# syncdoth/face_mask_inpaint

Hardware: AMD Instinct MI355X
Metric: train images/sec at 256x256 bs=8 per GPU (PICNet-ref train step) (higher is better)
Workload: dtype f32; 1 GPU; train_reference_fill.py PICNet-ref 256x256 fp32, bs=8 per GPU, synthetic CelebA-HQ-shaped batch + random binary_map (BASELINE configs[1]); global_batch=8, parallelism=dp1

## Files before the change

face_mask_inpaint_amd/_lib.py:

```python
from __future__ import annotations

import ctypes as C
import os

_HERE = os.path.dirname(os.path.abspath(__file__))
LIB_PATH = os.path.join(_HERE, "csrc", "libfmi_hip.so")

c_f = C.c_void_p
i32, i64, f32, f64, vp = C.c_int, C.c_int64, C.c_float, C.c_double, C.c_void_p


class ConvDesc(C.Structure):

    _fields_ = [(n, C.c_int) for n in ("N", "H", "W", "C", "OH", "OW", "K", "x_cstride", "y_cstride", "kh", "kw", "stride", "pad", "pad_mode", "dil")] + [("w3", C.c_void_p), ("x3", C.c_void_p), ("y3", C.c_void_p)]


class WeightEntry(C.Structure):
    _fields_ = [("w", vp), ("u", vp), ("v", vp), ("wf", vp), ("wt", vp), ("sigma", vp), ("rows", i32), ("C", i32), ("taps", i32), ("iters", i32), ("wf3", vp), ("wt3", vp)]


class WeightGradEntry(C.Structure):
    _fields_ = [("w", vp), ("u", vp), ("v", vp), ("sigma", vp), ("dwf", vp), ("dw", vp), ("rows", i32), ("C", i32), ("taps", i32), ("pad_", i32)]


class AdamEntry(C.Structure):
    _fields_ = [("p", vp), ("g", vp), ("m", vp), ("v", vp), ("n", i64)]


class RangerEntry(C.Structure):
    _fields_ = [("p", vp), ("g", vp), ("m", vp), ("v", vp), ("slow", vp), ("row_mean", vp), ("n", i64), ("cols", i64)]


PD = C.POINTER(ConvDesc)

SIGNATURES = {
    "fmi_gemm_f32": [vp, vp, vp, i32, i32, i32, i64, i64, i64, i64, i64, i64, i32, i64, i64, i64, f32, f32, vp, vp],
    "fmi_ssim_valid_f32": [vp, vp, vp, i32, i32, i32, i32, f32, f32, vp, vp, i64, vp],
    "fmi_avgpool2_pad_f32": [vp, vp, i32, i32, i32, i32, i32, vp],
    "fmi_resample_u8": [vp, vp, i32, i32, i32, i32, i32, i32, i32, i32, vp, vp, i32, vp],
    "fmi_gather_u8_i64": [vp, vp, i32, i32, i32, i32, i32, vp, vp, vp],
    "fmi_u8_lut_chw_f32": [vp, vp, vp, i32, i32, i32, i32, vp],
    "fmi_split3_f32": [vp, vp, vp, i64, i32, i32, f32, vp],
    "fmi_split3_colsum_f32": [vp, vp, vp, i64, i32, vp],
    "fmi_merge3_f32": [vp, vp, i64, i32, vp],
    "fmi_conv2d_fwd_f32": [PD, vp, vp, vp, vp, vp, i32, i32, i64, vp],
    "fmi_conv2d_dgrad_f32": [PD, vp, vp, vp, vp, vp, i32, i64, vp],
    "fmi_conv_transpose2d_pair_f32": [PD, vp, vp, i32, vp, vp, vp, vp],
    "fmi_conv_transpose2d_pair_bwd_f32": [PD, vp, vp, i32, vp, vp, vp, vp, vp, vp, vp, vp, vp, i64, vp],
    "fmi_conv2d_dgrad_masked_f32": [PD, vp, vp, vp, f32, vp, vp],
    "fmi_conv2d_dgrad_masked_add_f32": [PD, vp, vp, vp, f32, vp, vp, vp],
    "fmi_conv2d_wgrad_f32": [PD, vp, vp, vp, vp, i32, i64, vp],
    "fmi_conv2d_thin_fwd_f32": [PD, vp, vp, vp, vp, vp, i32, vp],
    "fmi_conv2d_thin_dgrad_f32": [PD, vp, vp, vp, vp],
    "fmi_conv2d_thin_input_dgrad_f32": [PD, vp, vp, vp, vp],
    "fmi_conv2d_thin_in_fwd_f32": [PD, vp, vp, vp, vp, vp, i32, vp],
    "fmi_conv2d_thin_in_wgrad_f32": [PD, vp, vp, vp, vp, vp, i64, vp],
    "fmi_conv2d_thin_lrelu_fwd_f32": [PD, vp, f32, vp, vp, vp, i32, vp],
    "fmi_conv2d_thin_lrelu_fwd_bf16": [PD, vp, f32, vp, vp, vp, i32, vp],
    "fmi_conv2d_thin_lrelu_dgrad_f32": [PD, vp, vp, vp, f32, vp, vp],
    "fmi_conv2d_thin_lrelu_wgrad_f32": [PD, vp, f32, vp, vp, vp, vp],
    "fmi_conv2d_thin_wgrad_f32": [PD, vp, vp, vp, vp, vp],
    "fmi_conv2d_thin_lrelu_bwd_f32": [PD, vp, f32, vp, vp, vp, vp, vp, vp, vp, i64, vp],
    "fmi_conv2d_fwd_bf16": [PD, vp, vp, vp, vp, vp, i64, vp],
    "fmi_conv2d_dgrad_bf16": [PD, vp, vp, vp, vp, vp, i64, vp],
    "fmi_conv2d_wgrad_bf16": [PD, vp, vp, vp, vp],
    "fmi_pack_weight_bf16": [vp, vp, i32, i32, i32, vp],
    "fmi_scale_channels_bf16": [vp, vp, vp, i32, i64, i32, vp],
    "fmi_scale_channels_gs_bf16": [vp, vp, vp, vp, i64, i32, i64, i32, vp],
    "fmi_noise_bias_act_bf16": [vp, vp, vp, vp, vp, i64, i32, f32, f32, vp],
    "fmi_noise_bias_act_bwd_bf16": [vp, vp, vp, vp, vp, vp, vp, i64, i64, i32, f32, f32, vp],
    "fmi_upfirdn2d_nhwc_bf16": [vp, vp, vp] + [i32] * 14 + [vp],
    "fmi_styled_out_bwd_bf16": [vp] * 11 + [i64, vp, i32, i64, i32, f32, f32, vp],
    "fmi_conv2d_fwd_act_bf16": [PD, vp, vp, vp, vp, vp, vp, f32, f32, vp, vp],
    "fmi_conv2d_fwd_chan_bf16": [PD, vp, vp, vp, vp, vp, vp, vp, i64, vp],
    "fmi_se_gate_f32": [vp, i32, i64, f32, vp, vp, vp, i32, i32, vp],
    "fmi_irse_tail_bf16": [vp] * 8 + [i32] * 7 + [vp],
    "fmi_irse_stem_bf16": [vp] * 5 + [i64, i32, vp],
    "fmi_conv2d_thin_in_fwd_bf16": [PD, vp, vp, vp, f32, vp, vp],
    "fmi_conv2d_c32_fwd_bf16": [PD, vp, vp, vp, f32, vp, vp],
    "fmi_resblock_tail_bf16": [vp] * 5 + [i32] * 5 + [f32, vp],
    "fmi_picnet_stem_tail_bf16": [vp] * 6 + [i32] * 5 + [f32, vp],
    "fmi_guided_attention_fwd_bf16": [vp] * 5 + [i32] * 5 + [vp],
    "fmi_blur_act_bf16": [vp, vp, vp] + [i32] * 8 + [vp, vp, vp, vp, f32, f32, i32, vp],
    "fmi_torgb_fwd_bf16": [vp, vp, vp, vp, vp, vp, i32, i64, i32, vp],
    "fmi_torgb_bwd_bf16": [vp, vp, vp, vp, vp, vp, i64, vp, vp, vp, i32, i64, i32, vp],
    "fmi_bias_grad_f32": [vp, i64, i32, i32, vp, vp],
    "fmi_reflect_pad_fold_f32": [vp, vp, i32, i32, i32, i32, i32, vp],
    "fmi_weight_prepare_f32": [vp, i32, vp],
    "fmi_weight_grad_f32": [vp, i32, vp, vp],
    "fmi_softmax_rows_f32": [vp, vp, i64, i32, vp],
    "fmi_softmax_rows_bwd_f32": [vp, vp, vp, i64, i32, vp],
    "fmi_attention_fwd_f32": [vp, vp, vp, vp, vp, vp, i32, i32, i32, i32, i32, vp],
    "fmi_attention_fwd_bf16": [vp] * 6 + [i32] * 5 + [vp],
    "fmi_attention_bwd_f32": [vp] * 12 + [i32] * 5 + [vp],
    "fmi_attention_fwd_image_bytes": [i32, i32, i32, i32, i32, C.POINTER(i64)],
    "fmi_attention_fwd_pieces_f32": [vp] * 4 + [i64] + [vp] * 3 + [i32] * 5 + [vp],
    "fmi_attention_bwd_image_bytes": [i32, i32, i32, i32, i32, C.POINTER(i64)],
    "fmi_attention_bwd_pieces_f32": [vp] * 10 + [i64] + [vp] * 3 + [i32] * 5 + [vp],
    "fmi_eltwise_f32": [i32, vp, vp, vp, i64, f32, vp],
    "fmi_axpy_dev_f32": [vp, vp, vp, vp, i64, vp],
    "fmi_dot_f32": [vp, vp, i64, f32, vp, vp],
    "fmi_mask_binarise_i64": [vp, vp, i64, vp],
    "fmi_mask_mul_f32": [vp, vp, vp, i64, i32, i32, vp],
    "fmi_guide_blend_f32": [vp, vp, vp, vp, i64, i32, i32, vp],
    "fmi_guide_blend_bwd_f32": [vp, vp, vp, vp, i64, i32, i32, vp],
    "fmi_vae_sample_f32": [vp, vp, vp, vp, vp, i64, i32, vp],
    "fmi_vae_sample_bwd_f32": [vp, vp, vp, vp, vp, vp, vp, i64, i32, vp],
    "fmi_avgpool_f32": [vp, vp, i32, i32, i32, i32, i32, vp],
    "fmi_avgpool_bwd_f32": [vp, vp, i32, i32, i32, i32, i32, vp],
    "fmi_maxpool2_f32": [vp, vp, i32, i32, i32, i32, vp],
    "fmi_maxpool2_bf16": [vp, vp, i32, i32, i32, i32, vp],
    "fmi_maxpool2_bwd_bf16": [vp, vp, vp, i32, i32, i32, i32, vp],
    "fmi_up2_cat_bf16": [vp, vp, vp, i32, i32, i32, i32, i32, i32, i32, vp],
    "fmi_up2_cat_bwd_bf16": [vp, vp, vp, i32, i32, i32, i32, i32, i32, i32, vp],
    "fmi_head1x1_bf16": [vp, vp, vp, vp, i64, i32, i32, vp],
    "fmi_head1x1_argmax_bf16": [vp, vp, vp, vp, i64, i32, i32, vp],
    "fmi_head1x1_bwd_bf16": [vp, vp, vp, vp, vp, vp, vp, i64, i64, i32, i32, vp],
    "fmi_adaptive_avgpool_f32": [vp, vp, i32, i32, i32, i32, i32, i32, vp],
    "fmi_adaptive_avgpool_bwd_f32": [vp, vp, i32, i32, i32, i32, i32, i32, vp],
    "fmi_maxpool_f32": [vp, vp, vp, i32, i32, i32, i32, i32, i32, vp],
    "fmi_maxpool_bwd_f32": [vp, vp, vp, i32, i32, i32, i32, i32, i32, vp],
    "fmi_argmax_channels_f32": [vp, vp, i64, i32, vp],
    "fmi_image_tail_f32": [vp, vp, vp, vp, i32, i32, f32, f32, vp],
    "fmi_planes_to_u8_f32": [vp, vp, i32, i32, i32, i32, f32, f32, vp],
    "fmi_instnorm_stats_bf16": [vp, vp, vp, i32, i32, i32, f32, vp, i64, vp],
    "fmi_instnorm_apply_bf16": [vp, vp, vp, vp, vp, i32, i32, i32, f32, vp],
    "fmi_instnorm_bwd_reduce_bf16": [vp, vp, vp, vp, vp, vp, i32, i32, i32, f32, vp, i64, vp],
    "fmi_instnorm_bwd_apply_bf16": [vp, vp, vp, vp, vp, vp, vp, vp, vp, vp, i32, i32, i32, f32, vp],
    "fmi_prelu_bf16": [vp, vp, vp, i64, i32, vp],
    "fmi_prelu_bwd_bf16": [vp, vp, vp, vp, vp, vp, i64, i64, i32, vp],
    "fmi_scale_channels_add_bf16": [vp, vp, vp, vp, i32, i64, i32, vp],
    "fmi_add_bf16": [vp, vp, vp, i64, vp],
    "fmi_global_avgpool_bf16": [vp, vp, vp, i64, i32, i64, i32, vp],
    "fmi_add_bcast_bf16": [vp, vp, vp, i32, i64, i32, vp],
    "fmi_add_bcast_f32": [vp, vp, vp, i32, i64, i32, vp],
    "fmi_scale_channels_bwd_f32": [vp, vp, vp, vp, vp, vp, i64, i32, i64, i32, vp],
    "fmi_subsample_bf16": [vp, vp, i32, i32, i32, i32, i32, i32, vp],
    "fmi_scale_channels_add_f32": [vp, vp, vp, vp, i32, i64, i32, vp],
    "fmi_instnorm_bwd_apply_add_f32": [vp, vp, vp, vp, vp, vp, vp, vp, vp, vp, i32, i32, i32, f32, vp],
    "fmi_copy_channels_f32": [vp, vp, i64, i32, i32, i32, i32, i32, vp],
    "fmi_copy_channels_bf16": [vp, vp, i64, i32, i32, i32, i32, i32, vp],
    "fmi_l2norm_rows_f32": [vp, vp, vp, i64, i32, f32, vp],
    "fmi_l2norm_rows_bwd_f32": [vp, vp, vp, vp, i64, i32, f32, vp],
    "fmi_lpips_layer_f32": [vp, vp, vp, vp, i64, i32, f32, vp],
    "fmi_lpips_layer_bwd_f32": [vp, vp, vp, vp, vp, vp, i64, i32, f32, vp],
    "fmi_maxpool2_bwd_f32": [vp, vp, vp, i32, i32, i32, i32, vp],
    "fmi_resize_bilinear_f32": [vp, vp, i32, i32, i32, i32, i32, i32, vp, vp, vp],
    "fmi_resize_bilinear_bwd_f32": [vp, vp, i32, i32, i32, i32, i32, i32, vp, vp],
    "fmi_instnorm_stats_f32": [vp, vp, vp, i32, i32, i32, f32, vp, i64, vp],
    "fmi_batchnorm_running_update_f32": [vp, vp, vp, vp, vp, i32, i64, f32, f32, vp],
    "fmi_batchnorm_running_update_offset_f32": [vp, vp, vp, vp, vp, vp, i32, i64, f32, f32, vp],
    "fmi_instnorm_apply_f32": [vp, vp, vp, vp, vp, i32, i32, i32, f32, vp],
    "fmi_instnorm_bwd_reduce_f32": [vp, vp, vp, vp, vp, vp, i32, i32, i32, f32, vp, i64, vp],
    "fmi_instnorm_bwd_apply_f32": [vp, vp, vp, vp, vp, vp, vp, vp, vp, i32, i32, i32, f32, vp],
    "fmi_reduce_loss_f32": [i32, vp, vp, i64, f32, f32, vp, vp],
    "fmi_reduce_loss_bwd_f32": [i32, vp, vp, i64, f32, f32, vp, vp, vp],
    "fmi_ssim_f32": [vp, vp, vp, i32, i32, i32, i32, i32, vp, vp],
    "fmi_seg_ce_dice_fwd_f32": [vp, vp, i32, i64, i32, f64, vp, vp, vp, i64, vp],
    "fmi_seg_ce_dice_bwd_f32": [vp, vp, i32, i64, i32, f64, vp, vp, vp, vp],
    "fmi_seg_dice_score_f32": [vp, vp, i32, i32, i64, i32, f64, vp, vp, i64, vp],
    "fmi_plane_sums_f32": [vp, vp, i32, i64, vp, vp, i64, vp],
    "fmi_psp_pixel_head_fwd_f32": [vp, vp, vp, vp, vp, vp, vp, vp, i32, i32, i32, i32, vp, i64, vp],
    "fmi_psp_pixel_head_bwd_f32": [vp, vp, vp, vp, vp, vp, vp, vp, i32, i32, i32, i32, vp],
    "fmi_gan_image_head_fwd_f32": [vp, vp, vp, vp, vp, vp, vp, vp, vp, vp, i32, i32, i32, i32, i32, i32, vp, i64, vp],
    "fmi_gan_image_head_bwd_f32": [vp, vp, vp, vp, vp, vp, vp, i32, i32, i32, i32, i32, i32, vp],
    "fmi_cx_channel_mean_f32": [vp, vp, i64, i32, vp],
    "fmi_cx_normalise_f32": [vp, vp, vp, vp, i64, i32, vp],
    "fmi_cx_normalise_bwd_f32": [vp, vp, vp, vp, i64, i32, vp],
    "fmi_cx_rows_f32": [vp, vp, vp, vp, vp, i32, i32, f32, vp],
    "fmi_cx_cols_f32": [vp, vp, vp, i32, i32, vp],
    "fmi_cx_loss_f32": [vp, vp, vp, i32, i32, f32, vp],
    "fmi_cx_bwd_f32": [vp, vp, vp, vp, vp, vp, vp, vp, vp, i32, i32, f32, f32, vp],
    "fmi_adam_step_f32": [vp, i32, i64, f32, f32, f32, f32, f32, i32, vp],
    "fmi_adam_step_dev_f32": [vp, i32, f32, f32, f32, f32, f32, vp, vp],
    "fmi_adam_step_dev_guarded_f32": [vp, i32, f32, f32, f32, f32, f32, vp, vp, vp],
    "fmi_ranger_step_f32": [vp, i32, f32, f32, f32, f32, f32, f32, i32, f32, i32, vp],
    "fmi_upfirdn2d_f32": [vp, vp, vp, i32, i32, i32, i32, i32, i32, i32, i32, i32, i32, i32, i32, i32, vp],
    "fmi_upfirdn2d_bf16": [vp, vp, vp, i32, i32, i32, i32, i32, i32, i32, i32, i32, i32, i32, i32, i32, vp],
    "fmi_fused_bias_act_f32": [vp, vp, vp, vp, i64, i32, i32, i32, i32, f32, f32, vp],
    "fmi_fused_bias_act_bf16": [vp, vp, vp, vp, i64, i32, i32, i32, i32, f32, f32, vp],
    "fmi_scale_channels_f32": [vp, vp, vp, i32, i64, i32, vp],
    "fmi_scale_channels_gs_f32": [vp, vp, vp, vp, i64, i32, i64, i32, vp],
    "fmi_sqsum_last_f32": [vp, vp, i64, i32, vp],
    "fmi_sqsum_last_bwd_f32": [vp, vp, vp, i64, i32, vp],
    "fmi_noise_bias_act_bwd_f32": [vp, vp, vp, vp, vp, i64, i32, f32, f32, vp],
    "fmi_upfirdn2d_nhwc_f32": [vp, vp, vp, i32, i32, i32, i32, i32, i32, i32, i32, i32, i32, i32, i32, i32, i32, vp],
    "fmi_prelu_f32": [vp, vp, vp, i64, i32, vp],
    "fmi_prelu_bwd_f32": [vp, vp, vp, vp, vp, vp, i64, i64, i32, vp],
    "fmi_subsample_f32": [vp, vp, i32, i32, i32, i32, i32, i32, vp],
    "fmi_bias_grad_nchw_f32": [vp, i32, i32, i64, vp, vp],
    "fmi_bias_grad_nchw_bf16": [vp, i32, i32, i64, vp, vp],
    "fmi_noise_bias_act_f32": [vp, vp, vp, vp, vp, i64, i32, f32, f32, vp],
}

STATUS = {0: "ok", 1: "bad argument", 2: "unsupported shape/mode", 3: "kernel launch failed"}


PREDICATES = {"fmi_debug_bf16_tile": [i32], "fmi_set_deterministic": [i32], "fmi_get_deterministic": [], "fmi_conv2d_thin_supported": [PD], "fmi_conv2d_bf16_supported": [PD], "fmi_conv2d_thin_lrelu_supported": [PD], "fmi_conv2d_thin_lrelu_bwd_ws_bytes": [PD], "fmi_conv2d_thin_in_supported": [PD], "fmi_conv2d_thin_in_routed": [PD], "fmi_conv2d_thin_in_wgrad_ws_bytes": [PD], "fmi_conv_transpose2d_pair_bwd_supported": [PD, i32, i32], "fmi_conv_transpose2d_pair_bwd_ws_bytes": [PD, i32, i32], "fmi_attention_fwd_uses_pieces": [i32] * 5, "fmi_attention_bwd_uses_pieces": [i32] * 5, "fmi_attention_fwd_waves": [i32] * 2, "fmi_attention_fwd_bf16_waves": [i32] * 2, "fmi_guided_attention_fwd_bf16_waves": [i32] * 2, "fmi_attention_bwd_structure": [i32] * 2}


class FmiError(RuntimeError):
    pass


class Library:

    def __init__(self, path: str = LIB_PATH, strict: bool = True):
        if not os.path.exists(path):
            raise FmiError(
                f"{path} not found: build the HIP extension first (python -c 'import __graft_entry__ as g; g.build()'). "
                "There is no CPU fallback."
            )
        self.path = path
        self.cdll = C.CDLL(path)
        self.missing = []
        for name, argtypes in SIGNATURES.items():
            try:
                fn = getattr(self.cdll, name)
            except AttributeError:
                self.missing.append(name)
                continue
            fn.argtypes = argtypes
            fn.restype = C.c_int
            setattr(self, name[4:], self._checked(name, fn))
        for name, argtypes in PREDICATES.items():
            try:
                fn = getattr(self.cdll, name)
            except AttributeError:
                self.missing.append(name)
                continue
            fn.argtypes = argtypes
            fn.restype = C.c_int
            setattr(self, name[4:], fn)
        if strict and self.missing:
            raise FmiError(f"{path} lacks symbols {self.missing}")

    @staticmethod
    def _checked(name, fn):
        def call(*args):
            rc = fn(*args)
            if rc != 0:
                raise FmiError(f"{name} failed: {STATUS.get(rc, rc)}")

        call.__name__ = name
        return call


_LIB = None


def lib() -> Library:
    global _LIB
    if _LIB is None:
        _LIB = Library(os.environ.get("FMI_LIB_PATH", LIB_PATH))
    return _LIB
```

face_mask_inpaint_amd/csrc/conv.hip:

```cpp
#include "gemm_core.h"
#include "conv3x3.h"
#include "conv_p3.h"
#include "convt3x3.h"

static bool aligned16(const void* p) { return ((uintptr_t)p & 15) == 0; }
static int ep_vec(const ConvEp& ep, int Nout) {
  return Nout % 4 == 0 && ep.cstride % 4 == 0 && aligned16(ep.y) && aligned16(ep.bias) && aligned16(ep.res) && aligned16(ep.mask);
}

static int check_desc(const fmi_conv_desc* d) {
  if (!d) return FMI_ERR_BAD_ARG;
  if (d->N <= 0 || d->H <= 0 || d->W <= 0 || d->C <= 0 || d->K <= 0 || d->kh <= 0 || d->kw <= 0 || d->stride <= 0 ||
      d->pad < 0 || d->x_cstride < d->C || d->y_cstride < d->K)
    return FMI_ERR_BAD_ARG;
  const int pe = d->pad, dl = d->dil > 1 ? d->dil : 1;
  if (d->dil < 0 || (dl > 1 && d->pad_mode)) return FMI_ERR_BAD_ARG;
  if (d->OH != (d->H + 2 * pe - dl * (d->kh - 1) - 1) / d->stride + 1 || d->OW != (d->W + 2 * pe - dl * (d->kw - 1) - 1) / d->stride + 1)
    return FMI_ERR_BAD_ARG;
  if (d->OH <= 0 || d->OW <= 0) return FMI_ERR_BAD_ARG;
  if (d->pad_mode == 1 && (d->pad >= d->H || d->pad >= d->W)) return FMI_ERR_UNSUPPORTED;
  if (d->pad_mode != 0 && d->pad_mode != 1) return FMI_ERR_UNSUPPORTED;
  if ((int64_t)d->N * d->H * d->W > 0x7fffffffLL / 2 || (int64_t)d->kh * d->kw * d->C > 0x3fffffffLL) return FMI_ERR_UNSUPPORTED;
  return FMI_OK;
}

static ConvGeom fwd_geom(const fmi_conv_desc* d, const float* x, int n_eff) {
  ConvGeom g{};
  g.N = n_eff; g.IH = d->H; g.IW = d->W; g.C = d->C; g.cstride = d->x_cstride;
  g.GH = d->OH; g.GW = d->OW; g.S = d->stride;
  const int dl = d->dil > 1 ? d->dil : 1;
  g.nty = d->kh; g.ntx = d->kw; g.dy0 = -d->pad; g.dx0 = -d->pad; g.ystep = dl; g.xstep = dl;
  g.kh0 = 0; g.kw0 = 0; g.khstep = 1; g.kwstep = 1; g.kw = d->kw;
  g.pad_mode = d->pad_mode;
  g.vec = (d->C % 4 == 0) && (d->x_cstride % 4 == 0) && aligned16(x);
  g.dGW = make_fastdiv(g.GW); g.dG = make_fastdiv(g.GH * g.GW); g.dC = make_fastdiv(g.C); g.dntx = make_fastdiv(g.ntx);
  g.img_bs = (int64_t)d->H * d->W * d->x_cstride;
  return g;
}

static ConvGeom adj_geom(const fmi_conv_desc* d, const float* dy, int n_eff, int py, int px) {
  const int s = d->stride, dl = d->dil > 1 ? d->dil : 1;
  ConvGeom g{};
  g.N = n_eff; g.IH = d->OH; g.IW = d->OW; g.C = d->K; g.cstride = d->y_cstride;
  g.GH = (d->H - py + s - 1) / s; g.GW = (d->W - px + s - 1) / s; g.S = 1;
  g.kh0 = (py + d->pad) % s; g.kw0 = (px + d->pad) % s;
  g.nty = g.kh0 < d->kh ? (d->kh - g.kh0 + s - 1) / s : 0;
  g.ntx = g.kw0 < d->kw ? (d->kw - g.kw0 + s - 1) / s : 0;
  g.dy0 = (py + d->pad - g.kh0) / s; g.dx0 = (px + d->pad - g.kw0) / s;
  g.ystep = -dl; g.xstep = -dl; g.khstep = s; g.kwstep = s; g.kw = d->kw;
  g.pad_mode = 0;
  g.vec = (d->K % 4 == 0) && (d->y_cstride % 4 == 0) && aligned16(dy);
  g.dGW = make_fastdiv(g.GW); g.dG = make_fastdiv(g.GH * g.GW); g.dC = make_fastdiv(g.C);
  g.dntx = make_fastdiv(g.ntx > 0 ? g.ntx : 1);
  g.img_bs = (int64_t)d->OH * d->OW * d->y_cstride;
  if (g.nty == 0 || g.ntx == 0) { g.nty = 0; g.ntx = 1; }
  return g;
}

#ifndef FMI_HOST_EMU
__global__ void __launch_bounds__(256) conv_split_init_kernel(float* __restrict__ y, const float* __restrict__ bias,
                                                             const float* __restrict__ res, int K, int cstride, int64_t total) {
  for (int64_t i = (int64_t)blockIdx.x * 256 + threadIdx.x; i < total; i += (int64_t)gridDim.x * 256) {
    const int k = (int)(i % K);
    const int64_t o = (i / K) * cstride + k;
    float v = bias ? bias[k] : 0.f;
    if (res) v += res[o];
    y[o] = v;
  }
}
#endif

static int conv_ksplit(int64_t M, int N, int K) {
#ifdef FMI_HOST_EMU
  return 1;
#else
  const int64_t tiles = ceil_div64(M, 128) * ceil_div64(N, N <= 32 ? 32 : (N <= 64 ? 64 : 128));
  if (K < 512 || fmi_det()) return 1;
  if (tiles >= 320) {
    if (tiles >= 800 || K < 2304) return 1;
    return tiles <= 520 ? 2 : 3;
  }
  if (tiles >= 192 && K < 4608) return 1;
  int64_t ks = ceil_div64(384, tiles);
  const int64_t kmin = (M <= 128 && tiles <= 16) ? 64 : 256;
  if (ks > K / kmin) ks = K / kmin;
  return ks < 2 ? 1 : (int)(ks > (kmin == 64 ? 64 : 16) ? (kmin == 64 ? 64 : 16) : ks);
#endif
}

static int conv_phase(const fmi_conv_desc* d, const ConvGeom& g, const float* x, const void* x3, const float* w, const void* w3p,
                      int64_t w_bstride, int Nout, int flip, ConvEp ep, int batch_w, bool may_split, bool shared_init, hipStream_t st) {
  ConvK la{x, g};
  ConvWX lb{w, g, w_bstride, Nout, (Nout % 4 == 0) && aligned16(w) && (w_bstride % 4 == 0)};
  const int ks = may_split ? conv_ksplit(g.Mdim(), Nout, g.Kdim()) : 1;
#ifndef FMI_HOST_EMU
  if (shared_init || ks > 1) {
    if (!shared_init) {
      const int64_t total = (int64_t)g.N * ep.OHt * ep.OWt * Nout;
      hipLaunchKernelGGL(conv_split_init_kernel, dim3(fmi_bw_grid(total, 256)), dim3(256), 0, st, ep.y, ep.bias, ep.res, Nout, ep.cstride,
                         total);
    }
    ep.bias = nullptr;
    ep.res = nullptr;
    ep.act = 3;
    ep.vec = 0;
  }
  const uint16_t* w3 = (const uint16_t*)w3p;
  const int64_t w3_stride = (int64_t)d->kh * d->kw * d->C * d->K;
  const int64_t pixels = (int64_t)g.N * g.IH * g.IW;
  const bool tap3 = d->kh == 3 && d->kw == 3 && d->stride == 1 && d->pad == 1 && d->dil <= 1 && g.pad_mode == 0;
  const bool p3 = batch_w == 1 && g.cstride == g.C && g.Kdim() > 0 && p3_generic_ok(g, x3, w3, Nout);
  if (p3 && tap3 && conv3x3_p3_eligible(x3, w3, g.C, Nout, pixels)) {
    const C3P3Args ca{(const uint16_t*)x3, w3, g.N, g.IH, g.IW, g.C, Nout, flip, make_fastdiv(g.IW), make_fastdiv(g.IH * g.IW)};
    return launch_conv3x3_p3(ca, ep, g.Mdim(), ks, st);
  }
  if (p3)
    return launch_gemm_p3(ConvK3{(const uint16_t*)x3, g, make_fastdiv(g.ntaps())}, ConvWX3{w3, g, w3_stride, Nout}, ep, g.Mdim(), Nout,
                          g.Kdim(), ks, st);
  if (batch_w == 1 && tap3 && conv3x3_eligible(x, w, g.C, g.cstride, Nout, pixels)) {
    const C3Args ca{x, w, g.N, g.IH, g.IW, g.C, g.cstride, Nout, flip, make_fastdiv(g.IW), make_fastdiv(g.IH * g.IW), w3};
    return launch_conv3x3(ca, ep, g.Mdim(), ks, st);
  }
  if (w3 && la.dma_ok()) return launch_gemm(la, ConvWX3{w3, g, w3_stride, Nout}, ep, g.Mdim(), Nout, g.Kdim(), 1, ks, st);
#endif
  return launch_gemm(la, lb, ep, g.Mdim(), Nout, g.Kdim(), batch_w, ks, st);
}

static const void* weight_pieces(const fmi_conv_desc* d, int batch_w, int red_c) {
#ifndef FMI_HOST_EMU
  if (batch_w == 1 && red_c % 16 == 0 && aligned16(d->w3)) return d->w3;
#endif
  return nullptr;
}

static int check_y3(const fmi_conv_desc* d, int out_c, int out_cs) {
  if (!d->y3) return FMI_OK;
  return (out_c % 16 == 0 && out_cs == out_c && aligned16(d->y3)) ? FMI_OK : FMI_ERR_BAD_ARG;
}

extern "C" int fmi_conv2d_fwd_f32(const fmi_conv_desc* d, const float* x, const float* wf, const float* bias,
                                  const float* residual, float* y, int act, int batch_w, int64_t w_bstride,
                                  void* stream) {
  if (!d) return FMI_ERR_BAD_ARG;
  int rc = check_y3(d, d->K, d->y_cstride);
  if (rc) return rc;
  rc = check_desc(d);
  if (rc) return rc;
  if (!x || !wf || !y || batch_w < 1 || act < 0 || act > 2) return FMI_ERR_BAD_ARG;
  if (batch_w > 1 && batch_w != d->N) return FMI_ERR_BAD_ARG;
  auto finish = [&](int rc) {
#ifndef FMI_HOST_EMU
    if (rc == FMI_OK && d->y3) rc = fmi_split3_f32(y, d->y3, nullptr, (int64_t)d->N * d->OH * d->OW, d->K, 0, 0.f, stream);
#endif
    return rc;
  };
#ifndef FMI_HOST_EMU
  if (batch_w == 1 && fmi_conv2d_thin_supported(d) && aligned16(x))
    return finish(fmi_conv2d_thin_fwd_f32(d, x, wf, bias, residual, y, act, stream));
  if (batch_w == 1 && d->kh == 3 && fmi_conv2d_thin_in_routed(d) && aligned16(y) && aligned16(residual))
    return finish(fmi_conv2d_thin_in_fwd_f32(d, x, wf, bias, residual, y, act, stream));
#endif
  const ConvGeom g = fwd_geom(d, x, batch_w > 1 ? 1 : d->N);
  const void* w3 = weight_pieces(d, batch_w, d->C);
  ConvEp ep{y, bias, residual, d->OH, d->OW, 1, 0, 0, d->OH, d->OW, d->y_cstride, act, g.dGW, g.dG, (int64_t)d->OH * d->OW * d->y_cstride};
  ep.vec = ep_vec(ep, d->K);
  return finish(conv_phase(d, g, x, d->x3, wf, w3, w_bstride, d->K, 0, ep, batch_w, act == 0 && batch_w == 1, false, (hipStream_t)stream));
}

static int dgrad_impl(const fmi_conv_desc* d, const float* dy, const float* wt, const float* bias, const float* residual,
                      const float* mask, float mslope, float* dx, int batch_w, int64_t w_bstride, void* stream) {
  if (!d) return FMI_ERR_BAD_ARG;
  int rc = check_y3(d, d->C, d->x_cstride);
  if (rc) return rc;
  rc = check_desc(d);
  if (rc) return rc;
  if (!dy || !wt || !dx || batch_w < 1) return FMI_ERR_BAD_ARG;
  if (d->pad_mode != 0) return FMI_ERR_UNSUPPORTED;
  if (batch_w > 1 && batch_w != d->N) return FMI_ERR_BAD_ARG;
  if (mask && bias) return FMI_ERR_UNSUPPORTED;
  auto finish = [&](int rc) {
#ifndef FMI_HOST_EMU
    if (rc == FMI_OK && d->y3) rc = fmi_split3_f32(dx, d->y3, nullptr, (int64_t)d->N * d->H * d->W, d->C, 0, 0.f, stream);
#endif
    return rc;
  };
#ifndef FMI_HOST_EMU
  if (batch_w == 1 && !bias && !residual && !mask && fmi_conv2d_thin_supported(d) && aligned16(dx))
    return finish(fmi_conv2d_thin_dgrad_f32(d, dy, wt, dx, stream));
  if (batch_w == 1 && !bias && !residual && !mask && d->C <= 4 && d->x_cstride == d->C && d->kh == 3) {
    const int rc_thin = fmi_conv2d_thin_input_dgrad_f32(d, dy, wt, dx, stream);
    if (rc_thin != FMI_ERR_UNSUPPORTED) return finish(rc_thin);
  }
#endif
  const int n_eff = batch_w > 1 ? 1 : d->N;
  const int s = d->stride;
  const void* w3 = weight_pieces(d, batch_w, d->K);
  if (d->dil > 1 && s != 1) return FMI_ERR_UNSUPPORTED;
  bool strided_split = false;
#ifndef FMI_HOST_EMU
  if (s > 1 && batch_w == 1) {
    for (int py = 0; py < s && !strided_split; ++py)
      for (int px = 0; px < s && !strided_split; ++px) {
        const ConvGeom g = adj_geom(d, dy, n_eff, py, px);
        if (g.GH > 0 && g.GW > 0 && conv_ksplit(g.Mdim(), d->C, g.Kdim()) > 1) strided_split = true;
      }
    if (strided_split) {
      const int64_t total = (int64_t)d->N * d->H * d->W * d->C;
      hipLaunchKernelGGL(conv_split_init_kernel, dim3(fmi_bw_grid(total, 256)), dim3(256), 0, (hipStream_t)stream, dx, bias, residual, d->C,
                         d->x_cstride, total);
    }
  }
  if (batch_w == 1 && !strided_split && !d->x3 && convt3x3_eligible(d, dy, (const uint16_t*)w3)) {
    CT3Args ca{};
    ca.x = dy; ca.w3 = (const uint16_t*)w3; ca.N = d->N; ca.H = d->OH; ca.W = d->OW; ca.Cred = d->K; ca.cs = d->y_cstride; ca.Nout = d->C;
    ca.dW = make_fastdiv(d->OW); ca.dHW = make_fastdiv(d->OH * d->OW);
    ConvEp ep{dx, bias, residual, d->OH, d->OW, 2, 0, 0, d->H, d->W, d->x_cstride, 0, ca.dW, ca.dHW, (int64_t)d->H * d->W * d->x_cstride};
    ep.mask = mask;
    ep.mslope = mslope;
    ep.vec = ep_vec(ep, d->C);
    ca.ep = ep;
    return finish(launch_convt3x3(ca, d->N * d->OH * d->OW, (hipStream_t)stream));
  }
#endif
  for (int py = 0; py < s; ++py) {
    for (int px = 0; px < s; ++px) {
      const ConvGeom g = adj_geom(d, dy, n_eff, py, px);
      if (g.GH <= 0 || g.GW <= 0) continue;
      ConvEp ep{dx, bias, residual, g.GH, g.GW, s, py, px, d->H, d->W, d->x_cstride, 0, g.dGW, g.dG,
                (int64_t)d->H * d->W * d->x_cstride};
      ep.mask = mask;
      ep.mslope = mslope;
      ep.vec = ep_vec(ep, d->C);
      rc = conv_phase(d, g, dy, d->x3, wt, w3, w_bstride, d->C, 1, ep, batch_w, batch_w == 1 && (s == 1 || strided_split), strided_split,
                      (hipStream_t)stream);
      if (rc) return rc;
    }
  }
  return finish(FMI_OK);
}
extern "C" int fmi_conv2d_dgrad_f32(const fmi_conv_desc* d, const float* dy, const float* wt, const float* bias,
                                    const float* residual, float* dx, int batch_w, int64_t w_bstride, void* stream) {
  return dgrad_impl(d, dy, wt, bias, residual, nullptr, 0.f, dx, batch_w, w_bstride, stream);
}
extern "C" int fmi_conv_transpose2d_pair_f32(const fmi_conv_desc* d, const float* x1, const float* x2, int K2, const void* w3b,
                                             const float* bias, float* y, void* stream) {
  int rc = check_desc(d);
  if (rc) return rc;
  if (!x1 || !x2 || !w3b || !d->w3 || !y || K2 <= 0) return FMI_ERR_BAD_ARG;
#ifndef FMI_HOST_EMU
  const uint16_t* w3 = (d->K % 16 == 0 && aligned16(d->w3)) ? (const uint16_t*)d->w3 : nullptr;
  if (!convt3x3_eligible(d, x1, w3) || (K2 & 15) || !aligned16(x2) || !aligned16(w3b) || d->pad_mode != 0 || d->x3) return FMI_ERR_UNSUPPORTED;
  CT3Args ca{};
  ca.x = x1; ca.w3 = w3; ca.x2 = x2; ca.w3b = (const uint16_t*)w3b; ca.Cred2 = K2; ca.cs2 = K2;
  ca.N = d->N; ca.H = d->OH; ca.W = d->OW; ca.Cred = d->K; ca.cs = d->y_cstride; ca.Nout = d->C;
  ca.dW = make_fastdiv(d->OW); ca.dHW = make_fastdiv(d->OH * d->OW);
  ConvEp ep{y, bias, nullptr, d->OH, d->OW, 2, 0, 0, d->H, d->W, d->x_cstride, 0, ca.dW, ca.dHW, (int64_t)d->H * d->W * d->x_cstride};
  ep.vec = ep_vec(ep, d->C);
  ca.ep = ep;
  return launch_convt3x3(ca, d->N * d->OH * d->OW, (hipStream_t)stream);
#else
  return FMI_ERR_UNSUPPORTED;
#endif
}
extern "C" int fmi_conv2d_dgrad_masked_f32(const fmi_conv_desc* d, const float* dy, const float* wt, const float* mask, float mask_slope,
                                           float* dx, void* stream) {
  if (!mask) return FMI_ERR_BAD_ARG;
  return dgrad_impl(d, dy, wt, nullptr, nullptr, mask, mask_slope, dx, 1, 0, stream);
}

extern "C" int fmi_conv2d_dgrad_masked_add_f32(const fmi_conv_desc* d, const float* dy, const float* wt, const float* mask, float mask_slope,
                                               const float* gadd, float* dx, void* stream) {
  if (!mask || !gadd) return FMI_ERR_BAD_ARG;
  return dgrad_impl(d, dy, wt, nullptr, gadd, mask, mask_slope, dx, 1, 0, stream);
}

extern "C" int fmi_conv2d_wgrad_f32(const fmi_conv_desc* d, const float* x, const float* dy, float* dwf, float* dbias,
                                    int batch_w, int64_t w_bstride, void* stream) {
  int rc = check_desc(d);
  if (rc) return rc;
  if (!x || !dy || !dwf || batch_w < 1) return FMI_ERR_BAD_ARG;
  if (batch_w > 1 && batch_w != d->N) return FMI_ERR_BAD_ARG;
#ifndef FMI_HOST_EMU
  if (batch_w == 1 && fmi_conv2d_thin_supported(d) && aligned16(x)) return fmi_conv2d_thin_wgrad_f32(d, x, dy, dwf, dbias, stream);
#endif
#ifndef FMI_HOST_EMU
  if (batch_w == 1 && !dbias && wgrad_p3_ok(d, d->x3, d->y3))
    return launch_wgrad_p3(d, (const uint16_t*)d->x3, (const uint16_t*)d->y3, dwf, (hipStream_t)stream);
#endif
  const int n_eff = batch_w > 1 ? 1 : d->N;
  ConvGeom g = fwd_geom(d, x, n_eff);
  const bool fuse_bias = dbias && batch_w == 1 && (g.Kdim() % 4 == 0);
  if (dbias && !fuse_bias) return FMI_ERR_UNSUPPORTED;
  const int ones_row = fuse_bias ? g.Kdim() : -1;
  const int Mg = g.Kdim() + (fuse_bias ? 1 : 0), Ng = d->K, Kg = g.Mdim();
  WgradAX la{x, g, ones_row};
  DenseX lb{dy, (int64_t)d->y_cstride, (int64_t)d->OH * d->OW * d->y_cstride, Ng, Kg,
            (d->K % 4 == 0) && (d->y_cstride % 4 == 0) && aligned16(dy)};
  WgradEp ep{dwf, g, d->K, w_bstride, dbias, ones_row};
  const int64_t tiles = ceil_div64(Mg, 128) * ceil_div64(Ng, Ng <= 32 ? 32 : (Ng <= 64 ? 64 : 128));
  int64_t ksplit = 2048 / (tiles * batch_w);
  const int64_t kmax = Kg / 512;
  if (ksplit > kmax) ksplit = kmax;
  if (ksplit < 1) ksplit = 1;
  if (fmi_det()) ksplit = 1;
  if (ksplit * batch_w > 65535) ksplit = 65535 / batch_w;
  return launch_gemm(la, lb, ep, Mg, Ng, Kg, batch_w, (int)ksplit, (hipStream_t)stream);
}

#ifndef FMI_HOST_EMU
__global__ void __launch_bounds__(256) bias_grad_vec_f64_kernel(const float* __restrict__ g, int64_t rows, int K4, float* __restrict__ dbias) {
  __shared__ double part[256][4];
  const int cg = threadIdx.x % K4, rl = threadIdx.x / K4, RL = 256 / K4;
  double s[4] = {0, 0, 0, 0};
  for (int64_t r = rl; r < rows; r += RL) {
    const float4 v = reinterpret_cast<const float4*>(g)[r * K4 + cg];
    s[0] += v.x, s[1] += v.y, s[2] += v.z, s[3] += v.w;
  }
#pragma unroll
  for (int e = 0; e < 4; ++e) part[threadIdx.x][e] = s[e];
  __syncthreads();
  if (threadIdx.x < K4) {
    double t[4] = {0, 0, 0, 0};
    for (int l = 0; l < RL; ++l)
#pragma unroll
      for (int e = 0; e < 4; ++e) t[e] += part[l * K4 + threadIdx.x][e];
#pragma unroll
    for (int e = 0; e < 4; ++e) atomicAdd(dbias + 4 * threadIdx.x + e, (float)t[e]);
  }
}
__global__ void __launch_bounds__(256) bias_grad_vec_kernel(const float* __restrict__ g, int64_t rows, int K4,
                                                            float* __restrict__ dbias, int64_t rows_per_block) {
  __shared__ float4 part[256];
  const int cg = threadIdx.x % K4, rl = threadIdx.x / K4, RL = 256 / K4;
  const int64_t r0 = (int64_t)blockIdx.x * rows_per_block;
  int64_t r1 = r0 + rows_per_block;
  if (r1 > rows) r1 = rows;
  float4 s = make_float4(0.f, 0.f, 0.f, 0.f);
  int64_t r = r0 + rl;
  for (; r + 3 * RL < r1; r += 4 * RL) {
    const float4 v0 = reinterpret_cast<const float4*>(g)[r * K4 + cg];
    const float4 v1 = reinterpret_cast<const float4*>(g)[(r + RL) * K4 + cg];
    const float4 v2 = reinterpret_cast<const float4*>(g)[(r + 2 * RL) * K4 + cg];
    const float4 v3 = reinterpret_cast<const float4*>(g)[(r + 3 * RL) * K4 + cg];
    s.x += (v0.x + v1.x) + (v2.x + v3.x);
    s.y += (v0.y + v1.y) + (v2.y + v3.y);
    s.z += (v0.z + v1.z) + (v2.z + v3.z);
    s.w += (v0.w + v1.w) + (v2.w + v3.w);
  }
  for (; r < r1; r += RL) {
    const float4 v = reinterpret_cast<const float4*>(g)[r * K4 + cg];
    s.x += v.x; s.y += v.y; s.z += v.z; s.w += v.w;
  }
  part[threadIdx.x] = s;
  __syncthreads();
  if (threadIdx.x < K4) {
    float4 t = part[threadIdx.x];
    for (int l = 1; l < RL; ++l) {
      const float4 v = part[l * K4 + threadIdx.x];
      t.x += v.x; t.y += v.y; t.z += v.z; t.w += v.w;
    }
    atomicAdd(dbias + 4 * threadIdx.x + 0, t.x);
    atomicAdd(dbias + 4 * threadIdx.x + 1, t.y);
    atomicAdd(dbias + 4 * threadIdx.x + 2, t.z);
    atomicAdd(dbias + 4 * threadIdx.x + 3, t.w);
  }
}
__global__ void __launch_bounds__(256) bias_grad_kernel(const float* __restrict__ g, int64_t rows, int K, int cstride,
                                                        float* __restrict__ dbias, int64_t rows_per_block) {
  __shared__ float part[4][64];
  const int tx = threadIdx.x & 63, ty = threadIdx.x >> 6;
  const int64_t r0 = (int64_t)blockIdx.x * rows_per_block;
  int64_t r1 = r0 + rows_per_block;
  if (r1 > rows) r1 = rows;
  for (int cg = 0; cg < K; cg += 64) {
    const int c = cg + tx;
    float s = 0.f;
    if (c < K)
      for (int64_t r = r0 + ty; r < r1; r += 4) s += g[r * cstride + c];
    part[ty][tx] = s;
    __syncthreads();
    if (ty == 0 && c < K) atomicAdd(dbias + c, part[0][tx] + part[1][tx] + part[2][tx] + part[3][tx]);
    __syncthreads();
  }
}

extern "C" int fmi_bias_grad_f32(const float* g, int64_t rows, int K, int cstride, float* dbias, void* stream) {
  if (!g || !dbias || rows <= 0 || K <= 0 || cstride < K) return FMI_ERR_BAD_ARG;
// ... 48 lines not shown
```

face_mask_inpaint_amd/csrc/gemm_core.h:

```cpp
#pragma once
#include "common.h"
#include <cstdio>
#include <cstdlib>
extern "C" long fmi_debug_launch_counter;
#include <type_traits>

#ifndef FMI_HOST_EMU
#include "x6.h"
#endif

struct FastDiv {
  uint32_t m, s1, s2, d;
};
static inline FastDiv make_fastdiv(uint32_t d) {
  FastDiv f;
  if (d == 0) d = 1;
  f.d = d;
  uint32_t l = 0;
  while ((1ull << l) < d) ++l;
  f.m = (uint32_t)(((1ull << 32) * ((1ull << l) - d)) / d + 1);
  f.s1 = l < 1 ? l : 1;
  f.s2 = l > 0 ? l - 1 : 0;
  return f;
}
// ... 261 lines not shown
    const uint16_t* q = p3 + (((int64_t)wtap * g.C + c) >> 3) * Nout * 8 + (int64_t)x * 8 + (c & 7);
    const float x0 = __uint_as_float((uint32_t)q[0] << 16), x1 = __uint_as_float((uint32_t)q[pstride] << 16), x2 = __uint_as_float((uint32_t)q[2 * pstride] << 16);
    return (x2 + x1) + x0;
  }
  __device__ __forceinline__ float4 load4(const Ctx&, int x, int k) const { return make_float4(elem(x, k), elem(x + 1, k), elem(x + 2, k), elem(x + 3, k)); }
  __host__ __device__ __forceinline__ bool dma_ok() const { return (g.C & 15) == 0 && ((uintptr_t)p3 & 15) == 0; }
  struct DCtx {
    int64_t off;
  };
  struct Tile {
    const uint16_t* base;
  };
  __device__ __forceinline__ DCtx dprep3(int piece, int kg, int x) const { return DCtx{x < Nout ? piece * pstride + ((int64_t)kg * Nout + x) * 8 : -1}; }
  __device__ __forceinline__ Tile tile(int k0) const {
    const int t = (int)fdiv((uint32_t)k0, g.dC);
    if (t >= g.ntaps()) return Tile{nullptr};
    const int i = (int)fdiv((uint32_t)t, g.dntx), j = t - i * g.ntx;
    const int wtap = (g.kh0 + g.khstep * i) * g.kw + (g.kw0 + g.kwstep * j);
    return Tile{p3 + (((int64_t)wtap * g.C + (k0 - t * g.C)) >> 3) * Nout * 8};
  }
  __device__ __forceinline__ const void* chunk(const DCtx& d, const Tile& t) const { return (d.off >= 0 && t.base) ? (const void*)(t.base + d.off) : nullptr; }
};
#endif

struct WgradAX {
  static constexpr bool KMODE = false;
  const float* p;
  ConvGeom g;
  int ones_row;
  struct Ctx {
    int t0, c0;
  };
  __device__ __forceinline__ void set_batch(int b) { p += (int64_t)b * g.img_bs; }
  __device__ __forceinline__ Ctx prep(int x) const {
    Ctx c;
    c.t0 = (int)fdiv((uint32_t)x, g.dC);
    c.c0 = x - c.t0 * g.C;
    return c;
  }
  __device__ __forceinline__ float elem_tc(int t, int c, int n, int gy, int gx) const {
    if (t >= g.ntaps()) return 0.f;
    const int i = (int)fdiv((uint32_t)t, g.dntx), j = t - i * g.ntx;
    int iy = gy * g.S + g.dy0 + g.ystep * i, ix = gx * g.S + g.dx0 + g.xstep * j;
    if (g.pad_mode) {
      iy = reflect_idx(iy, g.IH);
      ix = reflect_idx(ix, g.IW);
    }
    if ((unsigned)iy >= (unsigned)g.IH || (unsigned)ix >= (unsigned)g.IW) return 0.f;
    return p[((int64_t)(n * g.IH + iy) * g.IW + ix) * g.cstride + c];
  }
  __device__ __forceinline__ float4 load4(const Ctx& cx, int x, int k) const {
    const int t0 = cx.t0, c0 = cx.c0;
    if (k >= g.Mdim()) return zero4();
    if (x == ones_row) return make_float4(1.f, 0.f, 0.f, 0.f);
    const uint32_t n = fdiv((uint32_t)k, g.dG);
    const uint32_t rem = (uint32_t)k - n * (uint32_t)(g.GH * g.GW);
    const uint32_t gy = fdiv(rem, g.dGW);
    const uint32_t gx = rem - gy * (uint32_t)g.GW;
    if (g.vec) {
      if (t0 >= g.ntaps()) return zero4();
      const int i = (int)fdiv((uint32_t)t0, g.dntx), j = t0 - i * g.ntx;
      int iy = (int)gy * g.S + g.dy0 + g.ystep * i, ix = (int)gx * g.S + g.dx0 + g.xstep * j;
      if (g.pad_mode) {
        iy = reflect_idx(iy, g.IH);
        ix = reflect_idx(ix, g.IW);
      }
      if ((unsigned)iy >= (unsigned)g.IH || (unsigned)ix >= (unsigned)g.IW) return zero4();
      return ldg4(p + ((int64_t)((int)n * g.IH + iy) * g.IW + ix) * g.cstride + c0);
    }
    float v[4];
#pragma unroll
    for (int e = 0; e < 4; ++e) {
      const int xe = x + e;
      const int t = (int)fdiv((uint32_t)xe, g.dC);
      v[e] = elem_tc(t, xe - t * g.C, (int)n, (int)gy, (int)gx);
    }
    return make_float4(v[0], v[1], v[2], v[3]);
  }
  __host__ __device__ __forceinline__ bool dma_ok() const { return g.vec != 0; }
  struct DCtx {
    Ctx c;
    int x, kr, dy, dx;
    int k, n, gy, gx;
  };
  struct Tile {
    int k0;
  };
  __device__ __forceinline__ void dstart(DCtx& d, int k_begin) const {
    d.k = k_begin + d.kr;
    const uint32_t n = fdiv((uint32_t)d.k, g.dG);
    const uint32_t rem = (uint32_t)d.k - n * (uint32_t)(g.GH * g.GW);
    const uint32_t gy = fdiv(rem, g.dGW);
    d.n = (int)n;
    d.gy = (int)gy;
    d.gx = (int)(rem - gy * (uint32_t)g.GW);
  }
  __device__ __forceinline__ void advance(DCtx& d) const {
    d.k += 16;
    d.gx += 16;
    while (d.gx >= g.GW) {
      d.gx -= g.GW;
      if (++d.gy == g.GH) {
        d.gy = 0;
        ++d.n;
      }
    }
  }
  __device__ __forceinline__ DCtx dprep(int x, int kr) const {
    DCtx d;
    d.c = prep(x);
    d.x = x;
    d.kr = kr;
    const int i = (int)fdiv((uint32_t)d.c.t0, g.dntx), j = d.c.t0 - i * g.ntx;
    d.dy = g.dy0 + g.ystep * i;
    d.dx = g.dx0 + g.xstep * j;
    return d;
  }
  __device__ __forceinline__ Tile tile(int k0) const { return Tile{k0}; }
  __device__ __forceinline__ const float* chunk(const DCtx& d, const Tile& t) const;
};

struct DenseEp {
  static constexpr bool HAS_VEC4 = false;
  float* c;
  const float* bias;
  int64_t sc_m, sc_n, bs;
  float alpha, beta;
  int atomic;
  __device__ __forceinline__ void set_batch(int b) { c += (int64_t)b * bs; }
  __device__ __forceinline__ int64_t row_off(int row) const { return (int64_t)row * sc_m; }
  __device__ __forceinline__ void store(int64_t off, int col, float v) const {
    float* q = c + off + (int64_t)col * sc_n;
    v *= alpha;
    if (bias) v += bias[col];
    if (atomic) {
      atomicAdd(q, v);
      return;
    }
    if (beta != 0.f) v += beta * *q;
    *q = v;
  }
};

struct ConvEp {
  float* y;
  const float* bias;
  const float* res;
  int GH, GW, OS, py, px, OHt, OWt, cstride, act;
  FastDiv dGW, dG;
  int64_t bs;
  int vec = 0;
  const float* mask = nullptr;
  float mslope = 0.f;
  static constexpr bool HAS_VEC4 = true;
  __device__ __forceinline__ void set_batch(int b) {
    y += (int64_t)b * bs;
    if (res) res += (int64_t)b * bs;
    if (mask) mask += (int64_t)b * bs;
  }
  __device__ __forceinline__ void store4(int64_t off, int col, float4 v) const {
    if (mask) {
      const float4 m4 = *reinterpret_cast<const float4*>(mask + off + col);
      v.x *= m4.x > 0.f ? 1.f : mslope, v.y *= m4.y > 0.f ? 1.f : mslope, v.z *= m4.z > 0.f ? 1.f : mslope, v.w *= m4.w > 0.f ? 1.f : mslope;
    }
    if (bias) {
      const float4 b4 = *reinterpret_cast<const float4*>(bias + col);
      v.x += b4.x, v.y += b4.y, v.z += b4.z, v.w += b4.w;
    }
    if (res) {
      const float4 r4 = *reinterpret_cast<const float4*>(res + off + col);
      v.x += r4.x, v.y += r4.y, v.z += r4.z, v.w += r4.w;
    }
    if (act == 1) v.x = tanhf(v.x), v.y = tanhf(v.y), v.z = tanhf(v.z), v.w = tanhf(v.w);
    else if (act == 2) v.x = fmaxf(v.x, 0.f), v.y = fmaxf(v.y, 0.f), v.z = fmaxf(v.z, 0.f), v.w = fmaxf(v.w, 0.f);
    *reinterpret_cast<float4*>(y + off + col) = v;
  }
  __device__ __forceinline__ int64_t row_off(int row) const {
    const uint32_t n = fdiv((uint32_t)row, dG);
    const uint32_t rem = (uint32_t)row - n * (uint32_t)(GH * GW);
    const uint32_t gy = fdiv(rem, dGW);
    const uint32_t gx = rem - gy * (uint32_t)GW;
    return ((int64_t)((int)n * OHt + (int)gy * OS + py) * OWt + ((int)gx * OS + px)) * cstride;
  }
  __device__ __forceinline__ void store(int64_t off, int col, float v) const {
    if (mask) v *= mask[off + col] > 0.f ? 1.f : mslope;
    if (act == 3) {
      atomicAdd(y + off + col, v);
      return;
    }
    if (bias) v += bias[col];
    if (res) v += res[off + col];
    if (act == 1) v = tanhf(v);
    else if (act == 2) v = fmaxf(v, 0.f);
    y[off + col] = v;
  }
};

struct WgradEp {
  static constexpr bool HAS_VEC4 = false;
  float* dw;
  ConvGeom g;
  int Kout;
  int64_t bs;
  float* dbias;
  int ones_row;
  __device__ __forceinline__ void set_batch(int b) { dw += (int64_t)b * bs; }
  __device__ __forceinline__ int64_t row_off(int row) const {
    if (row == ones_row) return -1;
    const int t = (int)fdiv((uint32_t)row, g.dC);
    const int i = (int)fdiv((uint32_t)t, g.dntx), j = t - i * g.ntx;
    const int wtap = (g.kh0 + g.khstep * i) * g.kw + (g.kw0 + g.kwstep * j);
    return ((int64_t)wtap * g.C + (row - t * g.C)) * Kout;
  }
  __device__ __forceinline__ void store(int64_t off, int col, float v) const {
    if (off < 0) atomicAdd(dbias + col, v);
    else atomicAdd(dw + off + col, v);
  }
};

#ifndef FMI_HOST_EMU
__device__ __forceinline__ float dpp_quad(float v, bool stage2) {
  const int i = __float_as_int(v);
  return __int_as_float(stage2 ? __builtin_amdgcn_mov_dpp(i, 0x4E, 0xF, 0xF, true)
                               : __builtin_amdgcn_mov_dpp(i, 0xB1, 0xF, 0xF, true));
}
__device__ __forceinline__ void quad_transpose(float (&a)[4], int c) {
  const bool b0 = c & 1, b1 = c & 2;
#pragma unroll
  for (int p = 0; p < 4; p += 2) {
    const float recv = dpp_quad(b0 ? a[p] : a[p + 1], false);
    a[p] = b0 ? recv : a[p];
    a[p + 1] = b0 ? a[p + 1] : recv;
  }
#pragma unroll
  for (int q = 0; q < 2; ++q) {
    const float recv = dpp_quad(b1 ? a[q] : a[q + 2], true);
    a[q] = b1 ? recv : a[q];
    a[q + 2] = b1 ? a[q + 2] : recv;
  }
}

template <class EP, class T>
__device__ __forceinline__ void store_tile(const EP& ep, f32x16 (&acc)[T::TM][T::TN], int M, int N, int row0, int col0, int lh, int l31) {
  if constexpr (EP::HAS_VEC4) {
    if (ep.vec) {
      const int c = l31 & 3, colq = l31 & ~3;
#pragma unroll
      for (int i = 0; i < T::TM; ++i) {
#pragma unroll
        for (int g = 0; g < 4; ++g) {
          const int row = row0 + i * 32 + 8 * g + 4 * lh + c;
          const int64_t off = row < M ? ep.row_off(row) : 0;
#pragma unroll
          for (int j = 0; j < T::TN; ++j) {
            float a[4] = {acc[i][j][4 * g + 0], acc[i][j][4 * g + 1], acc[i][j][4 * g + 2], acc[i][j][4 * g + 3]};
            quad_transpose(a, c);
            const int col = col0 + j * 32 + colq;
            if (row < M && col < N) ep.store4(off, col, make_float4(a[0], a[1], a[2], a[3]));
          }
        }
      }
      return;
    }
  }
#pragma unroll
  for (int i = 0; i < T::TM; ++i) {
#pragma unroll
    for (int r = 0; r < 16; ++r) {
      const int row = row0 + i * 32 + (r & 3) + 8 * (r >> 2) + 4 * lh;
      if (row >= M) continue;
      const int64_t off = ep.row_off(row);
#pragma unroll
      for (int j = 0; j < T::TN; ++j) {
        const int col = col0 + j * 32 + l31;
        if (col < N) ep.store(off, col, acc[i][j][r]);
      }
    }
  }
}

static __device__ __attribute__((aligned(16))) float fmi_chunk_zero[4] = {0.f, 0.f, 0.f, 0.f};
__device__ __forceinline__ const float* fmi_zero_chunk_ptr() {
  const float* p = fmi_chunk_zero;
  asm volatile("" : "+s"(p));
  return p;
}
static __device__ __attribute__((aligned(16))) float fmi_chunk_one[4] = {1.f, 0.f, 0.f, 0.f};

__device__ __forceinline__ const float* WgradAX::chunk(const DCtx& d, const Tile&) const {
  if (d.k >= g.Mdim()) return nullptr;
  if (d.x == ones_row) return fmi_chunk_one;
  if (d.c.t0 >= g.ntaps()) return nullptr;
  const int n = d.n;
  int iy = d.gy * g.S + d.dy, ix = d.gx * g.S + d.dx;
  if (g.pad_mode) {
    iy = reflect_idx(iy, g.IH);
    ix = reflect_idx(ix, g.IW);
  }
  if ((unsigned)iy >= (unsigned)g.IH || (unsigned)ix >= (unsigned)g.IW) return nullptr;
  return p + ((int64_t)(n * g.IH + iy) * g.IW + ix) * g.cstride + d.c.c0;
}
#endif

#ifndef FMI_HOST_EMU
template <class LA, class LB, class EP, class T>
__global__ void __launch_bounds__(256) gemm_mfma_f32_kernel(LA la, LB lb, EP ep, int M, int N, int K, int tiles_n,
                                                            int ksplit, int kchunk) {
  constexpr int BM = T::BM, BN = T::BN, BK = T::BK, LDA = T::LDA, LDB = T::LDB;
  constexpr int NLA = BM / 64 > 0 ? BM / 64 : 1, NLB = BN / 64 > 0 ? BN / 64 : 1;
  __shared__ __attribute__((aligned(16))) float lds[2 * BK * (LDA + LDB)];
  float* As = lds;
  float* Bs = lds + 2 * BK * LDA;

  const int tid = threadIdx.x, lane = tid & 63, wid = tid >> 6;
  const int l31 = lane & 31, lh = lane >> 5;
  const int lid = xcd_remap(blockIdx.x, gridDim.x);
  const int tile_m = lid / tiles_n, tile_n = lid - tile_m * tiles_n;
  const int zb = blockIdx.y / ksplit, zs = blockIdx.y - zb * ksplit;
  la.set_batch(zb);
  lb.set_batch(zb);
  ep.set_batch(zb);
  const int m0 = tile_m * BM, n0 = tile_n * BN;
  const int k_begin = zs * kchunk;
  int k_end = k_begin + kchunk;
  if (k_end > K) k_end = K;
  const int wm = (wid / T::WN) * T::TM * 32, wn = (wid % T::WN) * T::TN * 32;

  int ax[NLA], ak[NLA], bx[NLB], bk[NLB];
  bool aact[NLA], bact[NLB];
  typename LA::Ctx ca[NLA];
  typename LB::Ctx cb[NLB];
#pragma unroll
  for (int j = 0; j < NLA; ++j) {
    if (LA::KMODE) {
      ax[j] = (tid >> 2) + 64 * j;
      ak[j] = (tid & 3) * 4;
      aact[j] = ax[j] < BM;
    } else {
      const int idx = tid + 256 * j;
      ak[j] = idx / (BM / 4);
      ax[j] = (idx % (BM / 4)) * 4;
      aact[j] = ak[j] < BK;
    }
    ca[j] = la.prep(m0 + ax[j]);
  }
#pragma unroll
  for (int j = 0; j < NLB; ++j) {
    if (LB::KMODE) {
// ... 451 lines not shown
```

face_mask_inpaint_amd/csrc/pool.hip:

```cpp
#include "common.h"


template <int V>
struct VecT;
template <>
struct VecT<1> {
  typedef float T;
  static __device__ __forceinline__ float zero() { return 0.f; }
  static __device__ __forceinline__ void add(float& a, float b) { a += b; }
  static __device__ __forceinline__ void scale(float& a, float s) { a *= s; }
};
template <>
struct VecT<4> {
  typedef float4 T;
  static __device__ __forceinline__ float4 zero() { return make_float4(0.f, 0.f, 0.f, 0.f); }
  static __device__ __forceinline__ void add(float4& a, float4 b) {
    a.x += b.x; a.y += b.y; a.z += b.z; a.w += b.w;
  }
  static __device__ __forceinline__ void scale(float4& a, float s) {
    a.x *= s; a.y *= s; a.z *= s; a.w *= s;
  }
};

template <int V>
__global__ void __launch_bounds__(256) avgpool_kernel(const float* __restrict__ x, float* __restrict__ y, int H, int W,
                                                      int CV, int k, int64_t total) {
  typedef typename VecT<V>::T T;
  const int OH = H / k, OW = W / k;
  const float inv = 1.f / (float)(k * k);
  for (int64_t i = (int64_t)blockIdx.x * 256 + threadIdx.x; i < total; i += (int64_t)gridDim.x * 256) {
    const int c = (int)(i % CV);
    int64_t r = i / CV;
    const int ox = (int)(r % OW);
    r /= OW;
    const int oy = (int)(r % OH);
    const int n = (int)(r / OH);
    T s = VecT<V>::zero();
    for (int a = 0; a < k; ++a)
      for (int b = 0; b < k; ++b)
        VecT<V>::add(s, reinterpret_cast<const T*>(x)[(((int64_t)n * H + oy * k + a) * W + ox * k + b) * CV + c]);
    VecT<V>::scale(s, inv);
    reinterpret_cast<T*>(y)[i] = s;
  }
}
template <int V>
__global__ void __launch_bounds__(256) avgpool_bwd_kernel(const float* __restrict__ gy, float* __restrict__ gx, int H,
                                                          int W, int CV, int k, int64_t total) {
  typedef typename VecT<V>::T T;
  const int OH = H / k, OW = W / k;
  const float inv = 1.f / (float)(k * k);
  for (int64_t i = (int64_t)blockIdx.x * 256 + threadIdx.x; i < total; i += (int64_t)gridDim.x * 256) {
    const int c = (int)(i % CV);
    int64_t r = i / CV;
    const int xx = (int)(r % W);
    r /= W;
    const int yy = (int)(r % H);
    const int n = (int)(r / H);
    T v = VecT<V>::zero();
    if (yy / k < OH && xx / k < OW) {
      v = reinterpret_cast<const T*>(gy)[(((int64_t)n * OH + yy / k) * OW + xx / k) * CV + c];
      VecT<V>::scale(v, inv);
    }
    reinterpret_cast<T*>(gx)[i] = v;
  }
}

__global__ void __launch_bounds__(256) global_avgpool_kernel(const float* __restrict__ x, float* __restrict__ y, int64_t HW, int C4,
                                                            int64_t rows_per_block, float inv) {
  __shared__ float4 part[256];
  const int cg = threadIdx.x % C4, rl = threadIdx.x / C4, RL = 256 / C4;
  const int n = blockIdx.y;
  const int64_t r0 = (int64_t)blockIdx.x * rows_per_block;
  int64_t r1 = r0 + rows_per_block;
  if (r1 > HW) r1 = HW;
  const float4* xp = reinterpret_cast<const float4*>(x) + (int64_t)n * HW * C4;
  float4 s = make_float4(0.f, 0.f, 0.f, 0.f);
  int64_t r = r0 + rl;
  for (; r + RL < r1; r += 2 * RL) {
    const float4 v0 = xp[r * C4 + cg], v1 = xp[(r + RL) * C4 + cg];
    s.x += v0.x + v1.x; s.y += v0.y + v1.y; s.z += v0.z + v1.z; s.w += v0.w + v1.w;
  }
  for (; r < r1; r += RL) {
    const float4 v = xp[r * C4 + cg];
    s.x += v.x; s.y += v.y; s.z += v.z; s.w += v.w;
  }
  part[threadIdx.x] = s;
  __syncthreads();
  if (threadIdx.x < C4) {
    float4 t = part[threadIdx.x];
    for (int l = 1; l < RL; ++l) {
      const float4 v = part[l * C4 + threadIdx.x];
      t.x += v.x; t.y += v.y; t.z += v.z; t.w += v.w;
    }
    float* o = y + ((int64_t)n * C4 + threadIdx.x) * 4;
    atomicAdd(o + 0, t.x * inv);
    atomicAdd(o + 1, t.y * inv);
    atomicAdd(o + 2, t.z * inv);
    atomicAdd(o + 3, t.w * inv);
  }
}

extern "C" int fmi_avgpool_f32(const float* x, float* y, int N, int H, int W, int C, int k, void* stream) {
  if (!x || !y || N <= 0 || H <= 0 || W <= 0 || C <= 0 || k <= 0 || H / k <= 0 || W / k <= 0) return FMI_ERR_BAD_ARG;
  {
    const int C4 = C / 4;
    if (k == H && k == W && k >= 8 && C % 4 == 0 && C4 <= 256 && (C4 & (C4 - 1)) == 0 && fmi_al16(x) && fmi_al16(y) && N <= 65535) {
      const int64_t HW = (int64_t)H * W;
      int64_t blocks = ceil_div64(HW, 128);
      if (blocks * N > 2048) blocks = ceil_div64(2048, N);
      if (fmi_det()) blocks = 1;
      const int64_t rpb = ceil_div64(HW, blocks);
      blocks = ceil_div64(HW, rpb);
      if (hipMemsetAsync(y, 0, (size_t)N * C * sizeof(float), (hipStream_t)stream) != hipSuccess) return FMI_ERR_LAUNCH;
      hipLaunchKernelGGL(global_avgpool_kernel, dim3((unsigned)blocks, (unsigned)N), dim3(256), 0, (hipStream_t)stream, x, y, HW, C4, rpb,
                         1.f / (float)HW);
      return fmi_launch_status();
    }
  }
  const bool v4 = (C % 4 == 0) && fmi_al16(x) && fmi_al16(y);
  const int CV = v4 ? C / 4 : C;
  const int64_t total = (int64_t)N * (H / k) * (W / k) * CV;
  if (v4) hipLaunchKernelGGL((avgpool_kernel<4>), dim3(fmi_bw_grid(total, 256)), dim3(256), 0, (hipStream_t)stream, x, y, H, W, CV, k, total);
  else hipLaunchKernelGGL((avgpool_kernel<1>), dim3(fmi_bw_grid(total, 256)), dim3(256), 0, (hipStream_t)stream, x, y, H, W, CV, k, total);
  return fmi_launch_status();
}
extern "C" int fmi_avgpool_bwd_f32(const float* gy, float* gx, int N, int H, int W, int C, int k, void* stream) {
  if (!gy || !gx || N <= 0 || H <= 0 || W <= 0 || C <= 0 || k <= 0 || H / k <= 0 || W / k <= 0) return FMI_ERR_BAD_ARG;
  const bool v4 = (C % 4 == 0) && fmi_al16(gx) && fmi_al16(gy);
  const int CV = v4 ? C / 4 : C;
  const int64_t total = (int64_t)N * H * W * CV;
  if (v4) hipLaunchKernelGGL((avgpool_bwd_kernel<4>), dim3(fmi_bw_grid(total, 256)), dim3(256), 0, (hipStream_t)stream, gy, gx, H, W, CV, k, total);
  else hipLaunchKernelGGL((avgpool_bwd_kernel<1>), dim3(fmi_bw_grid(total, 256)), dim3(256), 0, (hipStream_t)stream, gy, gx, H, W, CV, k, total);
  return fmi_launch_status();
}

__global__ void __launch_bounds__(256) maxpool2_kernel(const float* __restrict__ x, float* __restrict__ y, int H, int W,
                                                       int C, int64_t total) {
  const int OH = H / 2, OW = W / 2;
  for (int64_t i = (int64_t)blockIdx.x * 256 + threadIdx.x; i < total; i += (int64_t)gridDim.x * 256) {
    const int c = (int)(i % C);
    int64_t r = i / C;
    const int ox = (int)(r % OW);
    r /= OW;
    const int oy = (int)(r % OH);
    const int n = (int)(r / OH);
    const float* p = x + (((int64_t)n * H + oy * 2) * W + ox * 2) * C + c;
    float m = p[0];
    m = fmaxf(m, p[C]);
    m = fmaxf(m, p[(int64_t)W * C]);
    m = fmaxf(m, p[(int64_t)W * C + C]);
    y[i] = m;
  }
}
__global__ void __launch_bounds__(256) maxpool2_bwd_kernel(const float* __restrict__ x, const float* __restrict__ gy,
                                                           float* __restrict__ gx, int H, int W, int C, int64_t total) {
  const int OH = H / 2, OW = W / 2;
  for (int64_t i = (int64_t)blockIdx.x * 256 + threadIdx.x; i < total; i += (int64_t)gridDim.x * 256) {
    const int c = (int)(i % C);
    int64_t r = i / C;
    const int xx = (int)(r % W);
    r /= W;
    const int yy = (int)(r % H);
    const int n = (int)(r / H);
    const int oy = yy >> 1, ox = xx >> 1;
    float g = 0.f;
    if (oy < OH && ox < OW) {
      const float* p = x + (((int64_t)n * H + oy * 2) * W + ox * 2) * C + c;
      const float v0 = p[0], v1 = p[C], v2 = p[(int64_t)W * C], v3 = p[(int64_t)W * C + C];
      int arg = 0;
      float m = v0;
      if (v1 > m) { m = v1; arg = 1; }
      if (v2 > m) { m = v2; arg = 2; }
      if (v3 > m) { m = v3; arg = 3; }
      if (arg == ((yy & 1) * 2 + (xx & 1))) g = gy[(((int64_t)n * OH + oy) * OW + ox) * C + c];
    }
    gx[i] = g;
  }
}
extern "C" int fmi_maxpool2_f32(const float* x, float* y, int N, int H, int W, int C, void* stream) {
  if (!x || !y || N <= 0 || H < 2 || W < 2 || C <= 0) return FMI_ERR_BAD_ARG;
  const int64_t total = (int64_t)N * (H / 2) * (W / 2) * C;
  hipLaunchKernelGGL(maxpool2_kernel, dim3(fmi_bw_grid(total, 256)), dim3(256), 0, (hipStream_t)stream, x, y, H, W, C, total);
  return fmi_launch_status();
}
extern "C" int fmi_maxpool2_bwd_f32(const float* x, const float* gy, float* gx, int N, int H, int W, int C, void* stream) {
  if (!x || !gy || !gx || N <= 0 || H < 2 || W < 2 || C <= 0) return FMI_ERR_BAD_ARG;
  const int64_t total = (int64_t)N * H * W * C;
  hipLaunchKernelGGL(maxpool2_bwd_kernel, dim3(fmi_bw_grid(total, 256)), dim3(256), 0, (hipStream_t)stream, x, gy, gx, H, W, C, total);
  return fmi_launch_status();
}

__global__ void __launch_bounds__(256) resize_kernel(const float* __restrict__ x, float* __restrict__ y, int H, int W, int C,
                                                     int OH, int OW, const float* __restrict__ mean,
                                                     const float* __restrict__ stdv, int64_t total) {
  for (int64_t i = (int64_t)blockIdx.x * 256 + threadIdx.x; i < total; i += (int64_t)gridDim.x * 256) {
    const int c = (int)(i % C);
    int64_t r = i / C;
    const int ox = (int)(r % OW);
    r /= OW;
    const int oy = (int)(r % OH);
    const int n = (int)(r / OH);
    const Lerp ly = lerp_of(oy, H, OH), lx = lerp_of(ox, W, OW);
    const float* b = x + (int64_t)n * H * W * C + c;
    const float v00 = b[((int64_t)ly.i0 * W + lx.i0) * C], v01 = b[((int64_t)ly.i0 * W + lx.i1) * C];
    const float v10 = b[((int64_t)ly.i1 * W + lx.i0) * C], v11 = b[((int64_t)ly.i1 * W + lx.i1) * C];
    float v = ly.l0 * (lx.l0 * v00 + lx.l1 * v01) + ly.l1 * (lx.l0 * v10 + lx.l1 * v11);
    if (mean) v = (v - mean[c]) / stdv[c];
    y[i] = v;
  }
}
__global__ void __launch_bounds__(256) resize_bwd_kernel(const float* __restrict__ gy, float* __restrict__ gx, int H, int W,
                                                         int C, int OH, int OW, const float* __restrict__ stdv,
                                                         int64_t total) {
  for (int64_t i = (int64_t)blockIdx.x * 256 + threadIdx.x; i < total; i += (int64_t)gridDim.x * 256) {
    const int c = (int)(i % C);
    int64_t r = i / C;
    const int ox = (int)(r % OW);
    r /= OW;
    const int oy = (int)(r % OH);
    const int n = (int)(r / OH);
    const Lerp ly = lerp_of(oy, H, OH), lx = lerp_of(ox, W, OW);
    float g = gy[i];
    if (stdv) g = g / stdv[c];
    float* b = gx + (int64_t)n * H * W * C + c;
    atomicAdd(b + ((int64_t)ly.i0 * W + lx.i0) * C, ly.l0 * lx.l0 * g);
    atomicAdd(b + ((int64_t)ly.i0 * W + lx.i1) * C, ly.l0 * lx.l1 * g);
    atomicAdd(b + ((int64_t)ly.i1 * W + lx.i0) * C, ly.l1 * lx.l0 * g);
    atomicAdd(b + ((int64_t)ly.i1 * W + lx.i1) * C, ly.l1 * lx.l1 * g);
  }
}
__global__ void __launch_bounds__(256) resize_bwd_gather_kernel(const float* __restrict__ gy, float* __restrict__ gx, int H, int W, int C,
                                                                int OH, int OW, const float* __restrict__ stdv, int64_t total) {
  for (int64_t i = (int64_t)blockIdx.x * 256 + threadIdx.x; i < total; i += (int64_t)gridDim.x * 256) {
    const int c = (int)(i % C);
    int64_t r = i / C;
    const int ix = (int)(r % W);
    r /= W;
    const int iy = (int)(r % H);
    const int n = (int)(r / H);
    int ylo, yhi, xlo, xhi;
    resize_cands(iy, H, OH, ylo, yhi);
    resize_cands(ix, W, OW, xlo, xhi);
    const float* b = gy + (int64_t)n * OH * OW * C + c;
    float s = 0.f;
    for (int oy = ylo; oy <= yhi; ++oy) {
      const Lerp ly = lerp_of(oy, H, OH);
      const float wy = (ly.i0 == iy ? ly.l0 : 0.f) + (ly.i1 == iy ? ly.l1 : 0.f);
      if (ly.i0 != iy && ly.i1 != iy) continue;
      for (int ox = xlo; ox <= xhi; ++ox) {
        const Lerp lx = lerp_of(ox, W, OW);
        if (lx.i0 != ix && lx.i1 != ix) continue;
        const float wx = (lx.i0 == ix ? lx.l0 : 0.f) + (lx.i1 == ix ? lx.l1 : 0.f);
        float g = b[((int64_t)oy * OW + ox) * C];
        if (stdv) g = g / stdv[c];
        if (ly.i0 == iy && ly.i1 == iy) {
          if (lx.i0 == ix) s += ly.l0 * lx.l0 * g + ly.l1 * lx.l0 * g;
          if (lx.i1 == ix) s += ly.l0 * lx.l1 * g + ly.l1 * lx.l1 * g;
        } else {
          const float w1 = ly.i0 == iy ? ly.l0 : ly.l1;
          if (lx.i0 == ix) s += w1 * lx.l0 * g;
          if (lx.i1 == ix) s += w1 * lx.l1 * g;
        }
        (void)wx;
        (void)wy;
      }
    }
    gx[i] = s;
  }
}
extern "C" int fmi_resize_bilinear_f32(const float* x, float* y, int N, int H, int W, int C, int OH, int OW,
                                       const float* ch_mean, const float* ch_std, void* stream) {
  if (!x || !y || N <= 0 || H <= 0 || W <= 0 || C <= 0 || OH <= 0 || OW <= 0) return FMI_ERR_BAD_ARG;
  if ((ch_mean == nullptr) != (ch_std == nullptr)) return FMI_ERR_BAD_ARG;
  const int64_t total = (int64_t)N * OH * OW * C;
  hipLaunchKernelGGL(resize_kernel, dim3(fmi_bw_grid(total, 256)), dim3(256), 0, (hipStream_t)stream, x, y, H, W, C, OH, OW,
                     ch_mean, ch_std, total);
  return fmi_launch_status();
}
extern "C" int fmi_resize_bilinear_bwd_f32(const float* gy, float* gx, int N, int H, int W, int C, int OH, int OW,
                                           const float* ch_std, void* stream) {
  if (!gy || !gx || N <= 0 || H <= 0 || W <= 0 || C <= 0 || OH <= 0 || OW <= 0) return FMI_ERR_BAD_ARG;
  if (fmi_det()) {
    const int64_t tin = (int64_t)N * H * W * C;
    hipLaunchKernelGGL(resize_bwd_gather_kernel, dim3(fmi_bw_grid(tin, 256)), dim3(256), 0, (hipStream_t)stream, gy, gx, H, W, C, OH, OW, ch_std, tin);
    return fmi_launch_status();
  }
  const int64_t total = (int64_t)N * OH * OW * C;
  hipLaunchKernelGGL(resize_bwd_kernel, dim3(fmi_bw_grid(total, 256)), dim3(256), 0, (hipStream_t)stream, gy, gx, H, W, C, OH,
                     OW, ch_std, total);
  return fmi_launch_status();
}

__device__ __forceinline__ int aap_lo(int i, int L, int OL) { return (int)(((int64_t)i * L) / OL); }
__device__ __forceinline__ int aap_hi(int i, int L, int OL) { return (int)(((int64_t)(i + 1) * L + OL - 1) / OL); }
template <int V>
__global__ void __launch_bounds__(256) adaptive_avgpool_kernel(const float* __restrict__ x, float* __restrict__ y, int H, int W, int OH,
                                                               int OW, int CV, int64_t total) {
  typedef typename VecT<V>::T T;
  for (int64_t i = (int64_t)blockIdx.x * 256 + threadIdx.x; i < total; i += (int64_t)gridDim.x * 256) {
    const int c = (int)(i % CV);
    int64_t r = i / CV;
    const int ox = (int)(r % OW);
    r /= OW;
    const int oy = (int)(r % OH);
    const int n = (int)(r / OH);
    const int y0 = aap_lo(oy, H, OH), y1 = aap_hi(oy, H, OH), x0 = aap_lo(ox, W, OW), x1 = aap_hi(ox, W, OW);
    T s = VecT<V>::zero();
    for (int a = y0; a < y1; ++a)
      for (int b = x0; b < x1; ++b) VecT<V>::add(s, reinterpret_cast<const T*>(x)[(((int64_t)n * H + a) * W + b) * CV + c]);
    VecT<V>::scale(s, 1.f / (float)((y1 - y0) * (x1 - x0)));
    reinterpret_cast<T*>(y)[i] = s;
  }
}
template <int V>
__global__ void __launch_bounds__(256) adaptive_avgpool_bwd_kernel(const float* __restrict__ gy, float* __restrict__ gx, int H, int W,
                                                                   int OH, int OW, int CV, int64_t total) {
  typedef typename VecT<V>::T T;
  for (int64_t i = (int64_t)blockIdx.x * 256 + threadIdx.x; i < total; i += (int64_t)gridDim.x * 256) {
    const int c = (int)(i % CV);
    int64_t r = i / CV;
    const int xx = (int)(r % W);
    r /= W;
    const int yy = (int)(r % H);
    const int n = (int)(r / H);
    int oy0 = (int)(((int64_t)yy * OH) / H);
    while (oy0 > 0 && aap_hi(oy0 - 1, H, OH) > yy) --oy0;
    int ox0 = (int)(((int64_t)xx * OW) / W);
    while (ox0 > 0 && aap_hi(ox0 - 1, W, OW) > xx) --ox0;
    T s = VecT<V>::zero();
    for (int oy = oy0; oy < OH && aap_lo(oy, H, OH) <= yy; ++oy) {
      if (aap_hi(oy, H, OH) <= yy) continue;
      const int hy = aap_hi(oy, H, OH) - aap_lo(oy, H, OH);
      for (int ox = ox0; ox < OW && aap_lo(ox, W, OW) <= xx; ++ox) {
        if (aap_hi(ox, W, OW) <= xx) continue;
        const int hx = aap_hi(ox, W, OW) - aap_lo(ox, W, OW);
        T v = reinterpret_cast<const T*>(gy)[(((int64_t)n * OH + oy) * OW + ox) * CV + c];
        VecT<V>::scale(v, 1.f / (float)(hy * hx));
        VecT<V>::add(s, v);
      }
// ... 130 lines not shown
```

face_mask_inpaint_amd/functional.py:

```python
from __future__ import annotations

import ctypes as C
import math
from typing import List, Optional, Sequence, Tuple

import torch

from . import _lib
from ._lib import ConvDesc, FmiError

EW_LRELU, EW_LRELU_BWD, EW_TANH_BWD, EW_ADD, EW_SCALE, EW_AXPY, EW_MUL, EW_RELU_BWD_OUT, EW_SOFTPLUS, EW_SOFTPLUS_BWD, EW_SUB, EW_RSQRT, EW_RSQRT_BWD, EW_SIGMOID, EW_SIGMOID_BWD = range(15)
ACT_NONE, ACT_TANH, ACT_RELU = 0, 1, 2

ATTN_CHUNK_BYTES = 96 * 1024 * 1024

PROFILE = None


class _prof:
    def __init__(self, tag, flops):
        self.tag, self.flops = tag, flops

    def __enter__(self):
        if PROFILE is not None:
            self.s = torch.cuda.Event(enable_timing=True)
            self.e = torch.cuda.Event(enable_timing=True)
            self.s.record()
        return self

    def __exit__(self, *exc):
        if PROFILE is not None:
            self.e.record()
            PROFILE.append((self.tag, float(self.flops), self.s, self.e))
        return False


class _ZeroSlab:

    SLAB_BYTES = 32 << 20
    MAX_BYTES = 4 << 20
    buf = None
    off = 0

    @classmethod
    def take(cls, shape, device, dtype=torch.float32):
        if isinstance(shape, int):
            shape = (shape,)
        numel = 1
        for d in shape:
            numel *= int(d)
        nbytes = numel * torch.empty((), dtype=dtype).element_size()
        if nbytes > cls.MAX_BYTES or nbytes == 0 or device.type != "cuda" or torch.cuda.is_current_stream_capturing():
            return torch.zeros(shape, device=device, dtype=dtype)
        nbytes_al = (nbytes + 255) & ~255
        if cls.buf is None or cls.buf.device != device or cls.off + nbytes_al > cls.SLAB_BYTES:
            cls.buf = torch.zeros(cls.SLAB_BYTES, device=device, dtype=torch.uint8)
            cls.off = 0
        out = cls.buf[cls.off:cls.off + nbytes].view(dtype).view(shape)
        cls.off += nbytes_al
        return out


def _zeros(shape, device, dtype=torch.float32):
    return _ZeroSlab.take(tuple(shape) if not isinstance(shape, int) else shape, device, dtype)


def _zeros_like(t):
    return _ZeroSlab.take(tuple(t.shape), t.device, t.dtype)


def _L():
    return _lib.lib()


def _typed(name, t):
    return getattr(_L(), f"{name}_{'bf16' if t.dtype == torch.bfloat16 else 'f32'}")


def _st():
    return C.c_void_p(torch.cuda.current_stream().cuda_stream)


def _p(t: Optional[torch.Tensor], off: int = 0):
    if t is None:
        return None
    return C.c_void_p(t.data_ptr() + 4 * off)


def _chk(*ts, dtype=torch.float32):
    for t in ts:
        if t is None:
            continue
        if not t.is_cuda:
            raise FmiError("face_mask_inpaint_amd ops need device tensors (there is no CPU fallback)")
        if t.dtype != dtype:
            raise FmiError(f"expected {dtype}, got {t.dtype}")
        if not t.is_contiguous():
            raise FmiError("expected a contiguous tensor")


class deterministic:

    def __init__(self, on: bool = True):
        self.on = bool(on)

    def __enter__(self):
        self.prev = _L().set_deterministic(1 if self.on else 0)
        return self

    def __exit__(self, *exc):
        _L().set_deterministic(self.prev)
        return False


def to_nhwc(x: torch.Tensor) -> torch.Tensor:
    return x.permute(0, 2, 3, 1).contiguous()


def to_nchw(x: torch.Tensor) -> torch.Tensor:
    return x.permute(0, 3, 1, 2)


def gemm_raw(a_ptr, b_ptr, c_ptr, M, N, K, sa, sb, sc, batch=1, bs=(0, 0, 0), alpha=1.0, beta=0.0, bias=None, tag="gemm"):
    with _prof(f"{tag}|{M}x{N}x{K} b{batch}", 2.0 * M * N * K * batch):
        _L().gemm_f32(a_ptr, b_ptr, c_ptr, M, N, K, sa[0], sa[1], sb[0], sb[1], sc[0], sc[1], batch, bs[0], bs[1], bs[2],
                      alpha, beta, _p(bias), _st())


def eltwise(op: int, a: torch.Tensor, b: Optional[torch.Tensor] = None, p0: float = 0.0, out: Optional[torch.Tensor] = None):
    _chk(a, b)
    y = torch.empty_like(a) if out is None else out
    if a.numel():
        _L().eltwise_f32(op, _p(a), _p(b), _p(y), a.numel(), float(p0), _st())
    return y


def conv_desc(n, h, w, c, k, kh, kw, stride, pad, pad_mode=0, x_cs=None, y_cs=None, dil=1, w3=None, x3=None) -> Tuple[ConvDesc, int, int]:
    oh = (h + 2 * pad - dil * (kh - 1) - 1) // stride + 1
    ow = (w + 2 * pad - dil * (kw - 1) - 1) // stride + 1
    d = ConvDesc(n, h, w, c, oh, ow, k, x_cs or c, y_cs or k, kh, kw, stride, pad, pad_mode, dil)
    if w3 is not None:
        d.w3 = w3.data_ptr()
        if x3 is not None:
            d.x3 = x3.data_ptr()
    return d, oh, ow


P3_ENABLED = True
P3_MIN_PIXELS = 16384
P3_MIN_WORK = 1152
P3_MIN_COUT = 64


def p3_wanted(pixels: int, cred: int, cout: int, taps: int) -> bool:
    return P3_ENABLED and cred % 16 == 0 and cred >= 64 and cout >= P3_MIN_COUT and pixels >= P3_MIN_PIXELS and taps * cout >= P3_MIN_WORK


def p3_of(t: torch.Tensor, lrelu_from: Optional[torch.Tensor] = None, slope: float = 0.0, colsum: Optional[list] = None) -> Optional[torch.Tensor]:
    c = t.shape[-1]
    if c % 16 or t.dtype != torch.float32 or not t.is_cuda or not t.is_contiguous() or t.data_ptr() % 16:
        if lrelu_from is not None:
            eltwise(EW_LRELU, lrelu_from, None, slope, out=t)
        return None
    p = getattr(t, "_fmi_p3", None)
    if p is not None and p[1] == t._version and lrelu_from is None:
        return p[0]
    x3 = torch.empty(t.numel() * 3, device=t.device, dtype=torch.bfloat16)
    if lrelu_from is not None:
        _L().split3_f32(_p(lrelu_from), C.c_void_p(x3.data_ptr()), _p(t), t.numel() // c, c, 1, float(slope), _st())
    elif colsum is not None and c <= 512 and 256 % (c // 8) == 0 and not _L().get_deterministic():
        gb = _zeros(c, t.device, torch.float32)
        _L().split3_colsum_f32(_p(t), C.c_void_p(x3.data_ptr()), _p(gb), t.numel() // c, c, _st())
        colsum.append(gb)
    else:
        _L().split3_f32(_p(t), C.c_void_p(x3.data_ptr()), None, t.numel() // c, c, 0, 0.0, _st())
    t._fmi_p3 = (x3, t._version)
    return x3


class PackedWeight:

    __slots__ = ("wf", "wt", "rows", "C", "kh", "kw", "w3", "wnk")

    def __init__(self, wf, wt, rows, Cc, kh, kw, w3=(None, None)):
        self.wf, self.wt, self.rows, self.C, self.kh, self.kw = wf, wt, rows, Cc, kh, kw
        self.w3 = w3
        self.wnk = None


W3_ENABLED = True
_LAST_W3: List[Tuple[Optional[torch.Tensor], Optional[torch.Tensor]]] = []


class _WeightPrepare(torch.autograd.Function):

    @staticmethod
    def forward(ctx, metas, *ws):
        lib = _L()
        n = len(ws)
        dev = ws[0].device
        sig = torch.ones(n, device=dev, dtype=torch.float32)
        entries = (_lib.WeightEntry * n)()
        wfs, wts, w3s = [], [], []
        for i, (w, meta) in enumerate(zip(ws, metas)):
            u, v = meta[0], meta[1]
            want_w3 = meta[2] if len(meta) > 2 else True
            iters = int(meta[3]) if len(meta) > 3 else 1
            _chk(w, u, v)
            rows, cc, kh, kw = w.shape
            if u is not None and rows > 4096:
                raise FmiError("spectral-norm weight with more than 4096 rows")
            wf = torch.empty((kh * kw, cc, rows), device=dev, dtype=torch.float32)
            wt = torch.empty((kh * kw, rows, cc), device=dev, dtype=torch.float32)
            pieces = W3_ENABLED and want_w3 and kh * kw <= 36 and w.is_cuda
            wf3 = torch.empty(3 * kh * kw * cc * rows, device=dev, dtype=torch.bfloat16) if pieces and cc % 16 == 0 else None
            wt3 = torch.empty(3 * kh * kw * cc * rows, device=dev, dtype=torch.bfloat16) if pieces and rows % 16 == 0 else None
            w3s.append((wf3, wt3))
            e = entries[i]
            e.wf3 = wf3.data_ptr() if wf3 is not None else None
            e.wt3 = wt3.data_ptr() if wt3 is not None else None
            e.w = w.data_ptr()
            e.u = u.data_ptr() if u is not None else None
            e.v = v.data_ptr() if v is not None else None
            e.wf, e.wt = wf.data_ptr(), wt.data_ptr()
            e.sigma = sig.data_ptr() + 4 * i
            e.rows, e.C, e.taps, e.iters = rows, cc, kh * kw, iters
            wfs.append(wf)
            wts.append(wt)
        lib.weight_prepare_f32(entries, n, _st())
        ctx.metas, ctx.ws, ctx.sig = metas, ws, sig
        _LAST_W3[:] = w3s
        ctx.mark_non_differentiable(sig, *wts)
        ctx.set_materialize_grads(False)
        return (sig,) + tuple(wfs) + tuple(wts)

    @staticmethod
    def backward(ctx, _gsig, *gs):
        lib = _L()
        n = len(ctx.ws)
        gwf = gs[:n]
        live = [i for i, g in enumerate(gwf) if g is not None and ctx.needs_input_grad[1 + i]]
        grads: List[Optional[torch.Tensor]] = [None] * n
        if live:
            entries = (_lib.WeightGradEntry * len(live))()
            keep = []
            for j, i in enumerate(live):
                w = ctx.ws[i]
                u, v = ctx.metas[i][0], ctx.metas[i][1]
                g = gwf[i].contiguous()
                dw = torch.empty_like(w)
                keep.append(g)
                e = entries[j]
                e.w = w.data_ptr()
                e.u = u.data_ptr() if u is not None else None
                e.v = v.data_ptr() if v is not None else None
                e.sigma = ctx.sig.data_ptr() + 4 * i
                e.dwf = g.data_ptr()
                e.dw = dw.data_ptr()
                e.rows, e.C, e.taps = w.shape[0], w.shape[1], w.shape[2] * w.shape[3]
                grads[i] = dw
            scratch = _zeros(len(live), ctx.sig.device, torch.float32)
            lib.weight_grad_f32(entries, len(live), _p(scratch), _st())
        return (None,) + tuple(grads)


def prepare_weights(items: Sequence[tuple]) -> List[PackedWeight]:
    metas = tuple(tuple(it[1:]) for it in items)
    ws = tuple(it[0] for it in items)
    n = len(ws)
    res = _WeightPrepare.apply(metas, *ws)
    w3s = list(_LAST_W3)
    _LAST_W3.clear()
    return [PackedWeight(res[1 + i], res[1 + n + i], w.shape[0], w.shape[1], w.shape[2], w.shape[3], w3s[i]) for i, w in enumerate(ws)]


def _act_bwd(g, y, act):
    if act == ACT_TANH:
        return eltwise(EW_TANH_BWD, g, y)
    if act == ACT_RELU:
        return eltwise(EW_RELU_BWD_OUT, g, y)
    return g


class _Conv2d(torch.autograd.Function):

    @staticmethod
    def forward(ctx, x, wf, bias, residual, wt, kh, kw, stride, pad, pad_mode, act, in_act=None, skip_act_bwd=False, dil=1, passthrough=False, w3=(None, None)):
        _chk(x, wf, bias, residual)
        lib = _L()
        x_in = x
        n, h, w, c = x.shape
        k = wf.shape[2]
        use3 = w3[0] is not None and pad_mode == 0 and p3_wanted(n * h * w, c, k, kh * kw)
        x3 = None
        if in_act is not None and in_act[0] == "apply":
            if use3:
                x = torch.empty_like(x_in)
                x3 = p3_of(x, lrelu_from=x_in, slope=in_act[1])
            else:
                x = eltwise(EW_LRELU, x, None, in_act[1])
        elif use3:
            x3 = p3_of(x)
        d, oh, ow = conv_desc(n, h, w, c, k, kh, kw, stride, pad, pad_mode, dil=dil, w3=w3[0], x3=x3)
        ctx.wt3 = w3[1]
        ctx.x3 = x3
        y = torch.empty((n, oh, ow, k), device=x.device, dtype=torch.float32)
        with _prof(f"conv_fwd|{n}x{h}x{w} {c}->{k} k{kh}s{stride}" + (f"d{dil}" if dil > 1 else ""), 2.0 * n * oh * ow * k * c * kh * kw):
            lib.conv2d_fwd_f32(C.byref(d), _p(x), _p(wf), _p(bias), _p(residual), _p(y), act, 1, 0, _st())
        ctx.save_for_backward(x, wf, y if (act and not skip_act_bwd) else None)
        ctx.wt, ctx.cfg, ctx.has = wt, (kh, kw, stride, pad, pad_mode, act), (bias is not None, residual is not None)
        ctx.dil = dil
        ctx.in_slope = None if in_act is None else float(in_act[1])
        ctx.skip_act_bwd = bool(skip_act_bwd)
        if passthrough:
            return y, x_in.view_as(x_in)
        return y

    @staticmethod
    def backward(ctx, gy, gpass=None):
        lib = _L()
        x, wf, y = ctx.saved_tensors
        if gy is None:
            return (gpass,) + (None,) * 15
        kh, kw, stride, pad, pad_mode, act = ctx.cfg
        gy = gy.contiguous()
        if act and not ctx.skip_act_bwd:
            gy = _act_bwd(gy, y, act)
        n, h, w, c = x.shape
        k = wf.shape[2]
        gx = gwf = gb = gres = None
        masked = False
        dil = ctx.dil
        gb_of_split = [] if (ctx.has[0] and ctx.needs_input_grad[2]) else None
        if ctx.needs_input_grad[0]:
            d0, _, _ = conv_desc(n, h, w, c, k, kh, kw, stride, pad, pad_mode, dil=dil)
            if pad_mode == 1 and lib.conv2d_thin_supported(C.byref(d0)):
                gx = torch.empty_like(x)
                with _prof(f"conv_dgrad|{n}x{h}x{w} {c}->{k} k{kh}s{stride}", 2.0 * gy.numel() * c * kh * kw):
                    lib.conv2d_thin_dgrad_f32(C.byref(d0), _p(gy), _p(ctx.wt), _p(gx), _st())
            elif pad_mode == 1:
                hp, wp = h + 2 * pad, w + 2 * pad
                d, _, _ = conv_desc(n, hp, wp, c, k, kh, kw, stride, 0, w3=ctx.wt3)
                gpad = torch.empty((n, hp, wp, c), device=x.device, dtype=torch.float32)
                with _prof(f"conv_dgrad|{n}x{h}x{w} {c}->{k} k{kh}s{stride}", 2.0 * gy.numel() * c * kh * kw):
                    lib.conv2d_dgrad_f32(C.byref(d), _p(gy), _p(ctx.wt), None, None, _p(gpad), 1, 0, _st())
                gx = torch.empty_like(x)
                lib.reflect_pad_fold_f32(_p(gpad), _p(gx), n, h, w, c, pad, _st())
            else:
                oh_, ow_ = gy.shape[1], gy.shape[2]
                gy3 = p3_of(gy, colsum=gb_of_split) if (ctx.wt3 is not None and p3_wanted(n * oh_ * ow_, k, c, kh * kw)) else None
                d, _, _ = conv_desc(n, h, w, c, k, kh, kw, stride, pad, dil=dil, w3=ctx.wt3, x3=gy3)
                gx = torch.empty_like(x)
                with _prof(f"conv_dgrad|{n}x{h}x{w} {c}->{k} k{kh}s{stride}", 2.0 * gy.numel() * c * kh * kw):
                    if ctx.in_slope is not None and gpass is not None:
                        lib.conv2d_dgrad_masked_add_f32(C.byref(d), _p(gy), _p(ctx.wt), _p(x), ctx.in_slope, _p(gpass.contiguous()), _p(gx), _st())
                        masked, gpass = True, None
                    elif ctx.in_slope is not None:
                        lib.conv2d_dgrad_masked_f32(C.byref(d), _p(gy), _p(ctx.wt), _p(x), ctx.in_slope, _p(gx), _st())
                        masked = True
                    elif gpass is not None:
                        lib.conv2d_dgrad_f32(C.byref(d), _p(gy), _p(ctx.wt), None, _p(gpass.contiguous()), _p(gx), 1, 0, _st())
                        gpass = None
                    else:
                        lib.conv2d_dgrad_f32(C.byref(d), _p(gy), _p(ctx.wt), None, None, _p(gx), 1, 0, _st())
            if ctx.in_slope is not None and not masked:
                gx = eltwise(EW_LRELU_BWD, gx, x, ctx.in_slope)
            if gpass is not None:
                gx = eltwise(EW_ADD, gx, gpass.contiguous())
        elif gpass is not None:
            gx = gpass
        if ctx.needs_input_grad[1]:
            d, _, _ = conv_desc(n, h, w, c, k, kh, kw, stride, pad, pad_mode, dil=dil)
            want_gb = ctx.has[0] and ctx.needs_input_grad[2]
            if lib.conv2d_thin_in_routed(C.byref(d)) and gy.data_ptr() % 16 == 0:
                gwf = torch.empty(wf.shape, device=x.device, dtype=torch.float32)
                if want_gb:
                    gb = torch.empty(k, device=x.device, dtype=torch.float32)
                ws_bytes = lib.conv2d_thin_in_wgrad_ws_bytes(C.byref(d))
                ws = _parts_ws(x.device, ws_bytes // 4)
                with _prof(f"conv_wgrad|{n}x{h}x{w} {c}->{k} k{kh}s{stride}", 2.0 * gy.numel() * c * kh * kw):
                    lib.conv2d_thin_in_wgrad_f32(C.byref(d), _p(x), _p(gy), _p(gwf), _p(gb), _p(ws), ws_bytes, _st())
            else:
                gwf = _zeros_like(wf)
                if ctx.x3 is not None and pad_mode == 0 and c % 32 == 0 and k % 16 == 0 and p3_wanted(gy.numel() // k, c, k, kh * kw):
                    gy3 = p3_of(gy, colsum=gb_of_split)
                    if gy3 is not None:
                        d.w3 = None
                        d.x3, d.y3 = ctx.x3.data_ptr(), gy3.data_ptr()
                        want_gb_fused = False
                    else:
                        want_gb_fused = want_gb
                else:
                    want_gb_fused = want_gb
                fuse = want_gb_fused and (kh * kw * c) % 4 == 0
                if fuse:
                    gb = _zeros(k, x.device, torch.float32)
                with _prof(f"conv_wgrad|{n}x{h}x{w} {c}->{k} k{kh}s{stride}", 2.0 * gy.numel() * c * kh * kw):
                    lib.conv2d_wgrad_f32(C.byref(d), _p(x), _p(gy), _p(gwf), _p(gb) if fuse else None, 1, 0, _st())
        if ctx.has[0] and ctx.needs_input_grad[2] and gb is None:
            if gb_of_split:
                gb = gb_of_split[0]
            else:
                gb = _zeros(k, x.device, torch.float32)
                lib.bias_grad_f32(_p(gy), gy.numel() // k, k, k, _p(gb), _st())
        if ctx.has[1] and ctx.needs_input_grad[3]:
            gres = gy
        return gx, gwf, gb, gres, None, None, None, None, None, None, None, None, None, None, None, None


class _ThinConvLReLU(torch.autograd.Function):

    @staticmethod
    def forward(ctx, x, wf, bias, wt, slope, pad_mode, act):
        _chk(x, wf, bias)
        n, h, w, c = x.shape
        k = wf.shape[2]
        d, oh, ow = conv_desc(n, h, w, c, k, 3, 3, 1, 1, pad_mode)
        y = torch.empty((n, oh, ow, k), device=x.device, dtype=torch.float32)
        with _prof(f"conv_fwd|{n}x{h}x{w} {c}->{k} k3s1", 2.0 * n * oh * ow * k * c * 9):
            _L().conv2d_thin_lrelu_fwd_f32(C.byref(d), _p(x), slope, _p(wf), _p(bias), _p(y), act, _st())
        ctx.save_for_backward(x, wf, y if act else None)
        ctx.wt, ctx.cfg, ctx.has_b = wt, (slope, pad_mode, act), bias is not None
        return y

    @staticmethod
    def backward(ctx, gy):
        lib = _L()
        x, wf, y = ctx.saved_tensors
        slope, pad_mode, act = ctx.cfg
        gy = gy.contiguous()
        n, h, w, c = x.shape
        k = wf.shape[2]
        d, _, _ = conv_desc(n, h, w, c, k, 3, 3, 1, 1, pad_mode)
        gx = gwf = gb = None
        if ctx.needs_input_grad[0] and ctx.needs_input_grad[1]:
            yt = None
            if act == ACT_TANH:
                yt = y
            elif act:
                gy = _act_bwd(gy, y, act)
            gx = torch.empty_like(x)
            gwf = torch.empty(wf.shape, device=x.device, dtype=torch.float32)
            if ctx.has_b and ctx.needs_input_grad[2]:
                gb = torch.empty(k, device=x.device, dtype=torch.float32)
            ws_bytes = lib.conv2d_thin_lrelu_bwd_ws_bytes(C.byref(d))
            ws = torch.empty(ws_bytes // 4, device=x.device, dtype=torch.float32)
            with _prof(f"conv_bwd|{n}x{h}x{w} {c}->{k} k3s1", 4.0 * gy.numel() * c * 9):
                lib.conv2d_thin_lrelu_bwd_f32(C.byref(d), _p(x), slope, _p(gy), _p(yt), _p(ctx.wt), _p(gx), _p(gwf), _p(gb), _p(ws), ws_bytes, _st())
            return gx, gwf, gb, None, None, None, None
        if act:
            gy = _act_bwd(gy, y, act)
        if ctx.needs_input_grad[0]:
            gx = torch.empty_like(x)
            with _prof(f"conv_dgrad|{n}x{h}x{w} {c}->{k} k3s1", 2.0 * gy.numel() * c * 9):
                lib.conv2d_thin_lrelu_dgrad_f32(C.byref(d), _p(gy), _p(ctx.wt), _p(x), slope, _p(gx), _st())
        if ctx.needs_input_grad[1]:
            gwf = _zeros_like(wf)
            if ctx.has_b and ctx.needs_input_grad[2]:
                gb = _zeros(k, x.device, torch.float32)
            with _prof(f"conv_wgrad|{n}x{h}x{w} {c}->{k} k3s1", 2.0 * gy.numel() * c * 9):
                lib.conv2d_thin_lrelu_wgrad_f32(C.byref(d), _p(x), slope, _p(gy), _p(gwf), _p(gb), _st())
        elif ctx.has_b and ctx.needs_input_grad[2]:
            gb = _zeros(k, x.device, torch.float32)
            lib.bias_grad_f32(_p(gy), gy.numel() // k, k, k, _p(gb), _st())
        return gx, gwf, gb, None, None, None, None


def lrelu_conv2d(x, pw: PackedWeight, bias=None, slope=0.1, pad=1, pad_mode=0, act=ACT_NONE):
    if x.dtype == torch.float32 and pw.kh == 3 and pw.kw == 3 and pad == 1 and x.is_cuda:
        n, h, w, c = x.shape
        d, _, _ = conv_desc(n, h, w, c, pw.wf.shape[2], 3, 3, 1, 1, pad_mode)
        if _L().conv2d_thin_lrelu_supported(C.byref(d)) and x.data_ptr() % 16 == 0:
            return _ThinConvLReLU.apply(x, pw.wf, bias, pw.wt, float(slope), pad_mode, act)
    return conv2d(leaky_relu(x, slope), pw, bias, None, 1, pad, pad_mode, act)


def conv2d(x, pw: PackedWeight, bias=None, residual=None, stride=1, pad=0, pad_mode=0, act=ACT_NONE, in_act=None, skip_act_bwd=False, dilation=1,
           passthrough=False):
    if x.dtype == BF16:
        if bias is not None or residual is not None or pad_mode or act or in_act is not None or dilation != 1:
            raise FmiError("the bf16 convolution has no bias / residual / activation / reflect-padding / dilation form")
        return _Conv2dBF16.apply(x, pw.wf, pw.wt, pw.kh, pw.kw, stride, pad)
    return _Conv2d.apply(x, pw.wf, bias, residual, pw.wt, pw.kh, pw.kw, stride, pad, pad_mode, act, in_act, skip_act_bwd, int(dilation), bool(passthrough), pw.w3)


BF16 = torch.bfloat16


def _split_ws(out: torch.Tensor, kred: int):
    if out.numel() > (1 << 22) or kred < 1024:
        return None, 0
    ws = torch.zeros(out.numel(), device=out.device, dtype=torch.float32)
    return ws, ws.numel()


def _pack_bf16(src_tab: torch.Tensor) -> torch.Tensor:
    t, a, b = src_tab.shape
    out = torch.empty((b, t, a), device=src_tab.device, dtype=BF16)
    _L().pack_weight_bf16(_p(src_tab), _p(out), t, a, b, _st())
    return out


class _Conv2dBF16(torch.autograd.Function):

    @staticmethod
    def forward(ctx, x, wf, wt, kh, kw, stride, pad):
        _chk(x, dtype=BF16)
        _chk(wf, wt)
        lib = _L()
        n, h, w, c = x.shape
        k = wf.shape[2]
        d, oh, ow = conv_desc(n, h, w, c, k, kh, kw, stride, pad)
        y = torch.empty((n, oh, ow, k), device=x.device, dtype=BF16)
        wnk = _pack_bf16(wf)
        ws, wsn = _split_ws(y, c * kh * kw)
        with _prof(f"conv_fwd_bf16|{n}x{h}x{w} {c}->{k} k{kh}s{stride}", 2.0 * n * oh * ow * k * c * kh * kw):
            lib.conv2d_fwd_bf16(C.byref(d), _p(x), _p(wnk), None, _p(y), _p(ws), wsn, _st())
        ctx.save_for_backward(x, wf, wt)
        ctx.cfg = (kh, kw, stride, pad)
        return y

    @staticmethod
    def backward(ctx, gy):
        lib = _L()
        x, wf, wt = ctx.saved_tensors
        kh, kw, stride, pad = ctx.cfg
        gy = gy.contiguous()
        n, h, w, c = x.shape
        k = wf.shape[2]
        d, _, _ = conv_desc(n, h, w, c, k, kh, kw, stride, pad)
        gx = gwf = None
        if ctx.needs_input_grad[0]:
            gx = torch.empty_like(x)
            wck = _pack_bf16(wt)
            ws, wsn = _split_ws(gx, k * kh * kw)
            with _prof(f"conv_dgrad_bf16|{n}x{h}x{w} {c}->{k} k{kh}s{stride}", 2.0 * gy.numel() * c * kh * kw):
                lib.conv2d_dgrad_bf16(C.byref(d), _p(gy), _p(wck), None, _p(gx), _p(ws), wsn, _st())
        if ctx.needs_input_grad[1]:
            gwf = _zeros_like(wf)
            with _prof(f"conv_wgrad_bf16|{n}x{h}x{w} {c}->{k} k{kh}s{stride}", 2.0 * gy.numel() * c * kh * kw):
                lib.conv2d_wgrad_bf16(C.byref(d), _p(x), _p(gy), _p(gwf), _st())
        return gx, gwf, None, None, None, None, None


class _ConvTranspose2dBF16(torch.autograd.Function):

    @staticmethod
    def forward(ctx, x, wf, wt, kh, kw, stride, pad, out_pad):
        _chk(x, dtype=BF16)
        _chk(wf, wt)
        lib = _L()
        n, h, w, cs = x.shape
        cb = wf.shape[1]
        H = (h - 1) * stride - 2 * pad + kh + out_pad
        W = (w - 1) * stride - 2 * pad + kw + out_pad
        d, oh, ow = conv_desc(n, H, W, cb, cs, kh, kw, stride, pad)
        if (oh, ow) != (h, w):
            raise FmiError("unsupported ConvTranspose2d geometry")
        y = torch.empty((n, H, W, cb), device=x.device, dtype=BF16)
        wck = _pack_bf16(wt)
        ws, wsn = _split_ws(y, cs * kh * kw // (stride * stride))
        with _prof(f"convT_fwd_bf16|{n}x{h}x{w} {cs}->{cb}", 2.0 * x.numel() * cb * kh * kw):
            lib.conv2d_dgrad_bf16(C.byref(d), _p(x), _p(wck), None, _p(y), _p(ws), wsn, _st())
        ctx.save_for_backward(x, wf)
        ctx.cfg, ctx.HW = (kh, kw, stride, pad), (H, W)
        return y

    @staticmethod
    def backward(ctx, gy):
        lib = _L()
        x, wf = ctx.saved_tensors
        kh, kw, stride, pad = ctx.cfg
        H, W = ctx.HW
        gy = gy.contiguous()
        n, h, w, cs = x.shape
        cb = wf.shape[1]
        d, _, _ = conv_desc(n, H, W, cb, cs, kh, kw, stride, pad)
        gx = gwf = None
        if ctx.needs_input_grad[0]:
            gx = torch.empty_like(x)
            wnk = _pack_bf16(wf)
            ws, wsn = _split_ws(gx, cb * kh * kw)
            with _prof(f"convT_dgrad_bf16|{n}x{h}x{w} {cs}->{cb}", 2.0 * x.numel() * cb * kh * kw):
                lib.conv2d_fwd_bf16(C.byref(d), _p(gy), _p(wnk), None, _p(gx), _p(ws), wsn, _st())
        if ctx.needs_input_grad[1]:
            gwf = _zeros_like(wf)
            with _prof(f"convT_wgrad_bf16|{n}x{h}x{w} {cs}->{cb}", 2.0 * x.numel() * cb * kh * kw):
                lib.conv2d_wgrad_bf16(C.byref(d), _p(gy), _p(x), _p(gwf), _st())
        return gx, gwf, None, None, None, None, None, None


def _styled_out_bwd(g, y, noise, d, nw, bias, slope, gain, need_d, need_b, need_nw):
    n, c = y.shape[0], y.shape[-1]
    p = y.numel() // (n * c)
    t = torch.empty_like(y)
    gd = torch.empty((n, c), device=y.device, dtype=torch.float32) if (need_d and d is not None) else None
    gb = torch.empty(c, device=y.device, dtype=torch.float32) if (need_b and bias is not None) else None
    gnw = torch.empty(1, device=y.device, dtype=torch.float32) if (need_nw and noise is not None) else None
    ws = _parts_ws(y.device, max(2048, n) * 3 * c)
    sums = torch.empty(n * 3 * c, device=y.device, dtype=torch.float32)
    with _prof(f"bytes:noise_bias_act_fused_bwd|{tuple(y.shape)}", 3.0 * y.element_size() * y.numel()):
        _L().styled_out_bwd_bf16(_p(g), _p(y), _p(noise), _p(d), _p(nw), _p(bias), _p(t), _p(gd), _p(gb), _p(gnw), _p(ws), ws.numel(), _p(sums),
                                 n, p, c, slope, gain, _st())
    return t, gd, gb, gnw


class _StyledConvBF16(torch.autograd.Function):

    @staticmethod
    def forward(ctx, x, wf, wt, d, noise, nw, bias, kh, kw, pad, slope, gain):
        _chk(x, dtype=BF16)
        _chk(wf, wt, d, noise, nw, bias)
        lib = _L()
        n, h, w, c = x.shape
        k = wf.shape[2]
        dsc, oh, ow = conv_desc(n, h, w, c, k, kh, kw, 1, pad)
        y = torch.empty((n, oh, ow, k), device=x.device, dtype=BF16)
        wnk = _pack_bf16(wf)
        with _prof(f"conv_fwd_bf16|{n}x{h}x{w} {c}->{k} k{kh}s1 +out", 2.0 * n * oh * ow * k * c * kh * kw):
            lib.conv2d_fwd_act_bf16(C.byref(dsc), _p(x), _p(wnk), _p(d), _p(noise), _p(nw), _p(bias), slope, gain, _p(y), _st())
        ctx.save_for_backward(x, wf, wt, d, noise, nw, bias, y)
        ctx.cfg = (kh, kw, pad, slope, gain)
        return y

    @staticmethod
    def backward(ctx, g):
        lib = _L()
        x, wf, wt, d, noise, nw, bias, y = ctx.saved_tensors
        kh, kw, pad, slope, gain = ctx.cfg
        n, h, w, c = x.shape
        k = wf.shape[2]
        ni = ctx.needs_input_grad
        t, gd, gb, gnw = _styled_out_bwd(g.contiguous(), y, noise, d, nw, bias, slope, gain, ni[3], ni[6], ni[5])
        dsc, _, _ = conv_desc(n, h, w, c, k, kh, kw, 1, pad)
        gx = gwf = None
        if ni[0]:
# ... 273 lines not shown
        return eltwise(EW_MUL, g, b), None, g


class _Add(torch.autograd.Function):
    @staticmethod
    def forward(ctx, a, b):
        if a.dtype == BF16:
            _chk(a, b, dtype=BF16)
            y = torch.empty_like(a)
            _L().add_bf16(_p(a), _p(b), _p(y), a.numel(), _st())
            return y
        return eltwise(EW_ADD, a, b)

    @staticmethod
    def backward(ctx, g):
        return g, g


def add(a, b):
    return _Add.apply(a, b)


class _AvgPool(torch.autograd.Function):
    @staticmethod
    def forward(ctx, x, k):
        _chk(x)
        n, h, w, c = x.shape
        y = torch.empty((n, h // k, w // k, c), device=x.device, dtype=torch.float32)
        _L().avgpool_f32(_p(x), _p(y), n, h, w, c, k, _st())
        ctx.shape, ctx.k = x.shape, k
        return y

    @staticmethod
    def backward(ctx, g):
        n, h, w, c = ctx.shape
        gx = torch.empty(ctx.shape, device=g.device, dtype=torch.float32)
        _L().avgpool_bwd_f32(_p(g.contiguous()), _p(gx), n, h, w, c, ctx.k, _st())
        return gx, None


def avg_pool(x, k=2):
    return _AvgPool.apply(x, k)


class _AdaptiveAvgPool(torch.autograd.Function):
    @staticmethod
    def forward(ctx, x, oh, ow):
        _chk(x)
        n, h, w, c = x.shape
        y = torch.empty((n, oh, ow, c), device=x.device, dtype=torch.float32)
        _L().adaptive_avgpool_f32(_p(x), _p(y), n, h, w, c, oh, ow, _st())
        ctx.shape = x.shape
        return y

    @staticmethod
    def backward(ctx, g):
        n, h, w, c = ctx.shape
        gx = torch.empty(ctx.shape, device=g.device, dtype=torch.float32)
        _L().adaptive_avgpool_bwd_f32(_p(g.contiguous()), _p(gx), n, h, w, c, g.shape[1], g.shape[2], _st())
        return gx, None, None


def adaptive_avg_pool(x, oh, ow):
    n, h, w, c = x.shape
    if (h, w) == (oh, ow):
        return x
    if h % oh == 0 and w % ow == 0 and h // oh == w // ow:
        return avg_pool(x, h // oh)
    return _AdaptiveAvgPool.apply(x, int(oh), int(ow))


class _MaxPool(torch.autograd.Function):
    @staticmethod
    def forward(ctx, x, k, stride):
        _chk(x)
        n, h, w, c = x.shape
        oh, ow = (h - k) // stride + 1, (w - k) // stride + 1
        y = torch.empty((n, oh, ow, c), device=x.device, dtype=torch.float32)
        arg = torch.empty((n, oh, ow, c), device=x.device, dtype=torch.int32)
        _L().maxpool_f32(_p(x), _p(y), C.c_void_p(arg.data_ptr()), n, h, w, c, k, stride, _st())
        ctx.save_for_backward(arg)
        ctx.cfg = (x.shape, k, stride)
        return y

    @staticmethod
    def backward(ctx, g):
        (arg,) = ctx.saved_tensors
        (n, h, w, c), k, stride = ctx.cfg
        gx = torch.zeros((n, h, w, c), device=g.device, dtype=torch.float32)
        _L().maxpool_bwd_f32(_p(g.contiguous()), C.c_void_p(arg.data_ptr()), _p(gx), n, h, w, c, k, stride, _st())
        return gx, None, None


def max_pool(x, k, stride):
    if x.dtype == BF16:
        if k != 2 or stride != 2:
            raise FmiError("bf16 max pooling exists for k = 2, stride = 2 only")
        return max_pool2(x)
    if k == 2 and stride == 2 and x.shape[1] % 2 == 0 and x.shape[2] % 2 == 0:
        return max_pool2(x)
    return _MaxPool.apply(x, int(k), int(stride))


def argmax_channels(x_nhwc: torch.Tensor) -> torch.Tensor:
    x = x_nhwc.detach()
    _chk(x)
    out = torch.empty(x.shape[:-1], device=x.device, dtype=torch.float32)
    _L().argmax_channels_f32(_p(x), _p(out), out.numel(), x.shape[-1], _st())
    return out


def _no_grad_input(t, what):
    if t.requires_grad and torch.is_grad_enabled():
        raise FmiError(f"{what} is inference only (no backward): call it under torch.no_grad() or detach the input")
    return t.detach()


def image_tail(image_nhwc: torch.Tensor, want=("pooled", "unit", "u8"), shift: float = 1.0, scale: float = 0.5) -> dict:
    x = _no_grad_input(image_nhwc, "image_tail")
    _chk(x)
    want = tuple(want)
    if not want or any(w not in ("pooled", "unit", "u8") for w in want):
        raise FmiError(f"image_tail: want is a non-empty subset of ('pooled', 'unit', 'u8'), got {want}")
    if x.dim() != 4 or x.shape[3] != 3 or x.shape[1] != x.shape[2]:
        raise FmiError(f"image_tail: expected [N, S, S, 3], got {tuple(x.shape)}")
    n, s = x.shape[0], x.shape[1]
    out = {}
    for k in ("pooled", "unit"):
        if k in want:
            out[k] = torch.empty((n, 3, 256, 256), device=x.device, dtype=torch.float32)
    if "u8" in want:
        out["u8"] = torch.empty((n, 256, 256, 3), device=x.device, dtype=torch.uint8)
    _L().image_tail_f32(_p(x), _p(out.get("pooled")), _p(out.get("unit")), _p(out.get("u8")), n, s, float(shift), float(scale), _st())
    return out


def planes_to_u8(x_nchw: torch.Tensor, shift: float = 0.0, scale: float = 1.0) -> torch.Tensor:
    x = _no_grad_input(x_nchw, "planes_to_u8").contiguous()
    _chk(x)
    n, c, h, w = x.shape
    out = torch.empty((n, h, w, 3), device=x.device, dtype=torch.uint8)
    _L().planes_to_u8_f32(_p(x), _p(out), n, c, h, w, float(shift), float(scale), _st())
    return out


def mask_to_u8(mask: torch.Tensor, shift: float = 1.0, scale: float = 0.5) -> torch.Tensor:
    if mask.dim() != 3:
        raise FmiError(f"mask_to_u8: expected [N, H, W], got {tuple(mask.shape)}")
    return planes_to_u8(mask.unsqueeze(1), shift, scale)


class _MaxPool2(torch.autograd.Function):
    @staticmethod
    def forward(ctx, x):
        _chk(x)
        n, h, w, c = x.shape
        y = torch.empty((n, h // 2, w // 2, c), device=x.device, dtype=torch.float32)
        _L().maxpool2_f32(_p(x), _p(y), n, h, w, c, _st())
        ctx.save_for_backward(x)
        return y

    @staticmethod
    def backward(ctx, g):
        (x,) = ctx.saved_tensors
        n, h, w, c = x.shape
        gx = torch.empty_like(x)
        _L().maxpool2_bwd_f32(_p(x), _p(g.contiguous()), _p(gx), n, h, w, c, _st())
        return gx


class _MaxPool2BF16(torch.autograd.Function):

    @staticmethod
    def forward(ctx, x):
        _chk(x, dtype=BF16)
        n, h, w, c = x.shape
        if h % 2 or w % 2:
            raise FmiError(f"bf16 max pooling needs even H and W, got {h} x {w}")
        y = torch.empty((n, h // 2, w // 2, c), device=x.device, dtype=BF16)
        _L().maxpool2_bf16(_p(x), _p(y), n, h, w, c, _st())
        ctx.save_for_backward(x)
        return y

    @staticmethod
    def backward(ctx, g):
        (x,) = ctx.saved_tensors
        n, h, w, c = x.shape
        gx = torch.empty_like(x)
        _L().maxpool2_bwd_bf16(_p(x), _p(g.contiguous()), _p(gx), n, h, w, c, _st())
        return gx


def max_pool2(x):
    if x.dtype == BF16:
        return _MaxPool2BF16.apply(x)
    return _MaxPool2.apply(x)


class _Up2CatBF16(torch.autograd.Function):

    @staticmethod
    def forward(ctx, x1, skip):
        _chk(x1, skip, dtype=BF16)
        n, h, w, c1 = x1.shape
        n2, H, W, c2 = skip.shape
        if n2 != n or H < 2 * h or W < 2 * w:
            raise FmiError(f"up2_cat: x1 {tuple(x1.shape)} does not fit under the skip {tuple(skip.shape)}")
        y = torch.empty((n, H, W, c2 + c1), device=x1.device, dtype=BF16)
        _L().up2_cat_bf16(_p(x1), _p(skip), _p(y), n, h, w, c1, H, W, c2, _st())
        ctx.cfg = (n, h, w, c1, H, W, c2)
        return y

    @staticmethod
    def backward(ctx, g):
        n, h, w, c1, H, W, c2 = ctx.cfg
        g = g.contiguous()
        gx1 = torch.empty((n, h, w, c1), device=g.device, dtype=BF16)
        gskip = torch.empty((n, H, W, c2), device=g.device, dtype=BF16)
        _L().up2_cat_bwd_bf16(_p(g), _p(gskip), _p(gx1), n, h, w, c1, H, W, c2, _st())
        return gx1, gskip


def up2_cat(x1, skip):
    return _Up2CatBF16.apply(x1, skip)


_HEAD_ROWS = 512


def _head_args(x, w, b):
    _chk(x, dtype=BF16)
    _chk(w, b)
    k, c = w.shape[0], x.shape[-1]
    if w.numel() != k * c or b.numel() != k:
        raise FmiError(f"head1x1: weight {tuple(w.shape)} / bias {tuple(b.shape)} do not match {c} input channels")
    return k, c


class _Head1x1BF16(torch.autograd.Function):

    @staticmethod
    def forward(ctx, x, w, b):
        k, c = _head_args(x, w, b)
        y = torch.empty(x.shape[:-1] + (k,), device=x.device, dtype=torch.float32)
        _L().head1x1_bf16(_p(x), _p(w), _p(b), _p(y), x.numel() // c, c, k, _st())
        ctx.save_for_backward(x, w)
        return y

    @staticmethod
    def backward(ctx, g):
        x, w = ctx.saved_tensors
        k, c = w.shape[0], x.shape[-1]
        g = g.contiguous()
        gx = torch.empty_like(x)
        gw = torch.empty_like(w)
        gb = torch.empty(k, device=x.device, dtype=torch.float32)
        ws = torch.empty(_HEAD_ROWS * (k * c + k), device=x.device, dtype=torch.float64)
        _L().head1x1_bwd_bf16(_p(g), _p(x), _p(w), _p(gx), _p(gw), _p(gb), C.c_void_p(ws.data_ptr()), ws.numel(), x.numel() // c, c, k, _st())
        return gx, gw, gb


def head1x1(x, w, b):
    return _Head1x1BF16.apply(x, w.contiguous(), b.contiguous())


def head1x1_argmax(x, w, b):
    x, w, b = x.detach(), w.detach().contiguous(), b.detach().contiguous()
    k, c = _head_args(x, w, b)
    out = torch.empty(x.shape[:-1], device=x.device, dtype=torch.float32)
    _L().head1x1_argmax_bf16(_p(x), _p(w), _p(b), _p(out), out.numel(), c, k, _st())
    return out


class _ZeroGradOf(torch.autograd.Function):

    @staticmethod
    def forward(ctx, y, param):
        ctx.save_for_backward(param)
        return y.view_as(y)

    @staticmethod
    def backward(ctx, g):
        (param,) = ctx.saved_tensors
        return g, (torch.zeros_like(param) if ctx.needs_input_grad[1] else None)


def zero_grad_of(y, param):
    return _ZeroGradOf.apply(y, param)


def conv_bn_relu_eval_bf16(x, pw: PackedWeight, conv_bias, bn, pad=1):
    if torch.is_grad_enabled():
        raise FmiError("conv_bn_relu_eval_bf16 is the inference form of the bf16 UNet body (eval-mode BatchNorm): gradients must be off "
                       "(torch.no_grad()); train-mode BatchNorm is the path that differentiates")
    _chk(x, dtype=BF16)
    n, h, w, c = x.shape
    k = pw.wf.shape[2]
    ts = (bn.weight, bn.bias, bn.running_var, bn.running_mean) + ((conv_bias,) if conv_bias is not None else ())
    key = None if any(t.requires_grad for t in ts) else tuple((t.data_ptr(), t._version) for t in ts) + (bn.eps, n)
    kept = getattr(bn, "_fmi_fold", None)
    if key is not None and kept is not None and kept[0] == key:
        colscale, bias = kept[1], kept[2]
    else:
        scale = bn.weight / torch.sqrt(bn.running_var + bn.eps)
        bias = (bn.bias - bn.running_mean * scale if conv_bias is None else bn.bias + (conv_bias - bn.running_mean) * scale).contiguous()
        colscale = scale.unsqueeze(0).expand(n, k).contiguous()
        if key is not None:
            object.__setattr__(bn, "_fmi_fold", (key, colscale, bias))
    _chk(colscale, bias)
    dsc, oh, ow = conv_desc(n, h, w, c, k, pw.kh, pw.kw, 1, pad)
    y = torch.empty((n, oh, ow, k), device=x.device, dtype=BF16)
    wnk = _pack_bf16(pw.wf)
    with _prof(f"conv_fwd_bf16|{n}x{h}x{w} {c}->{k} k{pw.kh}s1 +bn", 2.0 * n * oh * ow * k * c * pw.kh * pw.kw):
        _L().conv2d_fwd_act_bf16(C.byref(dsc), _p(x), _p(wnk), _p(colscale), None, None, _p(bias), 0.0, 1.0, _p(y), _st())
    return y


def instance_norm_act_bf16(x, gamma, beta, eps=1e-5, slope=1.0):
    _chk(x, dtype=BF16)
    _chk(gamma, beta)
    lib = _L()
    n, h, w, c = x.shape
    sums, ws = _norm_ws(x.device, n, c)
    stats = torch.empty((n, c, 2), device=x.device, dtype=torch.float32)
    lib.instnorm_stats_bf16(_p(x), C.c_void_p(sums.data_ptr()), _p(stats), n, h * w, c, eps, C.c_void_p(ws.data_ptr()), ws.numel(), _st())
    y = torch.empty_like(x)
    lib.instnorm_apply_bf16(_p(x), _p(stats), _p(gamma), _p(beta), _p(y), n, h * w, c, slope, _st())
    return y


def conv2d_bias_bf16(x, pw: PackedWeight, bias, pad):
    _chk(x, dtype=BF16)
    _chk(bias)
    n, h, w, c = x.shape
    k = pw.wf.shape[2]
    if c % 64 or k % 4:
        raise FmiError(f"the bf16 convolution with a bias stage needs C % 64 == 0 and K % 4 == 0, got {c} -> {k}")
    dsc, oh, ow = conv_desc(n, h, w, c, k, pw.kh, pw.kw, 1, pad)
    y = torch.empty((n, oh, ow, k), device=x.device, dtype=BF16)
    wnk = _pack_bf16(pw.wf)
    with _prof(f"conv_fwd_bf16|{n}x{h}x{w} {c}->{k} k{pw.kh}s1 +bias", 2.0 * n * oh * ow * k * c * pw.kh * pw.kw):
        _L().conv2d_fwd_act_bf16(C.byref(dsc), _p(x), _p(wnk), None, None, None, _p(bias), 1.0, 1.0, _p(y), _st())
    return y


def conv_transpose2d_cat_bf16(x1, pw1: PackedWeight, x2, pw2: PackedWeight, bias=None):
    _chk(x1, x2, dtype=BF16)
    _chk(bias)
    lib = _L()
# ... 1594 lines not shown
```

face_mask_inpaint_amd/modules/loss.py:

```python
from __future__ import annotations

import torch
from torch import nn

from .. import functional as FF
from ..weights import packed
from .pluralistic_model import base_function
from .pluralistic_model.external_function import GANLoss, run_conv

VGG_CFG = [64, 64, "M", 128, 128, "M", 256, 256, 256, "M", 512, 512, 512, "M"]


def _vgg16_features(width_div: int = 1) -> nn.Sequential:
    layers, c_in = [], 3
    for v in VGG_CFG:
        if v == "M":
            layers.append(nn.MaxPool2d(kernel_size=2, stride=2))
        else:
            layers += [nn.Conv2d(c_in, v // width_div, kernel_size=3, padding=1), nn.ReLU(inplace=True)]
            c_in = v // width_div
    return nn.Sequential(*layers)


class VGGLoss(torch.nn.Module):
    def __init__(self, width_div: int = 1):
        super().__init__()
        try:
            import torchvision

            features = torchvision.models.vgg16(pretrained=True).features
        except Exception:
            features = _vgg16_features(width_div)
        blocks = [features[:4].eval(), features[4:9].eval(), features[9:16].eval(), features[16:23].eval()]
        for bl in blocks:
            for p in bl.parameters():
                p.requires_grad = False
        self.blocks = torch.nn.ModuleList(blocks)
        self.register_buffer("mean", torch.tensor([0.485, 0.456, 0.406]).view(1, 3, 1, 1))
        self.register_buffer("std", torch.tensor([0.229, 0.224, 0.225]).view(1, 3, 1, 1))
        self._cache = {}

    def _prepare(self):
        convs = [m for bl in self.blocks for m in bl if isinstance(m, nn.Conv2d)]
        key = tuple((c.weight.data_ptr(), c.weight._version) for c in convs)
        if self._cache.get("key") != key:
            with torch.no_grad():
                pws = FF.prepare_weights([(c.weight, None, None) for c in convs])
            self._cache = {"key": key, "pws": pws}
        for c, pw in zip(convs, self._cache["pws"]):
            object.__setattr__(c, "_fmi_packed", pw)

    def _block(self, bi, x):
        mods = [m for m in self.blocks[bi] if isinstance(m, (nn.MaxPool2d, nn.Conv2d))]
        prev_conv = False
        for i, m in enumerate(mods):
            if isinstance(m, nn.MaxPool2d):
                x = FF.max_pool2(x)
                prev_conv = False
            else:
                next_conv = i + 1 < len(mods) and isinstance(mods[i + 1], nn.Conv2d)
                x = run_conv(m, x, act=FF.ACT_RELU, in_act=("mask", 0.0) if prev_conv else None, skip_act_bwd=next_conv)
                prev_conv = True
        return x

    def _input(self, img):
        x = FF.to_nhwc(img)
        n, h, w, c = x.shape
        oh, ow = (224, 224) if w > 224 else (h, w)
        return FF.resize_bilinear(x, oh, ow, self.mean.view(3).contiguous(), self.std.view(3).contiguous())

    def forward(self, input, target, lossType="perceptual"):
        self._prepare()
        x = self._input(input)
        with torch.no_grad():
            y = self._input(target)
        loss = 0.0
        for i in range(len(self.blocks)):
            x = self._block(i, x)
            with torch.no_grad():
                y = self._block(i, y)
            n, h, w, c = x.shape
            dim = c * h * w
            if lossType == "perceptual":
                loss = loss + FF.l1_loss(x, y) / dim
            elif lossType == "style":
                gx = FF.gram_matrix(x.view(n, h * w, c))
                gy = FF.gram_matrix(y.view(n, h * w, c))
                loss = loss + FF.l1_loss(gx, gy) / (c * c * dim)
            elif lossType == "contextual" and i == 3:
                loss = loss + FF.contextual_loss(x.view(n, h * w, c), y.view(n, h * w, c)) / dim
        return loss


    def forward_multi(self, triples):
        x = torch.cat([self._input(t[0]) for t in triples], 0)
        with torch.no_grad():
            y = torch.cat([self._input(t[1]) for t in triples], 0)
        return self.forward_multi_prepared(x, y, [t[2] for t in triples])

    def forward_multi_prepared(self, x, y, loss_types):
        self._prepare()
        k = len(loss_types)
        n = x.shape[0] // k
        losses = [0.0] * k
        for i in range(len(self.blocks)):
            x = self._block(i, x)
            with torch.no_grad():
                y = self._block(i, y)
            _, h, w, c = x.shape
            dim = c * h * w
            xparts, yparts = x.split(n, 0), y.split(n, 0)
            for j, lossType in enumerate(loss_types):
                xs, ys = xparts[j], yparts[j]
                if lossType == "perceptual":
                    losses[j] = losses[j] + FF.l1_loss(xs, ys) / dim
                elif lossType == "style":
                    gx = FF.gram_matrix(xs.reshape(n, h * w, c))
                    gy = FF.gram_matrix(ys.reshape(n, h * w, c))
                    losses[j] = losses[j] + FF.l1_loss(gx, gy) / (c * c * dim)
                elif lossType == "contextual" and i == 3:
                    losses[j] = losses[j] + FF.contextual_loss(xs.reshape(n, h * w, c), ys.reshape(n, h * w, c)) / dim
        return losses


class GANOptimizer(nn.Module):

    def __init__(self, optimizer_D, optimizer_G, lambda_g=0.01, debug=False, vgg_width_div: int = 1):
        super().__init__()
        self.gan_loss = GANLoss("lsgan")
        self.vgg_loss = VGGLoss(vgg_width_div)
        self.debug = debug
        self.optimizer_D = optimizer_D
        self.optimizer_G = optimizer_G
        self.lambda_perc = 0.1
        self.lambda_style = 250
        self.lambda_cx = 1
        self.lambda_g = lambda_g
        self.early_d = None
        self.fused_head = False

    LOSS_TYPES = ("perceptual", "style", "contextual")

    @staticmethod
    def _masked(img, mask, invert):
        return FF.to_nchw(FF.mask_mul(FF.to_nhwc(img), mask.contiguous(), invert))

    def perceptual_loss(self, gt_img, gen_img):
        return self.vgg_loss(gen_img, gt_img, lossType="perceptual")

    def style_loss(self, gen_img, src_img, src_mask):
        return self.vgg_loss(self._masked(gen_img, src_mask, True), src_img, lossType="style")

    def contextual_loss(self, gen_img, ref_img, src_mask):
        return self.vgg_loss(self._masked(gen_img, src_mask, False), self._masked(ref_img, src_mask, False), lossType="contextual")

    def discriminator_loss(self, netD, real, fake):
        D_real_loss = self.gan_loss(netD(real), True, True)
        D_fake_loss = self.gan_loss(netD(fake.detach()), False, True)
        return (D_real_loss + D_fake_loss) * 0.5

    def generator_loss(self, netD, real, fake, freeze=True, l1=None):
        if freeze:
            base_function._freeze(netD)
        D_fake = netD(fake)
        loss_ad_g = self.gan_loss(D_fake, True, False) * self.lambda_g
        loss_l1_g = FF.l1_loss(FF.to_nhwc(fake), FF.to_nhwc(real)) if l1 is None else l1
        return loss_ad_g + loss_l1_g

    def _head(self, src_img, gt_img, ref_img, gen_img, src_mask):
        return FF.gan_image_head(gen_img, gt_img, src_img, ref_img, src_mask, self.vgg_loss.mean, self.vgg_loss.std)

    def __call__(self, discriminator, src_img, gt_img, ref_img, gen_img, src_mask):
        d_params = [p for p in discriminator.parameters() if p.requires_grad]
        for p in d_params:
            p.requires_grad_(False)
        head = self._head(src_img, gt_img, ref_img, gen_img, src_mask) if self.fused_head else None
        try:
            if head is None:
                G_loss = self.generator_loss(discriminator, gt_img, gen_img, freeze=False)
            else:
                G_loss = self.generator_loss(discriminator, gt_img, gen_img, freeze=False, l1=head[2])
        finally:
            for p in d_params:
                p.requires_grad_(True)
        if head is not None:
            perc, sty, cx = self.vgg_loss.forward_multi_prepared(head[0], head[1], self.LOSS_TYPES)
        else:
            perc, sty, cx = self.vgg_loss.forward_multi([
                (gen_img, gt_img, "perceptual"),
                (self._masked(gen_img, src_mask, True), src_img, "style"),
                (self._masked(gen_img, src_mask, False), self._masked(ref_img, src_mask, False), "contextual")])
        perc_loss, style_loss, cx_loss = perc * self.lambda_perc, sty * self.lambda_style, cx * self.lambda_cx
        G_loss = G_loss + perc_loss + style_loss + cx_loss
        early_d = self.early_d if self.early_d is not None else hasattr(self.optimizer_D, "launch")
        if early_d:
            D_loss = self.discriminator_loss(discriminator, gt_img, gen_img)
            self.optimizer_D.zero_grad()
            D_loss.backward()
            launch = getattr(self.optimizer_D, "launch", None)
            if launch is not None:
                launch()
            self.optimizer_G.zero_grad()
            G_loss.backward()
            self.optimizer_G.step()
            self.optimizer_D.step()
            return D_loss, G_loss, perc_loss, style_loss, cx_loss
        self.optimizer_G.zero_grad()
        G_loss.backward()
        self.optimizer_G.step()
        D_loss = self.discriminator_loss(discriminator, gt_img, gen_img)
        self.optimizer_D.zero_grad()
        D_loss.backward()
        self.optimizer_D.step()
        return D_loss, G_loss, perc_loss, style_loss, cx_loss
# ... 48 lines not shown
```

face_mask_inpaint_amd/modules/pluralistic_model/external_function.py:

```python
from __future__ import annotations

import torch
from torch import nn
from torch.nn import Parameter

from ... import functional as FF
from ...weights import packed, weight_scope


def l2normalize(v, eps=1e-12):
    return v / (v.norm() + eps)


class SpectralNorm(nn.Module):

    def __init__(self, module, name="weight", power_iterations=1):
        super().__init__()
        if not 1 <= int(power_iterations) <= 64:
            raise ValueError("power_iterations must be in 1 .. 64")
        if name != "weight" or not isinstance(module, (nn.Conv2d, nn.ConvTranspose2d)):
            raise NotImplementedError("SpectralNorm wraps the 'weight' of Conv2d / ConvTranspose2d only")
        self.module = module
        self.name = name
        self.power_iterations = power_iterations
        object.__setattr__(module, "_fmi_power_iterations", int(power_iterations))
        if not hasattr(module, name + "_bar"):
            w = getattr(module, name)
            height = w.data.shape[0]
            width = w.view(height, -1).data.shape[1]
            u = Parameter(l2normalize(w.data.new(height).normal_(0, 1)), requires_grad=False)
            v = Parameter(l2normalize(w.data.new(width).normal_(0, 1)), requires_grad=False)
            w_bar = Parameter(w.data)
            del module._parameters[name]
            module.register_parameter(name + "_u", u)
            module.register_parameter(name + "_v", v)
            module.register_parameter(name + "_bar", w_bar)

    def forward(self, x):
        return FF.to_nchw(self.nhwc(FF.to_nhwc(x)))

    def nhwc(self, x_nhwc, residual=None, act=FF.ACT_NONE, pad_mode=0, pad=None):
        with weight_scope(self):
            return run_conv(self.module, x_nhwc, residual=residual, act=act, pad_mode=pad_mode, pad=pad)


def run_conv(conv: nn.Module, x_nhwc, residual=None, act=FF.ACT_NONE, pad_mode=0, pad=None, in_act=None, skip_act_bwd=False, passthrough=False):
    pw = packed(conv)
    if isinstance(conv, nn.ConvTranspose2d):
        if conv.stride[0] != conv.stride[1] or conv.padding[0] != conv.padding[1] or conv.groups != 1:
            raise NotImplementedError("ConvTranspose2d geometry outside the hot path")
        if in_act is not None:
            if in_act[0] != "apply":
                raise NotImplementedError("ConvTranspose2d with a masked input gradient")
            x_nhwc = FF.leaky_relu(x_nhwc, in_act[1])
        return FF.conv_transpose2d(x_nhwc, pw, conv.bias, residual, conv.stride[0], conv.padding[0], conv.output_padding[0])
    if conv.stride[0] != conv.stride[1] or conv.padding[0] != conv.padding[1] or conv.groups != 1 or conv.dilation[0] != conv.dilation[1]:
        raise NotImplementedError("Conv2d geometry outside the hot path")
    p = conv.padding[0] if pad is None else pad
    return FF.conv2d(x_nhwc, pw, conv.bias, residual, conv.stride[0], p, pad_mode, act, in_act, skip_act_bwd, conv.dilation[0], passthrough)


class GANLoss(nn.Module):

    def __init__(self, gan_mode, target_real_label=1.0, target_fake_label=0.0):
        super().__init__()
        self.register_buffer("real_label", torch.tensor(target_real_label))
        self.register_buffer("fake_label", torch.tensor(target_fake_label))
        self.gan_mode = gan_mode
        if gan_mode != "lsgan":
            raise NotImplementedError("gan mode %s not implemented (the reference trainer uses lsgan)" % gan_mode)
        self._labels = (float(target_real_label), float(target_fake_label))

    def __call__(self, prediction, target_is_real, is_disc=False):
        return FF.mse_to_const(prediction, self._labels[0] if target_is_real else self._labels[1])


def _npc(x):
    n, c, h, w = x.shape
    return x.permute(0, 2, 3, 1).contiguous().view(n, h * w, c)


def GramMatrix(input):
    return FF.gram_matrix(_npc(input))


def StyleLoss(input, target):
    target = GramMatrix(target).detach()
    return FF.l1_loss(GramMatrix(input), target)


def contextual_loss(x, y, h=0.5):
    assert x.size() == y.size()
    return FF.contextual_loss(_npc(x), _npc(y).detach(), h)
```

include/fmi_hip.h:

```cpp
#ifndef FMI_HIP_H
#define FMI_HIP_H

#include <stdint.h>

#ifdef __cplusplus
extern "C" {
#endif

typedef enum {
  FMI_OK = 0,
  FMI_ERR_BAD_ARG = 1,
  FMI_ERR_UNSUPPORTED = 2,
  FMI_ERR_LAUNCH = 3
} fmi_status;

const char* fmi_status_string(int status);
int fmi_version(void);
int fmi_set_deterministic(int on);
int fmi_get_deterministic(void);

int fmi_debug_bf16_tile(int mode);

int fmi_gemm_f32(const float* A, const float* B, float* C, int M, int N, int K,
                 int64_t sa_m, int64_t sa_k, int64_t sb_k, int64_t sb_n, int64_t sc_m, int64_t sc_n,
// ... 78 lines not shown
int fmi_scale_channels_gs_bf16(const uint16_t* g, const uint16_t* x, float* gs, float* ws, int64_t ws_floats, int N, int64_t P, int C,
                               void* stream);
int fmi_noise_bias_act_bf16(const uint16_t* x, const float* bias, const float* noise, const float* nw, uint16_t* y, int64_t pixels, int C,
                            float alpha, float scale, void* stream);
int fmi_noise_bias_act_bwd_bf16(const uint16_t* g, const uint16_t* y, const float* noise, uint16_t* gx, float* gnw, float* gbias,
                                float* ws, int64_t ws_floats, int64_t pixels, int C, float alpha, float scale, void* stream);
int fmi_upfirdn2d_nhwc_bf16(const uint16_t* in, const float* kernel, uint16_t* out, int N, int in_h, int in_w, int C, int kh, int kw,
                            int up_x, int up_y, int down_x, int down_y, int pad_x0, int pad_x1, int pad_y0, int pad_y1, void* stream);
int fmi_blur_act_bf16(const uint16_t* in, const float* kernel, uint16_t* out, int N, int in_h, int in_w, int C, int pad_x0, int pad_x1,
                      int pad_y0, int pad_y1, const float* colscale, const float* noise, const float* nw, const float* bias, float slope,
                      float gain, int separable, void* stream);
int fmi_styled_out_bwd_bf16(const uint16_t* g, const uint16_t* y, const float* noise, const float* colscale, const float* nw,
                            const float* bias, uint16_t* t, float* gd, float* gbias, float* gnw, float* ws, int64_t ws_floats, float* sums,
                            int N, int64_t P, int C, float slope, float gain, void* stream);
int fmi_torgb_fwd_bf16(const uint16_t* x, const float* w, const float* s, const float* bias, const float* skip, float* out, int N,
                       int64_t P, int C, void* stream);
int fmi_torgb_bwd_bf16(const uint16_t* x, const float* w, const float* s, const float* g, uint16_t* gx, float* ws, int64_t ws_floats,
                       float* gw, float* gs, float* gbias, int N, int64_t P, int C, void* stream);

int fmi_bias_grad_f32(const float* g, int64_t rows, int K, int cstride, float* dbias, void* stream);
int fmi_reflect_pad_fold_f32(const float* gpad, float* gx, int N, int H, int W, int C, int pad, void* stream);

typedef struct {
  const float* w;
  float* u;
  float* v;
  float* wf;
  float* wt;
  float* sigma;
  int rows, C, taps;
  int iters;
  void* wf3;
  void* wt3;
} fmi_weight_entry;
int fmi_weight_prepare_f32(const fmi_weight_entry* entries, int count, void* stream);

typedef struct {
  const float* w;
  const float* u;
  const float* v;
  const float* sigma;
  const float* dwf;
  float* dw;
  int rows, C, taps, pad_;
} fmi_weight_grad_entry;
int fmi_weight_grad_f32(const fmi_weight_grad_entry* entries, int count, float* scratch_zeroed, void* stream);

int fmi_softmax_rows_f32(const float* x, float* y, int64_t rows, int cols, void* stream);
int fmi_softmax_rows_bwd_f32(const float* p, const float* dp, float* ds, int64_t rows, int cols, void* stream);

int fmi_attention_fwd_f32(const float* q, const float* v1, const float* v2, float* o1, float* o2, float* lse,
                          int N, int T, int D, int C1, int C2, void* stream);

int fmi_attention_fwd_waves(int N, int T);
int fmi_attention_bwd_structure(int N, int T);

int fmi_attention_fwd_bf16_waves(int N, int T);
int fmi_attention_fwd_bf16(const uint16_t* q, const uint16_t* v, uint16_t* o, float* lse, const float* gamma, const uint16_t* residual,
                           int N, int T, int D, int C, int waves, void* stream);

int fmi_attention_fwd_uses_pieces(int N, int T, int D, int C1, int C2);
int fmi_attention_fwd_image_bytes(int N, int T, int D, int C1, int C2, int64_t* bytes);
int fmi_attention_fwd_pieces_f32(const float* q, const float* v1, const float* v2, void* image, int64_t image_bytes, float* o1, float* o2,
                                 float* lse, int N, int T, int D, int C1, int C2, void* stream);

int fmi_attention_bwd_f32(const float* q, const float* v1, const float* v2, const float* o1, const float* o2,
                          const float* go1, const float* go2, const float* lse, float* delta_scratch,
                          float* gv1, float* gv2, float* gq_zeroed, int N, int T, int D, int C1, int C2, void* stream);

int fmi_attention_bwd_uses_pieces(int N, int T, int D, int C1, int C2);
int fmi_attention_bwd_image_bytes(int N, int T, int D, int C1, int C2, int64_t* bytes);
int fmi_attention_bwd_pieces_f32(const float* q, const float* v1, const float* v2, const float* o1, const float* o2,
                                 const float* go1, const float* go2, const float* lse, float* delta_scratch, void* image,
                                 int64_t image_bytes, float* gv1, float* gv2, float* gq_zeroed, int N, int T, int D, int C1, int C2,
                                 void* stream);

enum {
  FMI_EW_LRELU = 0,
  FMI_EW_LRELU_BWD = 1,
  FMI_EW_TANH_BWD = 2,
  FMI_EW_ADD = 3,
  FMI_EW_SCALE = 4,
  FMI_EW_AXPY = 5,
  FMI_EW_MUL = 6,
  FMI_EW_RELU_BWD_OUT = 7,
  FMI_EW_SOFTPLUS = 8,
  FMI_EW_SOFTPLUS_BWD = 9,
  FMI_EW_SUB = 10,
  FMI_EW_RSQRT = 11,
  FMI_EW_RSQRT_BWD = 12,
  FMI_EW_SIGMOID = 13,
  FMI_EW_SIGMOID_BWD = 14,
  FMI_EW_COUNT_
};
int fmi_eltwise_f32(int op, const float* a, const float* b, float* y, int64_t n, float p0, void* stream);
int fmi_axpy_dev_f32(const float* a, const float* s, const float* b, float* y, int64_t n, void* stream);
int fmi_dot_f32(const float* a, const float* b, int64_t n, float scale, float* out, void* stream);

int fmi_mask_binarise_i64(const int64_t* mask, float* out, int64_t n, void* stream);
int fmi_mask_mul_f32(const float* x, const float* m, float* y, int64_t pixels, int C, int invert, void* stream);
int fmi_guide_blend_f32(const float* ref_att, const float* ref, const float* m, float* out,
                        int64_t pixels, int C, int out_cstride, void* stream);
int fmi_guide_blend_bwd_f32(const float* g, const float* m, float* d_ref_att, float* d_ref,
                            int64_t pixels, int C, int g_cstride, void* stream);
int fmi_vae_sample_f32(const float* o_src, const float* o_ref, const float* eps_q, const float* eps_p,
                       float* z, int64_t pixels, int Z, void* stream);
int fmi_vae_sample_bwd_f32(const float* gz, const float* o_src, const float* o_ref, const float* eps_q,
                           const float* eps_p, float* g_src, float* g_ref, int64_t pixels, int Z, void* stream);

int fmi_avgpool_f32(const float* x, float* y, int N, int H, int W, int C, int k, void* stream);
int fmi_avgpool_bwd_f32(const float* gy, float* gx, int N, int H, int W, int C, int k, void* stream);
int fmi_instnorm_stats_bf16(const uint16_t* x, double* sums, float* stats, int N, int HW, int C, float eps, double* ws, int64_t ws_doubles,
                            void* stream);
int fmi_instnorm_apply_bf16(const uint16_t* x, const float* stats, const float* gamma, const float* beta, uint16_t* y, int N, int HW, int C,
                            float slope, void* stream);
int fmi_instnorm_bwd_reduce_bf16(const uint16_t* x, const uint16_t* gy, const float* stats, const float* gamma, const float* beta, double* red,
                                 int N, int HW, int C, float slope, double* ws, int64_t ws_doubles, void* stream);
int fmi_instnorm_bwd_apply_bf16(const uint16_t* x, const uint16_t* gy, const float* stats, const float* gamma, const float* beta,
                                const double* red, const uint16_t* gadd, uint16_t* gx, float* dgamma, float* dbeta, int N, int HW, int C,
                                float slope, void* stream);
int fmi_prelu_bf16(const uint16_t* x, const float* a, uint16_t* y, int64_t rows, int C, void* stream);
int fmi_prelu_bwd_bf16(const uint16_t* g, const uint16_t* x, const float* a, uint16_t* gx, float* ga, float* ws, int64_t ws_floats, int64_t rows,
                       int C, void* stream);
int fmi_scale_channels_add_bf16(const uint16_t* x, const float* s, const uint16_t* res, uint16_t* y, int N, int64_t P, int C, void* stream);
int fmi_add_bf16(const uint16_t* a, const uint16_t* b, uint16_t* y, int64_t n, void* stream);
int fmi_global_avgpool_bf16(const uint16_t* x, float* pooled, float* ws, int64_t ws_floats, int N, int64_t P, int C, void* stream);
int fmi_add_bcast_bf16(const uint16_t* g, const float* gpool, uint16_t* gx, int N, int64_t P, int C, void* stream);
int fmi_add_bcast_f32(const float* g, const float* gpool, float* gx, int N, int64_t P, int C, void* stream);
int fmi_subsample_bf16(const uint16_t* x, uint16_t* y, int N, int H, int W, int C, int stride, int backward, void* stream);
int fmi_scale_channels_add_f32(const float* x, const float* s, const float* res, float* y, int N, int64_t P, int C, void* stream);
int fmi_scale_channels_bwd_f32(const float* g, const float* x, const float* s, float* gx, float* gs, float* ws, int64_t ws_floats, int N,
                               int64_t P, int C, void* stream);
int fmi_instnorm_bwd_apply_add_f32(const float* x, const float* gy, const float* stats, const float* gamma, const float* beta,
                                   const double* red, const float* gadd, float* gx, float* dgamma, float* dbeta, int N, int HW, int C,
                                   float slope, void* stream);
int fmi_l2norm_rows_f32(const float* x, float* y, float* inv_norm, int64_t rows, int C, float eps, void* stream);
int fmi_l2norm_rows_bwd_f32(const float* g, const float* y, const float* inv_norm, float* gx, int64_t rows, int C, float eps, void* stream);
int fmi_lpips_layer_f32(const float* fx, const float* fy, const float* w, float* out, int64_t pixels, int C, float scale, void* stream);
int fmi_lpips_layer_bwd_f32(const float* fx, const float* fy, const float* w, const float* gout, float* gfx, float* gfy, int64_t pixels,
                            int C, float scale, void* stream);
int fmi_copy_channels_f32(const float* src, float* dst, int64_t rows, int src_stride, int src_c0, int dst_stride, int dst_c0, int c,
                          void* stream);
int fmi_copy_channels_bf16(const uint16_t* src, uint16_t* dst, int64_t rows, int src_stride, int src_c0, int dst_stride, int dst_c0, int c,
                           void* stream);
int fmi_adaptive_avgpool_f32(const float* x, float* y, int N, int H, int W, int C, int OH, int OW, void* stream);
int fmi_adaptive_avgpool_bwd_f32(const float* gy, float* gx, int N, int H, int W, int C, int OH, int OW, void* stream);
int fmi_maxpool_f32(const float* x, float* y, int32_t* argmax, int N, int H, int W, int C, int k, int stride, void* stream);
int fmi_maxpool_bwd_f32(const float* gy, const int32_t* argmax, float* gx, int N, int H, int W, int C, int k, int stride, void* stream);
int fmi_image_tail_f32(const float* x, float* pooled, float* unit, uint8_t* u8, int N, int S, float shift, float scale, void* stream);
int fmi_planes_to_u8_f32(const float* x, uint8_t* u8, int N, int C, int H, int W, float shift, float scale, void* stream);
int fmi_argmax_channels_f32(const float* x, float* out, int64_t pixels, int C, void* stream);
int fmi_maxpool2_f32(const float* x, float* y, int N, int H, int W, int C, void* stream);
int fmi_maxpool2_bwd_f32(const float* x, const float* gy, float* gx, int N, int H, int W, int C, void* stream);
int fmi_resize_bilinear_f32(const float* x, float* y, int N, int H, int W, int C, int OH, int OW,
                            const float* ch_mean, const float* ch_std, void* stream);
int fmi_resize_bilinear_bwd_f32(const float* gy, float* gx, int N, int H, int W, int C, int OH, int OW,
                                const float* ch_std, void* stream);
int fmi_instnorm_stats_f32(const float* x, double* sums , float* stats ,
                           int N, int HW, int C, float eps, double* ws, int64_t ws_doubles, void* stream);
int fmi_instnorm_apply_f32(const float* x, const float* stats, const float* gamma, const float* beta, float* y,
                           int N, int HW, int C, float slope, void* stream);
int fmi_batchnorm_running_update_f32(const float* stats, const double* sums, float* running_mean, float* running_var,
                                     int64_t* num_batches_tracked, int C, int64_t count, float eps, float momentum, void* stream);
int fmi_batchnorm_running_update_offset_f32(const float* stats, const double* sums, const float* mean_offset, float* running_mean,
                                            float* running_var, int64_t* num_batches_tracked, int C, int64_t count, float eps,
                                            float momentum, void* stream);
int fmi_instnorm_bwd_reduce_f32(const float* x, const float* gy, const float* stats, const float* gamma,
                                const float* beta, double* red, int N, int HW, int C, float slope, double* ws, int64_t ws_doubles,
                                void* stream);
int fmi_instnorm_bwd_apply_f32(const float* x, const float* gy, const float* stats, const float* gamma,
                               const float* beta, const double* red, float* gx, float* dgamma, float* dbeta,
                               int N, int HW, int C, float slope, void* stream);

int fmi_reduce_loss_f32(int kind, const float* a, const float* b, int64_t n, float c0, float scale,
                        float* out, void* stream);
int fmi_reduce_loss_bwd_f32(int kind, const float* a, const float* b, int64_t n, float c0, float scale,
                            const float* gscale, float* ga, void* stream);


int fmi_ssim_f32(const float* img1, const float* img2, const float* window1d, int ws, int planes, int H, int W,
                 int planes_per_out, float* out_zeroed, void* stream);
int fmi_ssim_valid_f32(const float* img1, const float* img2, const float* window1d, int ws, int planes, int H, int W, float C1, float C2,
                       float* out_plane2, double* ws_part, int64_t ws_doubles, void* stream);
int fmi_avgpool2_pad_f32(const float* x, float* y, int planes, int H, int W, int pad_h, int pad_w, void* stream);

int fmi_seg_ce_dice_fwd_f32(const float* logits, const void* target, int target_kind, int64_t P, int C, double eps, float* out3,
                            double* sums, double* ws_part, int64_t ws_doubles, void* stream);
int fmi_seg_ce_dice_bwd_f32(const float* logits, const void* target, int target_kind, int64_t P, int C, double eps, const double* sums,
                            const float* gout, float* dlogits, void* stream);
int fmi_seg_dice_score_f32(const float* logits, const void* target, int target_kind, int N, int64_t HW, int C, double eps, float* out,
                           double* ws_part, int64_t ws_doubles, void* stream);
int fmi_plane_sums_f32(const float* a, const float* b, int planes, int64_t n, double* out3, double* ws_part, int64_t ws_doubles, void* stream);

int fmi_psp_pixel_head_fwd_f32(const float* y_hat, const float* y, const float* ref, const float* mask, float* pair_out, float* pair_in,
                               double* sums, float* out2, int N, int H, int W, int y_hat_hwc, double* ws_part, int64_t ws_doubles, void* stream);
int fmi_psp_pixel_head_bwd_f32(const float* y_hat, const float* y, const float* ref, const float* mask, const float* g_pair_out,
                               const float* g_pair_in, const float* g2, float* d_y_hat, int N, int H, int W, int y_hat_hwc, void* stream);

int fmi_gan_image_head_fwd_f32(const float* gen, const float* gt, const float* src, const float* ref, const float* mask, const float* mean,
                               const float* stdv, float* x_in, float* y_in, float* l1, int N, int H, int W, int OH, int OW, int gen_hwc,
                               double* ws_part, int64_t ws_doubles, void* stream);
int fmi_gan_image_head_bwd_f32(const float* gen, const float* gt, const float* mask, const float* stdv, const float* gx, const float* g_l1,
                               float* d_gen, int N, int H, int W, int OH, int OW, int gen_hwc, void* stream);

int fmi_cx_channel_mean_f32(const float* y, float* mu , int64_t rows, int C, void* stream);
int fmi_cx_normalise_f32(const float* x, const float* mu, float* out, float* inv_norm, int64_t rows, int C, void* stream);
int fmi_cx_normalise_bwd_f32(const float* g, const float* xn, const float* inv_norm, float* gx, int64_t rows, int C, void* stream);
int fmi_cx_rows_f32(const float* cosm, float* cxij, float* dmin, int* argmin, float* rowsum, int N, int P, float h, void* stream);
int fmi_cx_cols_f32(const float* cxij, float* colmax, int* colarg, int N, int P, void* stream);
int fmi_cx_loss_f32(const float* colmax, float* cx , float* loss , int N, int P, float scale, void* stream);
int fmi_cx_bwd_f32(const float* cxij, const float* dmin, const int* argmin, const float* rowsum, const float* cosm,
                   const int* colarg, const float* cx, const float* gscale, float* dcos, int N, int P, float h, float scale,
                   void* stream);

typedef struct {
  float* p; const float* g; float* m; float* v; int64_t n;
} fmi_adam_entry;
int fmi_adam_step_f32(const fmi_adam_entry* entries , int count, int64_t max_n, float lr, float beta1, float beta2,
                      float eps, float weight_decay, int step, void* stream);
int fmi_adam_step_dev_f32(const fmi_adam_entry* entries , int count, float lr, float beta1, float beta2, float eps,
                          float weight_decay, int* step_dev, void* stream);
int fmi_adam_step_dev_guarded_f32(const fmi_adam_entry* entries , int count, float lr, float beta1, float beta2, float eps,
                                  float weight_decay, int* step_dev, const float* guard, void* stream);
typedef struct {
  float* p; const float* g; float* m; float* v; float* slow; float* row_mean; int64_t n; int64_t cols;
} fmi_ranger_entry;
int fmi_ranger_step_f32(const fmi_ranger_entry* entries , int count, float lr, float beta1, float beta2, float eps,
                        float weight_decay, float step_size, int rectified, float alpha, int lookahead, void* stream);

int fmi_upfirdn2d_f32(const float* in, const float* kernel, float* out, int major, int in_h, int in_w,
                      int kh, int kw, int up_x, int up_y, int down_x, int down_y,
                      int pad_x0, int pad_x1, int pad_y0, int pad_y1, void* stream);
int fmi_upfirdn2d_bf16(const uint16_t* in, const uint16_t* kernel, uint16_t* out, int major, int in_h, int in_w, int kh, int kw,
                       int up_x, int up_y, int down_x, int down_y, int pad_x0, int pad_x1, int pad_y0, int pad_y1, void* stream);
int fmi_fused_bias_act_f32(const float* x, const float* bias, const float* ref, float* out, int64_t n,
                           int step_b, int size_b, int act, int grad, float alpha, float scale, void* stream);
int fmi_fused_bias_act_bf16(const uint16_t* x, const uint16_t* bias, const uint16_t* ref, uint16_t* out, int64_t n, int step_b,
                            int size_b, int act, int grad, float alpha, float scale, void* stream);
int fmi_bias_grad_nchw_f32(const float* g, int N, int C, int64_t HW, float* dbias, void* stream);
int fmi_bias_grad_nchw_bf16(const void* g, int N, int C, int64_t HW, float* dbias, void* stream);
int fmi_noise_bias_act_f32(const float* x, const float* bias, const float* noise, const float* nw, float* y,
                           int64_t pixels, int C, float alpha, float scale, void* stream);

int fmi_scale_channels_f32(const float* x, const float* s, float* y, int N, int64_t P, int C, void* stream);
int fmi_scale_channels_gs_f32(const float* g, const float* x, float* gs, float* ws, int64_t ws_floats, int N, int64_t P, int C, void* stream);
int fmi_sqsum_last_f32(const float* x, float* out, int64_t rows, int k, void* stream);
int fmi_sqsum_last_bwd_f32(const float* x, const float* g, float* gx, int64_t rows, int k, void* stream);
int fmi_noise_bias_act_bwd_f32(const float* g, const float* y, const float* noise, float* gx, float* gnw,
                               int64_t pixels, int C, float alpha, float scale, void* stream);
int fmi_upfirdn2d_nhwc_f32(const float* in, const float* kernel, float* out, int N, int in_h, int in_w, int C,
                           int kh, int kw, int up_x, int up_y, int down_x, int down_y,
                           int pad_x0, int pad_x1, int pad_y0, int pad_y1, void* stream);

int fmi_prelu_f32(const float* x, const float* a, float* y, int64_t rows, int C, void* stream);
int fmi_prelu_bwd_f32(const float* g, const float* x, const float* a, float* gx, float* ga, float* ws, int64_t ws_floats, int64_t rows,
                      int C, void* stream);
int fmi_subsample_f32(const float* x, float* y, int N, int H, int W, int C, int stride, int backward, void* stream);

int fmi_maxpool2_bf16(const uint16_t* x, uint16_t* y, int N, int H, int W, int C, void* stream);
int fmi_maxpool2_bwd_bf16(const uint16_t* x, const uint16_t* gy, uint16_t* gx, int N, int H, int W, int C, void* stream);
int fmi_up2_cat_bf16(const uint16_t* x1, const uint16_t* skip, uint16_t* y, int N, int h, int w, int C1, int H, int W, int C2, void* stream);
int fmi_up2_cat_bwd_bf16(const uint16_t* g, uint16_t* gskip, uint16_t* gx1, int N, int h, int w, int C1, int H, int W, int C2, void* stream);
int fmi_head1x1_bf16(const uint16_t* x, const float* w, const float* b, float* y, int64_t P, int C, int K, void* stream);
int fmi_head1x1_argmax_bf16(const uint16_t* x, const float* w, const float* b, float* mask, int64_t P, int C, int K, void* stream);
int fmi_head1x1_bwd_bf16(const float* g, const uint16_t* x, const float* w, uint16_t* gx, float* gw, float* gb, double* ws,
                         int64_t ws_doubles, int64_t P, int C, int K, void* stream);

#define FMI_CHAN_COLSUM_ROWS 64
int fmi_conv2d_fwd_chan_bf16(const fmi_conv_desc* d, const uint16_t* x, const uint16_t* wnk, const float* scale, const float* bias,
                             const float* slope, uint16_t* y, float* colsum, int64_t colsum_floats, void* stream);
int fmi_se_gate_f32(const float* part, int rows_per_part, int64_t P, float inv_count, const float* fc1, const float* fc2, float* gates, int N,
                    int C, void* stream);
int fmi_irse_tail_bf16(const uint16_t* r, const float* gate, const uint16_t* sc, const float* next_scale, const float* next_shift, uint16_t* y,
                       uint16_t* z, float* tap, int N, int OH, int OW, int C, int SH, int SW, int sc_stride, void* stream);
int fmi_irse_stem_bf16(const float* x, const float* scale, const float* shift, uint16_t* y, uint16_t* z, int64_t rows, int C, void* stream);

int fmi_conv2d_thin_in_fwd_bf16(const fmi_conv_desc* d, const float* x, const float* wf, const float* bias, float slope, uint16_t* y,
                                void* stream);
int fmi_conv2d_c32_fwd_bf16(const fmi_conv_desc* d, const uint16_t* x, const uint16_t* wnk, const float* bias, float slope, uint16_t* y,
                            void* stream);
int fmi_resblock_tail_bf16(const uint16_t* main_, const uint16_t* shortcut, uint16_t* y_raw, uint16_t* y_act, float* y_f32, int N, int H, int W,
                           int C, int pool, float slope, void* stream);
int fmi_picnet_stem_tail_bf16(const uint16_t* h, const float* img, const float* wb, const float* bias, uint16_t* y_raw, uint16_t* y_act, int N,
                              int H, int W, int C, int K, float slope, void* stream);
int fmi_guided_attention_fwd_bf16_waves(int N, int T);
int fmi_guided_attention_fwd_bf16(const uint16_t* q, const uint16_t* src, const uint16_t* ref, const float* mask, uint16_t* out, int N, int T,
                                  int D, int C, int waves, void* stream);

#ifdef __cplusplus
}
#endif
#endif
```

Before: 105.3 images/s.

## Emit bf16 split-3 pieces directly from conv and maxpool epilogues in VGG loss

Adds an optional y3 output to the conv GEMM epilogue and a new maxpool2 kernel so the three-piece bf16 split of an output is written while the fp32 result is stored. This replaces the separate split3 pass that the next conv in the perceptual loss would otherwise run. Size thresholds gate the fused path, so it only applies to large tensors. It also adds float4-vectorised maxpool2 forward and backward kernels. The cost is extra epilogue stores and register pressure in the GEMM.

```diff
diff --git a/face_mask_inpaint_amd/_lib.py b/face_mask_inpaint_amd/_lib.py
--- a/face_mask_inpaint_amd/_lib.py
+++ b/face_mask_inpaint_amd/_lib.py
@@ -109,6 +109,7 @@
     "fmi_avgpool_f32": [vp, vp, i32, i32, i32, i32, i32, vp],
     "fmi_avgpool_bwd_f32": [vp, vp, i32, i32, i32, i32, i32, vp],
     "fmi_maxpool2_f32": [vp, vp, i32, i32, i32, i32, vp],
+    "fmi_maxpool2_p3_f32": [vp, vp, vp, i32, i32, i32, i32, vp],
     "fmi_maxpool2_bf16": [vp, vp, i32, i32, i32, i32, vp],
     "fmi_maxpool2_bwd_bf16": [vp, vp, vp, i32, i32, i32, i32, vp],
     "fmi_up2_cat_bf16": [vp, vp, vp, i32, i32, i32, i32, i32, i32, i32, vp],
diff --git a/face_mask_inpaint_amd/csrc/conv.hip b/face_mask_inpaint_amd/csrc/conv.hip
--- a/face_mask_inpaint_amd/csrc/conv.hip
+++ b/face_mask_inpaint_amd/csrc/conv.hip
@@ -89,7 +89,8 @@
 }
 
 static int conv_phase(const fmi_conv_desc* d, const ConvGeom& g, const float* x, const void* x3, const float* w, const void* w3p,
-                      int64_t w_bstride, int Nout, int flip, ConvEp ep, int batch_w, bool may_split, bool shared_init, hipStream_t st) {
+                      int64_t w_bstride, int Nout, int flip, ConvEp ep, int batch_w, bool may_split, bool shared_init, bool* y3_left,
+                      hipStream_t st) {
   ConvK la{x, g};
   ConvWX lb{w, g, w_bstride, Nout, (Nout % 4 == 0) && aligned16(w) && (w_bstride % 4 == 0)};
   const int ks = may_split ? conv_ksplit(g.Mdim(), Nout, g.Kdim()) : 1;
@@ -105,6 +106,8 @@
     ep.act = 3;
     ep.vec = 0;
   }
+  if (!ep.vec) ep.y3 = nullptr;
+  if (!ep.y3) *y3_left = true;
   const uint16_t* w3 = (const uint16_t*)w3p;
   const int64_t w3_stride = (int64_t)d->kh * d->kw * d->C * d->K;
   const int64_t pixels = (int64_t)g.N * g.IH * g.IW;
@@ -123,7 +126,8 @@
   }
   if (w3 && la.dma_ok()) return launch_gemm(la, ConvWX3{w3, g, w3_stride, Nout}, ep, g.Mdim(), Nout, g.Kdim(), 1, ks, st);
 #endif
-  return launch_gemm(la, lb, ep, g.Mdim(), Nout, g.Kdim(), batch_w, ks, st);
+  *y3_left = true;
+  return launch_gemm(la, lb, ConvEpF32(ep), g.Mdim(), Nout, g.Kdim(), batch_w, ks, st);
 }
 
 static const void* weight_pieces(const fmi_conv_desc* d, int batch_w, int red_c) {
@@ -148,9 +152,10 @@
   if (rc) return rc;
   if (!x || !wf || !y || batch_w < 1 || act < 0 || act > 2) return FMI_ERR_BAD_ARG;
   if (batch_w > 1 && batch_w != d->N) return FMI_ERR_BAD_ARG;
+  bool y3_left = true;
   auto finish = [&](int rc) {
 #ifndef FMI_HOST_EMU
-    if (rc == FMI_OK && d->y3) rc = fmi_split3_f32(y, d->y3, nullptr, (int64_t)d->N * d->OH * d->OW, d->K, 0, 0.f, stream);
+    if (rc == FMI_OK && d->y3 && y3_left) rc = fmi_split3_f32(y, d->y3, nullptr, (int64_t)d->N * d->OH * d->OW, d->K, 0, 0.f, stream);
 #endif
     return rc;
   };
@@ -164,7 +169,11 @@
   const void* w3 = weight_pieces(d, batch_w, d->C);
   ConvEp ep{y, bias, residual, d->OH, d->OW, 1, 0, 0, d->OH, d->OW, d->y_cstride, act, g.dGW, g.dG, (int64_t)d->OH * d->OW * d->y_cstride};
   ep.vec = ep_vec(ep, d->K);
-  return finish(conv_phase(d, g, x, d->x3, wf, w3, w_bstride, d->K, 0, ep, batch_w, act == 0 && batch_w == 1, false, (hipStream_t)stream));
+#ifndef FMI_HOST_EMU
+  ep.y3 = (uint16_t*)d->y3;
+  y3_left = false;
+#endif
+  return finish(conv_phase(d, g, x, d->x3, wf, w3, w_bstride, d->K, 0, ep, batch_w, act == 0 && batch_w == 1, false, &y3_left, (hipStream_t)stream));
 }
 
 static int dgrad_impl(const fmi_conv_desc* d, const float* dy, const float* wt, const float* bias, const float* residual,
@@ -178,9 +187,10 @@
   if (d->pad_mode != 0) return FMI_ERR_UNSUPPORTED;
   if (batch_w > 1 && batch_w != d->N) return FMI_ERR_BAD_ARG;
   if (mask && bias) return FMI_ERR_UNSUPPORTED;
+  bool y3_left = true;
   auto finish = [&](int rc) {
 #ifndef FMI_HOST_EMU
-    if (rc == FMI_OK && d->y3) rc = fmi_split3_f32(dx, d->y3, nullptr, (int64_t)d->N * d->H * d->W, d->C, 0, 0.f, stream);
+    if (rc == FMI_OK && d->y3 && y3_left) rc = fmi_split3_f32(dx, d->y3, nullptr, (int64_t)d->N * d->H * d->W, d->C, 0, 0.f, stream);
 #endif
     return rc;
   };
@@ -221,6 +231,7 @@
     ca.ep = ep;
     return finish(launch_convt3x3(ca, d->N * d->OH * d->OW, (hipStream_t)stream));
   }
+  y3_left = false;
 #endif
   for (int py = 0; py < s; ++py) {
     for (int px = 0; px < s; ++px) {
@@ -231,8 +242,9 @@
       ep.mask = mask;
       ep.mslope = mslope;
       ep.vec = ep_vec(ep, d->C);
+      if (!y3_left) ep.y3 = (uint16_t*)d->y3;
       rc = conv_phase(d, g, dy, d->x3, wt, w3, w_bstride, d->C, 1, ep, batch_w, batch_w == 1 && (s == 1 || strided_split), strided_split,
-                      (hipStream_t)stream);
+                      &y3_left, (hipStream_t)stream);
       if (rc) return rc;
     }
   }
diff --git a/face_mask_inpaint_amd/csrc/gemm_core.h b/face_mask_inpaint_amd/csrc/gemm_core.h
--- a/face_mask_inpaint_amd/csrc/gemm_core.h
+++ b/face_mask_inpaint_amd/csrc/gemm_core.h
@@ -437,13 +437,15 @@
   int vec = 0;
   const float* mask = nullptr;
   float mslope = 0.f;
+  uint16_t* y3 = nullptr;
   static constexpr bool HAS_VEC4 = true;
   __device__ __forceinline__ void set_batch(int b) {
     y += (int64_t)b * bs;
     if (res) res += (int64_t)b * bs;
     if (mask) mask += (int64_t)b * bs;
-  }
-  __device__ __forceinline__ void store4(int64_t off, int col, float4 v) const {
+    if (y3) y3 += 3 * (int64_t)b * bs;
+  }
+  __device__ __forceinline__ float4 store4_f32(int64_t off, int col, float4 v) const {
     if (mask) {
       const float4 m4 = *reinterpret_cast<const float4*>(mask + off + col);
       v.x *= m4.x > 0.f ? 1.f : mslope, v.y *= m4.y > 0.f ? 1.f : mslope, v.z *= m4.z > 0.f ? 1.f : mslope, v.w *= m4.w > 0.f ? 1.f : mslope;
@@ -459,6 +461,20 @@
     if (act == 1) v.x = tanhf(v.x), v.y = tanhf(v.y), v.z = tanhf(v.z), v.w = tanhf(v.w);
     else if (act == 2) v.x = fmaxf(v.x, 0.f), v.y = fmaxf(v.y, 0.f), v.z = fmaxf(v.z, 0.f), v.w = fmaxf(v.w, 0.f);
     *reinterpret_cast<float4*>(y + off + col) = v;
+    return v;
+  }
+  __device__ __forceinline__ void store4(int64_t off, int col, float4 v) const {
+    v = store4_f32(off, col, v);
+#ifndef FMI_HOST_EMU
+    if (y3) {
+      uint32_t w[3][2];
+      split3_pair(v.x, v.y, w[0][0], w[1][0], w[2][0]);
+      split3_pair(v.z, v.w, w[0][1], w[1][1], w[2][1]);
+      uint16_t* q = y3 + 3 * off + (col >> 4) * 48 + (col & 15);
+#pragma unroll
+      for (int pc = 0; pc < 3; ++pc) *reinterpret_cast<uint2*>(q + pc * 16) = make_uint2(w[pc][0], w[pc][1]);
+    }
+#endif
   }
   __device__ __forceinline__ int64_t row_off(int row) const {
     const uint32_t n = fdiv((uint32_t)row, dG);
@@ -479,6 +495,10 @@
     else if (act == 2) v = fmaxf(v, 0.f);
     y[off + col] = v;
   }
+};
+struct ConvEpF32 : ConvEp {
+  explicit ConvEpF32(const ConvEp& e) : ConvEp(e) { y3 = nullptr; }
+  __device__ __forceinline__ void store4(int64_t off, int col, float4 v) const { store4_f32(off, col, v); }
 };
 
 struct WgradEp {
diff --git a/face_mask_inpaint_amd/csrc/pool.hip b/face_mask_inpaint_amd/csrc/pool.hip
--- a/face_mask_inpaint_amd/csrc/pool.hip
+++ b/face_mask_inpaint_amd/csrc/pool.hip
@@ -1,4 +1,5 @@
 #include "common.h"
+#include "x6.h"
 
 
 template <int V>
@@ -177,14 +178,115 @@
     gx[i] = g;
   }
 }
-extern "C" int fmi_maxpool2_f32(const float* x, float* y, int N, int H, int W, int C, void* stream) {
+template <bool P3>
+__global__ void __launch_bounds__(256) maxpool2_v4_kernel(const float4* __restrict__ x, float4* __restrict__ y, uint16_t* __restrict__ y3, int N,
+                                                          int H, int W, int C4) {
+  const int OH = H / 2, OW = W / 2;
+  const int ox = blockIdx.x * blockDim.y + threadIdx.y;
+  if (ox >= OW) return;
+  const int64_t down = (int64_t)W * C4;
+  for (int n = blockIdx.z; n < N; n += gridDim.z)
+    for (int oy = blockIdx.y; oy < OH; oy += gridDim.y) {
+      const float4* p = x + (((int64_t)n * H + oy * 2) * W + ox * 2) * C4;
+      const int64_t pix = ((int64_t)n * OH + oy) * OW + ox;
+      for (int c = threadIdx.x; c < C4; c += blockDim.x) {
+        const float4 v0 = p[c], v1 = p[C4 + c], v2 = p[down + c], v3 = p[down + C4 + c];
+        float4 m;
+        m.x = fmaxf(fmaxf(fmaxf(v0.x, v1.x), v2.x), v3.x);
+        m.y = fmaxf(fmaxf(fmaxf(v0.y, v1.y), v2.y), v3.y);
+        m.z = fmaxf(fmaxf(fmaxf(v0.z, v1.z), v2.z), v3.z);
+        m.w = fmaxf(fmaxf(fmaxf(v0.w, v1.w), v2.w), v3.w);
+        y[pix * C4 + c] = m;
+        if (P3) {
+          uint32_t w[3][2];
+          split3_pair(m.x, m.y, w[0][0], w[1][0], w[2][0]);
+          split3_pair(m.z, m.w, w[0][1], w[1][1], w[2][1]);
+          uint16_t* q = y3 + (pix * (C4 >> 2) + (c >> 2)) * 48 + (c & 3) * 4;
+#pragma unroll
+          for (int pc = 0; pc < 3; ++pc) *reinterpret_cast<uint2*>(q + pc * 16) = make_uint2(w[pc][0], w[pc][1]);
+        }
+      }
+    }
+}
+__device__ __forceinline__ void maxpool2_route(float v0, float v1, float v2, float v3, float g, float& o0, float& o1, float& o2, float& o3) {
+  int arg = 0;
+  float m = v0;
+  if (v1 > m) { m = v1; arg = 1; }
+  if (v2 > m) { m = v2; arg = 2; }
+  if (v3 > m) { m = v3; arg = 3; }
+  o0 = arg == 0 ? g : 0.f, o1 = arg == 1 ? g : 0.f, o2 = arg == 2 ? g : 0.f, o3 = arg == 3 ? g : 0.f;
+}
+__global__ void __launch_bounds__(256) maxpool2_bwd_v4_kernel(const float4* __restrict__ x, const float4* __restrict__ gy, float4* __restrict__ gx,
+                                                              int N, int H, int W, int C4) {
+  const int OH = H / 2, OW = W / 2;
+  const int ox = blockIdx.x * blockDim.y + threadIdx.y;
+  if (ox >= OW) return;
+  const int64_t down = (int64_t)W * C4;
+  const bool tail_x = (W & 1) && ox == OW - 1;
+  const float4 z = make_float4(0.f, 0.f, 0.f, 0.f);
+  for (int n = blockIdx.z; n < N; n += gridDim.z)
+    for (int oy = blockIdx.y; oy < OH; oy += gridDim.y) {
+      const int64_t base = (((int64_t)n * H + oy * 2) * W + ox * 2) * C4;
+      const float4* p = x + base;
+      float4* o = gx + base;
+      const float4* gp = gy + (((int64_t)n * OH + oy) * OW + ox) * C4;
+      const bool tail_y = (H & 1) && oy == OH - 1;
+      for (int c = threadIdx.x; c < C4; c += blockDim.x) {
+        const float4 v0 = p[c], v1 = p[C4 + c], v2 = p[down + c], v3 = p[down + C4 + c], g = gp[c];
+        float4 o0, o1, o2, o3;
+        maxpool2_route(v0.x, v1.x, v2.x, v3.x, g.x, o0.x, o1.x, o2.x, o3.x);
+        maxpool2_route(v0.y, v1.y, v2.y, v3.y, g.y, o0.y, o1.y, o2.y, o3.y);
+        maxpool2_route(v0.z, v1.z, v2.z, v3.z, g.z, o0.z, o1.z, o2.z, o3.z);
+        maxpool2_route(v0.w, v1.w, v2.w, v3.w, g.w, o0.w, o1.w, o2.w, o3.w);
+        o[c] = o0, o[C4 + c] = o1, o[down + c] = o2, o[down + C4 + c] = o3;
+        if (tail_x) o[2 * C4 + c] = z, o[down + 2 * C4 + c] = z;
+        if (tail_y) {
+          o[2 * down + c] = z, o[2 * down + C4 + c] = z;
+          if (tail_x) o[2 * down + 2 * C4 + c] = z;
+        }
+      }
+    }
+}
+static void maxpool2_v4_dims(int N, int H, int W, int C4, dim3& grid, dim3& block) {
+  const int OH = H / 2, OW = W / 2;
+  const int bx = C4 < 256 ? C4 : 256;
+  int by = 256 / bx;
+  if (by > OW) by = OW;
+  block = dim3(bx, by);
+  grid = dim3((OW + by - 1) / by, OH < 65535 ? OH : 65535, N < 65535 ? N : 65535);
+}
+static int maxpool2_fwd(const float* x, float* y, void* y3, int N, int H, int W, int C, void* stream) {
   if (!x || !y || N <= 0 || H < 2 || W < 2 || C <= 0) return FMI_ERR_BAD_ARG;
+  const bool v4 = C % 4 == 0 && fmi_al16(x) && fmi_al16(y);
+  if (y3 && (!v4 || C % 16 != 0 || !fmi_al16(y3))) return FMI_ERR_BAD_ARG;
+  if (v4) {
+    dim3 grid, block;
+    maxpool2_v4_dims(N, H, W, C / 4, grid, block);
+    const float4* x4 = reinterpret_cast<const float4*>(x);
+    float4* y4 = reinterpret_cast<float4*>(y);
+    if (y3) hipLaunchKernelGGL(maxpool2_v4_kernel<true>, grid, block, 0, (hipStream_t)stream, x4, y4, (uint16_t*)y3, N, H, W, C / 4);
+    else hipLaunchKernelGGL(maxpool2_v4_kernel<false>, grid, block, 0, (hipStream_t)stream, x4, y4, (uint16_t*)nullptr, N, H, W, C / 4);
+    return fmi_launch_status();
+  }
   const int64_t total = (int64_t)N * (H / 2) * (W / 2) * C;
   hipLaunchKernelGGL(maxpool2_kernel, dim3(fmi_bw_grid(total, 256)), dim3(256), 0, (hipStream_t)stream, x, y, H, W, C, total);
   return fmi_launch_status();
 }
+extern "C" int fmi_maxpool2_f32(const float* x, float* y, int N, int H, int W, int C, void* stream) {
+  return maxpool2_fwd(x, y, nullptr, N, H, W, C, stream);
+}
+extern "C" int fmi_maxpool2_p3_f32(const float* x, float* y, void* y3, int N, int H, int W, int C, void* stream) {
+  return maxpool2_fwd(x, y, y3, N, H, W, C, stream);
+}
 extern "C" int fmi_maxpool2_bwd_f32(const float* x, const float* gy, float* gx, int N, int H, int W, int C, void* stream) {
   if (!x || !gy || !gx || N <= 0 || H < 2 || W < 2 || C <= 0) return FMI_ERR_BAD_ARG;
+  if (C % 4 == 0 && fmi_al16(x) && fmi_al16(gy) && fmi_al16(gx)) {
+    dim3 grid, block;
+    maxpool2_v4_dims(N, H, W, C / 4, grid, block);
+    hipLaunchKernelGGL(maxpool2_bwd_v4_kernel, grid, block, 0, (hipStream_t)stream, reinterpret_cast<const float4*>(x),
+                       reinterpret_cast<const float4*>(gy), reinterpret_cast<float4*>(gx), N, H, W, C / 4);
+    return fmi_launch_status();
+  }
   const int64_t total = (int64_t)N * H * W * C;
   hipLaunchKernelGGL(maxpool2_bwd_kernel, dim3(fmi_bw_grid(total, 256)), dim3(256), 0, (hipStream_t)stream, x, gy, gx, H, W, C, total);
   return fmi_launch_status();
diff --git a/face_mask_inpaint_amd/functional.py b/face_mask_inpaint_amd/functional.py
--- a/face_mask_inpaint_amd/functional.py
+++ b/face_mask_inpaint_amd/functional.py
@@ -147,6 +147,10 @@
 
 
 P3_ENABLED = True
+P3_FUSED_PIECES = True
+P3_SPLIT_PASSES = 0
+P3_FUSED_CONV_MIN_ELEMS = 1 << 25
+P3_FUSED_POOL_MIN_ELEMS = 1 << 23
 P3_MIN_PIXELS = 16384
 P3_MIN_WORK = 1152
 P3_MIN_COUT = 64
@@ -165,6 +169,8 @@
     p = getattr(t, "_fmi_p3", None)
     if p is not None and p[1] == t._version and lrelu_from is None:
         return p[0]
+    global P3_SPLIT_PASSES
+    P3_SPLIT_PASSES += 1
     x3 = torch.empty(t.numel() * 3, device=t.device, dtype=torch.bfloat16)
     if lrelu_from is not None:
         _L().split3_f32(_p(lrelu_from), C.c_void_p(x3.data_ptr()), _p(t), t.numel() // c, c, 1, float(slope), _st())
@@ -176,6 +182,17 @@
         _L().split3_f32(_p(t), C.c_void_p(x3.data_ptr()), None, t.numel() // c, c, 0, 0.0, _st())
     t._fmi_p3 = (x3, t._version)
     return x3
+
+
+def _p3_new(t: torch.Tensor, hint: bool) -> Optional[torch.Tensor]:
+    if not (hint and P3_FUSED_PIECES and P3_ENABLED) or t.shape[-1] % 16 or not t.is_cuda or t.data_ptr() % 16:
+        return None
+    return torch.empty(t.numel() * 3, device=t.device, dtype=torch.bfloat16)
+
+
+def _p3_put(t: torch.Tensor, x3: Optional[torch.Tensor]) -> None:
+    if x3 is not None:
+        t._fmi_p3 = (x3, t._version)
 
 
 class PackedWeight:
@@ -285,7 +302,8 @@
 class _Conv2d(torch.autograd.Function):
 
     @staticmethod
-    def forward(ctx, x, wf, bias, residual, wt, kh, kw, stride, pad, pad_mode, act, in_act=None, skip_act_bwd=False, dil=1, passthrough=False, w3=(None, None)):
+    def forward(ctx, x, wf, bias, residual, wt, kh, kw, stride, pad, pad_mode, act, in_act=None, skip_act_bwd=False, dil=1, passthrough=False, w3=(None, None),
+                y3_hint=False, gx3_hint=False):
         _chk(x, wf, bias, residual)
         lib = _L()
         x_in = x
@@ -305,8 +323,13 @@
         ctx.wt3 = w3[1]
         ctx.x3 = x3
         y = torch.empty((n, oh, ow, k), device=x.device, dtype=torch.float32)
+        y3 = _p3_new(y, y3_hint and y.numel() >= P3_FUSED_CONV_MIN_ELEMS)
+        if y3 is not None:
+            d.y3 = y3.data_ptr()
         with _prof(f"conv_fwd|{n}x{h}x{w} {c}->{k} k{kh}s{stride}" + (f"d{dil}" if dil > 1 else ""), 2.0 * n * oh * ow * k * c * kh * kw):
             lib.conv2d_fwd_f32(C.byref(d), _p(x), _p(wf), _p(bias), _p(residual), _p(y), act, 1, 0, _st())
+        _p3_put(y, y3)
+        ctx.gx3_hint = bool(gx3_hint)
         ctx.save_for_backward(x, wf, y if (act and not skip_act_bwd) else None)
         ctx.wt, ctx.cfg, ctx.has = wt, (kh, kw, stride, pad, pad_mode, act), (bias is not None, residual is not None)
         ctx.dil = dil
@@ -321,7 +344,7 @@
         lib = _L()
         x, wf, y = ctx.saved_tensors
         if gy is None:
-            return (gpass,) + (None,) * 15
+            return (gpass,) + (None,) * 17
         kh, kw, stride, pad, pad_mode, act = ctx.cfg
         gy = gy.contiguous()
         if act and not ctx.skip_act_bwd:
@@ -351,6 +374,9 @@
                 gy3 = p3_of(gy, colsum=gb_of_split) if (ctx.wt3 is not None and p3_wanted(n * oh_ * ow_, k, c, kh * kw)) else None
                 d, _, _ = conv_desc(n, h, w, c, k, kh, kw, stride, pad, dil=dil, w3=ctx.wt3, x3=gy3)
                 gx = torch.empty_like(x)
+                gx3 = _p3_new(gx, ctx.gx3_hint and gx.numel() >= P3_FUSED_CONV_MIN_ELEMS)
+                if gx3 is not None:
+                    d.y3 = gx3.data_ptr()
                 with _prof(f"conv_dgrad|{n}x{h}x{w} {c}->{k} k{kh}s{stride}", 2.0 * gy.numel() * c * kh * kw):
                     if ctx.in_slope is not None and gpass is not None:
                         lib.conv2d_dgrad_masked_add_f32(C.byref(d), _p(gy), _p(ctx.wt), _p(x), ctx.in_slope, _p(gpass.contiguous()), _p(gx), _st())
@@ -363,6 +389,7 @@
                         gpass = None
                     else:
                         lib.conv2d_dgrad_f32(C.byref(d), _p(gy), _p(ctx.wt), None, None, _p(gx), 1, 0, _st())
+                _p3_put(gx, gx3)
             if ctx.in_slope is not None and not masked:
                 gx = eltwise(EW_LRELU_BWD, gx, x, ctx.in_slope)
             if gpass is not None:
@@ -405,7 +432,7 @@
                 lib.bias_grad_f32(_p(gy), gy.numel() // k, k, k, _p(gb), _st())
         if ctx.has[1] and ctx.needs_input_grad[3]:
             gres = gy
-        return gx, gwf, gb, gres, None, None, None, None, None, None, None, None, None, None, None, None
+        return gx, gwf, gb, gres, None, None, None, None, None, None, None, None, None, None, None, None, None, None
 
 
 class _ThinConvLReLU(torch.autograd.Function):
@@ -476,12 +503,13 @@
 
 
 def conv2d(x, pw: PackedWeight, bias=None, residual=None, stride=1, pad=0, pad_mode=0, act=ACT_NONE, in_act=None, skip_act_bwd=False, dilation=1,
-           passthrough=False):
+           passthrough=False, y3_hint=False, gx3_hint=False):
     if x.dtype == BF16:
         if bias is not None or residual is not None or pad_mode or act or in_act is not None or dilation != 1:
             raise FmiError("the bf16 convolution has no bias / residual / activation / reflect-padding / dilation form")
         return _Conv2dBF16.apply(x, pw.wf, pw.wt, pw.kh, pw.kw, stride, pad)
-    return _Conv2d.apply(x, pw.wf, bias, residual, pw.wt, pw.kh, pw.kw, stride, pad, pad_mode, act, in_act, skip_act_bwd, int(dilation), bool(passthrough), pw.w3)
+    return _Conv2d.apply(x, pw.wf, bias, residual, pw.wt, pw.kh, pw.kw, stride, pad, pad_mode, act, in_act, skip_act_bwd, int(dilation), bool(passthrough), pw.w3,
+                         bool(y3_hint), bool(gx3_hint))
 
 
 BF16 = torch.bfloat16
@@ -1061,11 +1089,16 @@
 
 class _MaxPool2(torch.autograd.Function):
     @staticmethod
-    def forward(ctx, x):
+    def forward(ctx, x, y3_hint=False):
         _chk(x)
         n, h, w, c = x.shape
         y = torch.empty((n, h // 2, w // 2, c), device=x.device, dtype=torch.float32)
-        _L().maxpool2_f32(_p(x), _p(y), n, h, w, c, _st())
+        y3 = _p3_new(y, y3_hint and x.data_ptr() % 16 == 0 and y.numel() >= P3_FUSED_POOL_MIN_ELEMS)
+        if y3 is not None:
+            _L().maxpool2_p3_f32(_p(x), _p(y), C.c_void_p(y3.data_ptr()), n, h, w, c, _st())
+            _p3_put(y, y3)
+        else:
+            _L().maxpool2_f32(_p(x), _p(y), n, h, w, c, _st())
         ctx.save_for_backward(x)
         return y
 
@@ -1075,7 +1108,7 @@
         n, h, w, c = x.shape
         gx = torch.empty_like(x)
         _L().maxpool2_bwd_f32(_p(x), _p(g.contiguous()), _p(gx), n, h, w, c, _st())
-        return gx
+        return gx, None
 
 
 class _MaxPool2BF16(torch.autograd.Function):
@@ -1100,10 +1133,10 @@
         return gx
 
 
-def max_pool2(x):
+def max_pool2(x, y3_hint=False):
     if x.dtype == BF16:
         return _MaxPool2BF16.apply(x)
-    return _MaxPool2.apply(x)
+    return _MaxPool2.apply(x, bool(y3_hint))
 
 
 class _Up2CatBF16(torch.autograd.Function):
diff --git a/face_mask_inpaint_amd/modules/loss.py b/face_mask_inpaint_amd/modules/loss.py
--- a/face_mask_inpaint_amd/modules/loss.py
+++ b/face_mask_inpaint_amd/modules/loss.py
@@ -50,16 +50,25 @@
         for c, pw in zip(convs, self._cache["pws"]):
             object.__setattr__(c, "_fmi_packed", pw)
 
+    @staticmethod
+    def _takes_pieces(m, pixels, adjoint):
+        w3 = packed(m).w3[1 if adjoint else 0]
+        cred, cout = (m.out_channels, m.in_channels) if adjoint else (m.in_channels, m.out_channels)
+        return w3 is not None and FF.p3_wanted(pixels, cred, cout, m.kernel_size[0] * m.kernel_size[1])
+
     def _block(self, bi, x):
         mods = [m for m in self.blocks[bi] if isinstance(m, (nn.MaxPool2d, nn.Conv2d))]
         prev_conv = False
         for i, m in enumerate(mods):
+            next_conv = i + 1 < len(mods) and isinstance(mods[i + 1], nn.Conv2d)
+            n, h, w, _ = x.shape
             if isinstance(m, nn.MaxPool2d):
-                x = FF.max_pool2(x)
+                x = FF.max_pool2(x, y3_hint=next_conv and self._takes_pieces(mods[i + 1], n * (h // 2) * (w // 2), False))
                 prev_conv = False
             else:
-                next_conv = i + 1 < len(mods) and isinstance(mods[i + 1], nn.Conv2d)
-                x = run_conv(m, x, act=FF.ACT_RELU, in_act=("mask", 0.0) if prev_conv else None, skip_act_bwd=next_conv)
+                x = run_conv(m, x, act=FF.ACT_RELU, in_act=("mask", 0.0) if prev_conv else None, skip_act_bwd=next_conv,
+                             y3_hint=next_conv and self._takes_pieces(mods[i + 1], n * h * w, False),
+                             gx3_hint=prev_conv and self._takes_pieces(mods[i - 1], n * h * w, True))
                 prev_conv = True
         return x
 
diff --git a/face_mask_inpaint_amd/modules/pluralistic_model/external_function.py b/face_mask_inpaint_amd/modules/pluralistic_model/external_function.py
--- a/face_mask_inpaint_amd/modules/pluralistic_model/external_function.py
+++ b/face_mask_inpaint_amd/modules/pluralistic_model/external_function.py
@@ -44,7 +44,8 @@
             return run_conv(self.module, x_nhwc, residual=residual, act=act, pad_mode=pad_mode, pad=pad)
 
 
-def run_conv(conv: nn.Module, x_nhwc, residual=None, act=FF.ACT_NONE, pad_mode=0, pad=None, in_act=None, skip_act_bwd=False, passthrough=False):
+def run_conv(conv: nn.Module, x_nhwc, residual=None, act=FF.ACT_NONE, pad_mode=0, pad=None, in_act=None, skip_act_bwd=False, passthrough=False,
+             y3_hint=False, gx3_hint=False):
     pw = packed(conv)
     if isinstance(conv, nn.ConvTranspose2d):
         if conv.stride[0] != conv.stride[1] or conv.padding[0] != conv.padding[1] or conv.groups != 1:
@@ -57,7 +58,8 @@
     if conv.stride[0] != conv.stride[1] or conv.padding[0] != conv.padding[1] or conv.groups != 1 or conv.dilation[0] != conv.dilation[1]:
         raise NotImplementedError("Conv2d geometry outside the hot path")
     p = conv.padding[0] if pad is None else pad
-    return FF.conv2d(x_nhwc, pw, conv.bias, residual, conv.stride[0], p, pad_mode, act, in_act, skip_act_bwd, conv.dilation[0], passthrough)
+    return FF.conv2d(x_nhwc, pw, conv.bias, residual, conv.stride[0], p, pad_mode, act, in_act, skip_act_bwd, conv.dilation[0], passthrough,
+                     y3_hint, gx3_hint)
 
 
 class GANLoss(nn.Module):
diff --git a/include/fmi_hip.h b/include/fmi_hip.h
--- a/include/fmi_hip.h
+++ b/include/fmi_hip.h
@@ -254,6 +254,7 @@
 int fmi_argmax_channels_f32(const float* x, float* out, int64_t pixels, int C, void* stream);
 int fmi_maxpool2_f32(const float* x, float* y, int N, int H, int W, int C, void* stream);
 int fmi_maxpool2_bwd_f32(const float* x, const float* gy, float* gx, int N, int H, int W, int C, void* stream);
+int fmi_maxpool2_p3_f32(const float* x, float* y, void* y3, int N, int H, int W, int C, void* stream);
 int fmi_resize_bilinear_f32(const float* x, float* y, int N, int H, int W, int C, int OH, int OW,
                             const float* ch_mean, const float* ch_std, void* stream);
 int fmi_resize_bilinear_bwd_f32(const float* gy, float* gx, int N, int H, int W, int C, int OH, int OW,
```

Result: no change. 105.9 images/s (median of 6 runs) (+0.7%).
